# cy-rae/fast-slam

Hardware: AMD Instinct MI355X
Metric: particle-updates/s (higher is better)
Workload: dtype f64

## Files before the change

### fast-slam_amd/csrc/fs2_api.hip

```cpp
#include <hip/hip_runtime.h>

#include <sched.h>
#include <unistd.h>

#include <algorithm>
#include <atomic>
#include <chrono>
#include <condition_variable>
#include <functional>
#include <cmath>
#include <cstdarg>
#include <cstdio>
#include <cstdlib>
#include <cstring>
#include <mutex>
#include <new>
#include <string>
#include <thread>
#include <tuple>
#include <vector>

#include "../../include/fs2.h"
#include "fs2_comm.hpp"
#include "fs2_frontend.hpp"
// ... 190 lines not shown
        return n;
    }
};
ChunkCache g_chunks;

std::atomic<int> g_vm_fail_after_relocate{0};
struct GmStep {
    const char *what;
    size_t bytes;
    std::chrono::steady_clock::time_point t0 = std::chrono::steady_clock::now();
    ~GmStep() {
        static const bool on = std::getenv("FS2_TRACE") != nullptr;
        if (!on) return;
        const double ms = std::chrono::duration<double, std::milli>(std::chrono::steady_clock::now() - t0).count();
        std::fprintf(stderr, "[fs2 vmm] %s %zu MiB %.3f ms\n", what, bytes >> 20, ms);
    }
};
static void gm_drop(const GrowMem &g, size_t b, hipMemGenericAllocationHandle_t hd) {
    if (!g_chunks.put(ChunkCache::Chunk{g.device, g.shareable, b, hd})) (void)hipMemRelease(hd);
}
static hipError_t gm_grow(GrowMem &g, size_t bytes) {
    const size_t need = (bytes + g.gran - 1) / g.gran * g.gran;
    if (need <= g.mapped) return hipSuccess;
    std::vector<size_t> plan;
    size_t want = g.mapped;
    while (want < need) {
        plan.push_back(chunk_size(need - want, g.gran));
        want += plan.back();
    }
    if (want > g.reserved) {
        GmStep st{"relocate", want};
        const hipError_t e = gm_relocate(g, want);
        if (e != hipSuccess) return e;
        if (g_vm_fail_after_relocate.exchange(0)) return gm_fail(hipErrorOutOfMemory);
    }
    hipMemAllocationProp prop = gm_prop(g.device, g.shareable);
    const size_t mapped0 = g.mapped, nchunks0 = g.chunks.size();
    hipError_t e = hipSuccess;
    int cached = 0;
    {
        GmStep st{"chunks", want - mapped0};
        for (size_t b : plan) {
            hipMemGenericAllocationHandle_t hd{};
            if (g_chunks.take(g.device, g.shareable, b, &hd)) {
                ++cached;
            } else {
                e = hipMemCreate(&hd, b, &prop, 0);
                if (e == hipErrorOutOfMemory && g_chunks.release() > 0) {
                    (void)hipGetLastError();
                    e = hipMemCreate(&hd, b, &prop, 0);
                }
                if (e != hipSuccess) break;
            }
            e = hipMemMap(g.base + g.mapped, b, 0, hd, 0);
            if (e != hipSuccess) {
                gm_drop(g, b, hd);
                break;
            }
            g.chunks.push_back({hd, b});
            g.mapped += b;
        }
    }
    if (e == hipSuccess) {
        GmStep st{"access", want};
        e = gm_access(g, g.base, want);
    }
    if (e != hipSuccess) {
        while (g.chunks.size() > nchunks0) {
            const auto c = g.chunks.back();
            g.chunks.pop_back();
            g.mapped -= c.second;
            (void)hipMemUnmap(g.base + g.mapped, c.second);
            gm_drop(g, c.second, c.first);
        }
        g.mapped = mapped0;
        return gm_fail(e);
    }
    if (cached && std::getenv("FS2_TRACE")) std::fprintf(stderr, "[fs2 vmm] %d of %zu chunks from closed handles\n", cached, plan.size());
    return hipSuccess;
}
static void gm_free(GrowMem &g) {
    GmStep st{"free", g.mapped};
    size_t off = g.mapped;
    for (auto it = g.chunks.rbegin(); it != g.chunks.rend(); ++it) {
        off -= it->second;
        hipMemUnmap(g.base + off, it->second);
        gm_drop(g, it->second, it->first);
    }
    g.chunks.clear();
    if (g.base) hipMemAddressFree(g.base, g.reserved);
    g = GrowMem{};
}

struct Pool {
    const char *name;
    size_t item_bytes;
    int64_t id_limit;
    char *data = nullptr;
    int64_t n = 0;
    GrowMem vm;
    uint8_t *mark = nullptr;
    GrowMem mark_vm;
    uint32_t *freel = nullptr;
    GrowMem freel_vm;
    int64_t nfree = 0, cursor = 0;
    uint8_t epoch = 0;
    int64_t *bcnt = nullptr;
    int64_t bcnt_cap = 0;
    int64_t *nfree_dev = nullptr;

    int64_t room() const { return nfree - cursor; }
    int64_t live() const { return n - room(); }
    bool in_place() const { return vm.base && data == vm.base; }
    hipError_t next_epoch(hipStream_t s) {
        if (epoch == 255) {
            const hipError_t e = hipMemsetAsync(mark, 0, (size_t)n, s);
            if (e != hipSuccess) return e;
            epoch = 0;
        }
        epoch += 1;
        return hipSuccess;
    }
    bool mapped() const { return vm.base || mark_vm.base || freel_vm.base; }
    void release() {
        if (vm.base) gm_free(vm); else hipFree(data);
        if (mark_vm.base) gm_free(mark_vm); else hipFree(mark);
        if (freel_vm.base) gm_free(freel_vm); else hipFree(freel);
        hipFree(bcnt);
        hipFree(nfree_dev);
    }
};

}

struct MtCtx {
    fs2_mt_state in;
    double sigma = 0.0;
    int64_t N = 0, P = 0, A = 0, amb_cap = 0, pos0 = 0, have = 0, total = 0;
    int h0 = 0;
    fs2_mt_state *after = nullptr, *after_u0 = nullptr;
    double *u0_out = nullptr;
};

struct fs2_handle {
    fs2_config cfg{};
    int64_t n_global = 0, n = 0, first = 0;
    hipStream_t stream = nullptr;
    int cur = 0;
    double *x[2] = {}, *y[2] = {}, *yaw[2] = {}, *w[2] = {};
    int32_t *cnt[2] = {};
    Pool pages{"page", kPageBytes, (int64_t)kIdMask};
    Pool records{"record", kRecBytes, (int64_t)kRecIdLimit};
    Desc *pt[2] = {};
    uint32_t *bbox[2] = {};
    XDesc *rdesc = nullptr;
    XDesc *udesc = nullptr;
    size_t udesc_cap = 0;
    unsigned long long *xt_key = nullptr;
    uint32_t *xt_ref = nullptr, *xt_uidx = nullptr, *xt_cmask = nullptr, *xt_cbase = nullptr;
    uint32_t *xt_eslot = nullptr, *xt_ulist = nullptr;
    int64_t xt_cap = 0, xt_ecap = 0;
    SumFrame frame{-127.0f, 1.0f, 1.0f};
    float ext_seen = 0.0f;
    float *slb = nullptr;
    float *slb_pass = nullptr;
    uint32_t *ext_dev = nullptr;
    size_t rdesc_cap = 0;
    int rows = 0;
    uint32_t *sent_mask = nullptr;
    uint64_t collections = 0;
    int64_t u_recv = 0;
    int32_t *rank_d = nullptr, *rank_e = nullptr;
    int64_t *iblk = nullptr;
    int cap = 0, max_cap = kMaxSlots;
    double *wpart = nullptr, *part_sq = nullptr, *part_best_w = nullptr, *part_pose = nullptr;
    unsigned long long *cpart = nullptr;
    int64_t *part_best_i = nullptr;
    unsigned long long *part_slots = nullptr;
    int32_t *part_maxcnt = nullptr;
    double *cbuf = nullptr, *bsum = nullptr;
    DevStats *stats_dev = nullptr;
    char *post_host = nullptr, *post = nullptr;
    unsigned long long *post_flag = nullptr, *post_flag_dev = nullptr;
    unsigned long long post_seq = 0;
    PackPlan *plan = nullptr;
    DevStats *pub_stats = nullptr, *pub_stats_dev = nullptr;
    unsigned long long *pub_flag = nullptr, *pub_flag_dev = nullptr;
    unsigned long long pub_seq = 0;
    bool stats_clean = false;
    double *noise_dev = nullptr, *noise_pin = nullptr, *u0_dev = nullptr, *u0_pin = nullptr;
    struct MtWork {
        uint32_t *raw[2] = {};
        int64_t raw_cap[2] = {};
        int cur = 0;
        hipStream_t side = nullptr;
        hipEvent_t ev_words = nullptr, ev_pre = nullptr;
        bool pre_valid = false;
        uint32_t pre_key[2][624];
        int32_t pre_spos[2];
        int64_t pre_pos0[2];
        int64_t pre_total = 0;
        int32_t *boff = nullptr;
        int64_t boff_cap = 0;
        MtMeta *meta = nullptr, *meta_pin = nullptr;
        MtAmb *amb = nullptr, *amb_pin = nullptr;
        int64_t amb_cap = 0;
        uint32_t *words_pin = nullptr;
        int64_t *pidx = nullptr, *pidx_pin = nullptr;
        double *pval = nullptr, *pval_pin = nullptr;
        int64_t patch_cap = 0, pval_cap = 0;
        double *tab = nullptr;
        int64_t jJ = 0;
        int jG = 0;
        uint64_t *jpoly = nullptr;
        uint32_t *jwin = nullptr;
        bool tab_ready = false;
        bool armed = false;
        hipStream_t dstream = nullptr;
        hipEvent_t ev_in = nullptr, ev_noise = nullptr;
        bool deferred = false;
        MtCtx dc;
    } mt;
    int32_t *assoc_dev = nullptr;
    int64_t assoc_cap = 0;
    int32_t last_m = 0;
    uint64_t scan = 0;
    struct Pending {
        bool on = false;
        unsigned long long seq = 0;
        bool prof = false;
        int passes = 0;
        int32_t m = 0;
        uint64_t fixed_bytes = 0;
    } pending;
    struct TailCtx {
        int32_t M = 0;
        int passes = 0;
        uint64_t fixed_bytes = 0;
        bool prof = false;
        int evset = 0;
        int32_t want_collect = 0;
        bool has_u0 = false;
        int par = 0;
    };
    struct {
        bool on = false;
        int rc = FS2_OK;
        double pose[3] = {};
        fs2_iter_stats st{};
    } stash;
    uint32_t *gen_dev = nullptr;
    unsigned long long *go_dev = nullptr;
    BufSet *sets_dev = nullptr;
    uint64_t submitted = 0;
    int32_t cnt_upper = 0;
    double gate2 = 64.0;
    std::string err;
    bool profiling = false;
    int32_t prof_period = 1;
    uint64_t prof_tick = 0;
    ProfEvents ev;
    fs2_profile prof{};
    fs2comm::Transport *tp = nullptr;
    RankRecord *rec = nullptr, *recs = nullptr;
    double *totals = nullptr;
    int64_t *xrow = nullptr, *xmat = nullptr;
    int32_t *mlo = nullptr, *mhi = nullptr, *out_src = nullptr;
    uint32_t *runs_n = nullptr;
    int4 *runs = nullptr;
    uint64_t *cand = nullptr;
    int32_t *ncand = nullptr;
    char *sarena = nullptr, *rarena = nullptr;
    size_t scap = 0, rcap = 0;
    int32_t n_recv = 0;
    int32_t shard = 0;
    int8_t rank_of[kMaxRanks] = {};
    bool follow = false;
    uint64_t shard_moves = 0;

    int32_t *uinfo = nullptr, *uol = nullptr, *seql = nullptr, *bC = nullptr, *bpc = nullptr;
    uint32_t *bM = nullptr;
    int32_t *uel = nullptr, *bE = nullptr, *bpe = nullptr;
    long long *udelta = nullptr;
    unsigned long long *ugl = nullptr, *bD = nullptr, *bpd = nullptr;
    double *sout = nullptr, *part_w = nullptr, *np_part = nullptr, *np_leaf = nullptr, *sentry = nullptr;
    NpTailPlan *np_tail = nullptr;
    UnitRec *urec = nullptr;
    bool xsh_ok = false;
    bool refs = false;
    bool refs_off = false;
    bool refuse_maps = false;
    bool room_check = false;
    bool refs_shared = false;
    bool vm_share = false;
    uint32_t loc_epoch = 0;
    bool refs_live = false;
    uint64_t grows = 0;
    uint64_t vm_fallbacks = 0;
    int64_t appends_since_rcollect = 0;
    bool rcollect_exact = true;
    std::vector<uint8_t> imported;
    PeerMaps peers_host{};
    PeerMaps *peers_dev = nullptr;
    uint8_t *ep_dev = nullptr, *epochs_dev = nullptr;
    int64_t remote_rows = 0;
    int64_t remote_pages = INT64_MAX;
    int64_t remote_bound() const { return std::min(remote_rows, remote_pages); }
    int32_t collect_next = 0;
    ChainSummary *dch_send = nullptr, *dch_recv = nullptr;
    RankRecordX *recx = nullptr, *recxs = nullptr;
    double *est_base = nullptr;
    int32_t *uop = nullptr;
    NpTailPlan *np_tail_g = nullptr;
    std::vector<std::pair<hipEvent_t, hipEvent_t>> xev;
    size_t xev_used = 0;
    struct Guard {
        char *at;
        const char *name;
    };
    std::vector<Guard> guards;
    bool guard = false;
    char *json_text = nullptr;
    int64_t *json_boff = nullptr;
    size_t json_text_cap = 0, json_boff_cap = 0;
    double *post_part = nullptr, *post_out = nullptr;
    unsigned long long *post_grid = nullptr;
    size_t post_part_cap = 0, post_out_cap = 0, post_grid_cap = 0;
    char *map_scr = nullptr, *map_out = nullptr;
    double *map_part = nullptr;
    unsigned long long *map_grid = nullptr;
    size_t map_scr_cap = 0, map_out_cap = 0, map_part_cap = 0, map_grid_cap = 0;

    MapRef map() const {
        return MapRef{pages.data, pt[cur], std::max<int64_t>(n, 1), rows, records.data, frame, slb, row_boxes(cur),
                      refs_shared ? peers_dev : nullptr};
    }
    uint32_t *row_boxes(int b) const { return rows <= kBBoxRows ? bbox[b] : nullptr; }
    int64_t nblocks() const { return (n + kBlock - 1) / kBlock; }
    int reduce() const {
        const int mode = cfg.reduce_mode;
        if (tp) {
            if (mode == FS2_REDUCE_SEQUENTIAL) return FS2_REDUCE_SEQUENTIAL;
            return (mode != FS2_REDUCE_PARALLEL && xsh_ok) ? FS2_REDUCE_EXACT : FS2_REDUCE_PARALLEL;
        }
        if (mode != FS2_REDUCE_AUTO) return mode;
        return n_global <= 4096 ? FS2_REDUCE_SEQUENTIAL : FS2_REDUCE_EXACT;
    }
    ChainParams chain(const double *a, const double *bsum, double *c, double *total, bool lazy) const {
        ChainParams p{};
        p.a = a;
        p.n = n;
        p.bsum = bsum;
        p.nb = (int32_t)nblocks();
        p.lazy = lazy ? 1 : 0;
        p.uinfo = uinfo;
        p.udelta = udelta;
        p.ugl = ugl;
        p.uol = uol;
        p.bD = bD;
        p.bC = bC;
        p.bM = bM;
        p.bpd = bpd;
        p.bpc = bpc;
        p.uel = uel;
        p.bE = bE;
        p.bpe = bpe;
        p.seql = seql;
        p.sout = sout;
        p.urec = urec;
        p.sentry = sentry;
        p.c = c;
        p.total = total;
        p.stats = stats_dev;
        p.margin = std::ldexp(2.0 * (double)n_global + 8192.0, -53);
        p.chain_first = 1;
        return p;
    }
};

static hipError_t copy_sync(fs2_handle *h, void *dst, const void *src, size_t bytes, hipMemcpyKind kind) {
    hipError_t e = hipMemcpyAsync(dst, src, bytes, kind, h->stream);
    return e == hipSuccess ? hipStreamSynchronize(h->stream) : e;
}

struct CommTimer {
    fs2_handle *h;
    std::chrono::steady_clock::time_point t0 = std::chrono::steady_clock::now();
    explicit CommTimer(fs2_handle *hh) : h(hh) {}
    ~CommTimer();
};

CommTimer::~CommTimer() {
    if (!h->profiling) return;
    h->prof.comm_calls += 1;
    h->prof.comm_ms += std::chrono::duration<double, std::milli>(std::chrono::steady_clock::now() - t0).count();
}

static int recv_bufs(fs2_handle *h, size_t bytes) {
    if (bytes <= h->rdesc_cap && bytes <= h->udesc_cap) return FS2_OK;
    HIP_TRY(h, hipStreamSynchronize(h->stream));
    for (int k = 0; k < 2; ++k) {
        XDesc *&p = k ? h->udesc : h->rdesc;
        size_t &cap = k ? h->udesc_cap : h->rdesc_cap;
        if (bytes <= cap) continue;
        hipFree(p);
        p = nullptr;
        cap = 0;
        HIP_TRY(h, hipMalloc(&p, bytes));
        cap = bytes;
    }
    return FS2_OK;
}

static int reserve_xfer_table(fs2_handle *h, int64_t cap, int64_t nrows, bool in_scan);
static int xfer_bufs(fs2_handle *h) {
    const int64_t S = std::max<int64_t>(h->n, 1) * h->rows;
    int lg = 10;
    while ((int64_t(1) << lg) < 2 * S && lg < 31) ++lg;
    const int rc = reserve_xfer_table(h, int64_t(1) << lg, S, false);
    return rc ? rc : recv_bufs(h, sizeof(XDesc) * (size_t)S);
}

static int sync_sets(fs2_handle *h) {
    if (!h->sets_dev) return FS2_OK;
    BufSet b[2];
    for (int k = 0; k < 2; ++k)
        b[k] = BufSet{h->x[k], h->y[k], h->yaw[k], h->w[k], h->cnt[k], h->pt[k], h->row_boxes(k)};
    HIP_TRY(h, copy_sync(h, h->sets_dev, b, sizeof b, hipMemcpyHostToDevice));
    return FS2_OK;
}

static int grow_rows(fs2_handle *h, int need_slots) {
    if (need_slots <= h->cap) return FS2_OK;
    if (need_slots > h->max_cap)
        return set_err(&h->err, FS2_ERR_CAPACITY, "map needs %d landmark slots, limit is %d",
                       need_slots, h->max_cap);
    int rows = (need_slots + kPageSlots - 1) / kPageSlots;
    if (h->rows > 0) {
        const int geo = h->rows + std::max(h->rows / 4, 8);
        const int lim = std::min(h->max_cap / kPageSlots, rows <= kBBoxRows ? kBBoxRows : INT_MAX);
        rows = std::max(rows, std::min(geo, lim));
    }
    const size_t row_bytes = sizeof(Desc) * (size_t)std::max<int64_t>(h->n, 1);
    HIP_TRY(h, hipStreamSynchronize(h->stream));
    for (int b = 0; b < 2; ++b) {
        Desc *p = nullptr;
        HIP_TRY(h, hipMalloc(&p, row_bytes * rows));
        if (h->pt[b] && b == h->cur) HIP_TRY(h, copy_sync(h, p, h->pt[b], row_bytes * h->rows, hipMemcpyDeviceToDevice));
        hipFree(h->pt[b]);
        h->pt[b] = p;
    }
    h->rows = rows;
    h->cap = rows * kPageSlots;
    if (int rc = sync_sets(h)) return rc;
    if (h->rdesc) return xfer_bufs(h);
    return FS2_OK;
}

static int refs_short(fs2_handle *h, const char *what) {
    return set_err(&h->err, FS2_ERR_CAPACITY,
                   "page_refs mode: the %s pool ran short between collective collections (pools shared with "
                   "the other ranks cannot grow; size them with page_pool / record_pool)",
                   what);
}

static int collect_body(fs2_handle *h, bool recs_too);
struct PoolTimer {
    fs2_handle *h;
    bool grow;
    std::chrono::steady_clock::time_point t0 = std::chrono::steady_clock::now();
    ~PoolTimer() {
        const double ms = std::chrono::duration<double, std::milli>(std::chrono::steady_clock::now() - t0).count();
        if (grow) {
            h->prof.pool_grows += 1;
            h->prof.grow_ms += ms;
        } else {
            h->prof.pool_collections += 1;
            h->prof.collect_ms += ms;
        }
    }
};
static int collect(fs2_handle *h, bool recs_too) {
    PoolTimer pt{h, false};
    return collect_body(h, recs_too);
}
static int collect_records(fs2_handle *h) {
    Pool &p = h->pages, &r = h->records;
    if (r.n <= 0) return FS2_OK;
    hipStream_t s = h->stream;
    HIP_TRY(h, r.next_epoch(s));
// ... 707 lines not shown
    int prev_dev = -1;
    if (hipGetDevice(&prev_dev) != hipSuccess) prev_dev = -1;
    if (prev_dev != h->cfg.device) (void)hipSetDevice(h->cfg.device);
    if (h->stream) hipStreamSynchronize(h->stream);
    if (h->mt.dstream) hipStreamSynchronize(h->mt.dstream);
    const bool vmm = h->pages.mapped() || h->records.mapped();
    if (vmm) hipDeviceSynchronize();
    if (h->refs_shared && h->tp && !h->tp->in_process()) {
        std::string e;
        if (h->tp->allgather(h->ep_dev, h->epochs_dev, 1, h->stream, &e) == FS2_OK) hipStreamSynchronize(h->stream);
        h->tp->unshare();
        if (h->tp->allgather(h->ep_dev, h->epochs_dev, 1, h->stream, &e) == FS2_OK) hipStreamSynchronize(h->stream);
    }
    for (int s = 0; s < 2; ++s) {
        hipFree(h->x[s]); hipFree(h->y[s]); hipFree(h->yaw[s]); hipFree(h->w[s]); hipFree(h->cnt[s]);
        hipFree(h->pt[s]);
        hipFree(h->bbox[s]);
    }
    hipFree(h->rdesc); hipFree(h->udesc);
    hipFree(h->xt_key); hipFree(h->xt_ref); hipFree(h->xt_uidx); hipFree(h->xt_cmask); hipFree(h->xt_cbase);
    hipFree(h->xt_eslot); hipFree(h->xt_ulist);
    hipFree(h->sent_mask);
    h->pages.release();
    h->records.release();
    if (vmm) hipDeviceSynchronize();
    hipFree(h->slb); hipFree(h->slb_pass); hipFree(h->ext_dev);
    hipFree(h->rank_d); hipFree(h->rank_e); hipFree(h->iblk);
    hipFree(h->mlo); hipFree(h->mhi); hipFree(h->out_src); hipFree(h->runs); hipFree(h->runs_n);
    hipFree(h->rec); hipFree(h->recs); hipFree(h->totals); hipFree(h->xrow); hipFree(h->xmat);
    hipFree(h->sarena);
    hipFree(h->rarena);
    hipFree(h->cand); hipFree(h->ncand);
    hipFree(h->uinfo); hipFree(h->uol); hipFree(h->seql); hipFree(h->udelta); hipFree(h->ugl);
    hipFree(h->bD); hipFree(h->bC); hipFree(h->bM); hipFree(h->bpd); hipFree(h->bpc);
    hipFree(h->uel); hipFree(h->bE); hipFree(h->bpe);
    hipFree(h->sout); hipFree(h->np_leaf); hipFree(h->part_w); hipFree(h->np_part); hipFree(h->np_tail);
    hipFree(h->urec); hipFree(h->sentry);
    hipFree(h->dch_send); hipFree(h->dch_recv); hipFree(h->recx); hipFree(h->recxs); hipFree(h->est_base);
    hipFree(h->uop); hipFree(h->np_tail_g);
    hipFree(h->peers_dev); hipFree(h->ep_dev); hipFree(h->epochs_dev);
    hipFree(h->part_pose);
    hipFree(h->gen_dev); hipFree(h->sets_dev); hipFree(h->go_dev);
    hipFree(h->wpart); hipFree(h->cpart); hipFree(h->part_sq); hipFree(h->part_best_w); hipFree(h->part_best_i); hipFree(h->part_slots);
    hipFree(h->part_maxcnt); hipFree(h->cbuf); hipFree(h->bsum);
    hipFree(h->stats_dev); hipFree(h->noise_dev); hipFree(h->u0_dev); hipFree(h->assoc_dev);
    hipFree(h->json_text); hipFree(h->json_boff);
    hipFree(h->post_part); hipFree(h->post_out); hipFree(h->post_grid);
    hipFree(h->map_scr); hipFree(h->map_out); hipFree(h->map_part); hipFree(h->map_grid);
    if (h->post_host) hipHostFree(h->post_host);
    hipFree(h->plan);
    if (h->pub_stats) hipHostFree(h->pub_stats);
    if (h->noise_pin) hipHostFree(h->noise_pin);
    if (h->u0_pin) hipHostFree(h->u0_pin);
    if (h->mt.side) hipStreamSynchronize(h->mt.side);
    if (h->mt.dstream) {
        hipStreamSynchronize(h->mt.dstream);
        hipStreamDestroy(h->mt.dstream);
        hipEventDestroy(h->mt.ev_in);
        hipEventDestroy(h->mt.ev_noise);
    }
    hipFree(h->mt.raw[0]); hipFree(h->mt.raw[1]); hipFree(h->mt.boff);
    if (h->mt.ev_words) hipEventDestroy(h->mt.ev_words);
    if (h->mt.ev_pre) hipEventDestroy(h->mt.ev_pre);
    if (h->mt.side) hipStreamDestroy(h->mt.side); hipFree(h->mt.meta); hipFree(h->mt.amb); hipFree(h->mt.pidx);
    hipFree(h->mt.pval); hipFree(h->mt.tab); hipFree(h->mt.jpoly); hipFree(h->mt.jwin);
    if (h->mt.meta_pin) hipHostFree(h->mt.meta_pin);
    if (h->mt.amb_pin) hipHostFree(h->mt.amb_pin);
    if (h->mt.words_pin) hipHostFree(h->mt.words_pin);
    if (h->mt.pidx_pin) hipHostFree(h->mt.pidx_pin);
    if (h->mt.pval_pin) hipHostFree(h->mt.pval_pin);
    if (h->ev.ok)
        for (auto &set : h->ev.e)
            for (auto &e : set) hipEventDestroy(e);
    for (auto &e : h->xev) {
        hipEventDestroy(e.first);
        hipEventDestroy(e.second);
    }
    delete h->tp;
    if (h->stream) hipStreamDestroy(h->stream);
    const int dev = h->cfg.device;
    delete h;
    if (prev_dev >= 0 && prev_dev != dev) (void)hipSetDevice(prev_dev);
}

int fs2_create(const fs2_config *cfg, fs2_handle **out) {
    if (!cfg || !out) return set_err(nullptr, FS2_ERR_ARG, "fs2_create: null argument");
    *out = nullptr;
    if (cfg->num_particles <= 0)
        return set_err(nullptr, FS2_ERR_ARG, "num_particles must be positive");
    if (cfg->world_size < 1 || cfg->rank < 0 || cfg->rank >= cfg->world_size)
        return set_err(nullptr, FS2_ERR_ARG, "bad rank %d / world_size %d", cfg->rank, cfg->world_size);
    if (cfg->world_size > kMaxRanks)
        return set_err(nullptr, FS2_ERR_ARG, "world_size %d > %d", cfg->world_size, kMaxRanks);
    if (cfg->num_particles > (int64_t)INT32_MAX)
        return set_err(nullptr, FS2_ERR_ARG, "too many particles per rank");
    int ndev = 0;
    if (hipGetDeviceCount(&ndev) != hipSuccess || ndev == 0)
        return set_err(nullptr, FS2_ERR_HIP, "no HIP device available (libfs2 has no CPU path)");
    if (cfg->device < 0 || cfg->device >= ndev)
        return set_err(nullptr, FS2_ERR_ARG, "device %d out of range (%d devices)", cfg->device, ndev);

    fs2_handle *h = new fs2_handle();
    h->cfg = *cfg;
    h->n_global = cfg->num_particles;
    const int64_t G = cfg->world_size, r = cfg->rank;
    h->first = (h->n_global * r) / G;
    h->n = (h->n_global * (r + 1)) / G - h->first;
    h->shard = (int32_t)r;
    for (int q = 0; q < kMaxRanks; ++q) h->rank_of[q] = (int8_t)(q < G ? q : 0);
    {
        const char *e = std::getenv("FS2_SHARD_FOLLOW");
        h->follow = G > 1 && h->n_global % G == 0 && !(e && std::strcmp(e, "0") == 0);
    }
    h->max_cap = cfg->max_landmark_capacity > 0 ? std::min(cfg->max_landmark_capacity, kMaxSlots) : kMaxSlots;
    h->gate2 = gate_to_q(cfg->max_landmark_distance);
    auto fail = [&](int code) {
        std::string msg = h->err;
        free_handle(h);
        g_last_error = msg;
        return code;
    };
    if (hipSetDevice(cfg->device) != hipSuccess) return fail(set_err(&h->err, FS2_ERR_HIP, "hipSetDevice failed"));
    if (hipStreamCreateWithFlags(&h->stream, hipStreamNonBlocking) != hipSuccess)
        return fail(set_err(&h->err, FS2_ERR_HIP, "hipStreamCreate failed"));
    const int64_t n = std::max<int64_t>(h->n, 1);
    const int64_t nb = (n + kBlock - 1) / kBlock;
    const int64_t nsb = (n + 1023) / 1024;
    const bool guard = [] {
        const char *e = std::getenv("FS2_GUARD");
        return e && *e && std::strcmp(e, "0") != 0;
    }();
    h->guard = guard;
    auto alloc = [&](void **p, size_t bytes, const char *name) {
        const size_t b = bytes > 0 ? bytes : 16, tot = guard ? b + kGuardBytes : b;
        hipError_t e = hipMalloc(p, tot);
        if (e == hipErrorOutOfMemory && g_chunks.release() > 0) {
            (void)hipGetLastError();
            e = hipMalloc(p, tot);
        }
        if (e == hipSuccess && guard) {
            e = hipMemset(static_cast<char *>(*p) + b, kGuardByte, kGuardBytes);
            h->guards.push_back(fs2_handle::Guard{static_cast<char *>(*p) + b, name});
        }
        return e;
    };
#define FS2_ALLOC(ptr, bytes) alloc((void **)&(ptr), (size_t)(bytes), #ptr)
    bool ok = true;
    for (int s = 0; s < 2; ++s) {
        ok &= FS2_ALLOC(h->x[s], n * 8) == hipSuccess;
        ok &= FS2_ALLOC(h->y[s], n * 8) == hipSuccess;
        ok &= FS2_ALLOC(h->yaw[s], n * 8) == hipSuccess;
        ok &= FS2_ALLOC(h->w[s], n * 8) == hipSuccess;
        ok &= FS2_ALLOC(h->cnt[s], n * 4) == hipSuccess;
        ok &= FS2_ALLOC(h->bbox[s], nb * kBBoxRows * 4) == hipSuccess;
    }
    ok &= FS2_ALLOC(h->pages.nfree_dev, sizeof(int64_t)) == hipSuccess;
    ok &= FS2_ALLOC(h->records.nfree_dev, sizeof(int64_t)) == hipSuccess;
    ok &= FS2_ALLOC(h->slb, sizeof(float)) == hipSuccess;
    ok &= FS2_ALLOC(h->slb_pass, sizeof(float)) == hipSuccess;
    ok &= FS2_ALLOC(h->ext_dev, sizeof(uint32_t)) == hipSuccess;
    ok &= FS2_ALLOC(h->mlo, n * 4) == hipSuccess;
    ok &= FS2_ALLOC(h->mhi, n * 4) == hipSuccess;
    ok &= FS2_ALLOC(h->out_src, n * 4) == hipSuccess;
    ok &= FS2_ALLOC(h->runs, sizeof(int4) * kMaxLongRuns) == hipSuccess;
    ok &= FS2_ALLOC(h->runs_n, 4) == hipSuccess && hipMemset(h->runs_n, 0, 4) == hipSuccess;
    ok &= FS2_ALLOC(h->cand, n * 8 * kMaxCand) == hipSuccess;
    ok &= FS2_ALLOC(h->ncand, n * 4) == hipSuccess;
    ok &= FS2_ALLOC(h->rec, sizeof(RankRecord)) == hipSuccess;
    ok &= FS2_ALLOC(h->recs, sizeof(RankRecord) * G) == hipSuccess;
    ok &= FS2_ALLOC(h->totals, sizeof(double) * G) == hipSuccess;
    ok &= FS2_ALLOC(h->xrow, sizeof(int64_t) * kXrowWords * G) == hipSuccess;
    ok &= FS2_ALLOC(h->xmat, sizeof(int64_t) * kXrowWords * G * G) == hipSuccess;
    ok &= FS2_ALLOC(h->rank_d, n * 4) == hipSuccess;
    ok &= FS2_ALLOC(h->rank_e, n * 4) == hipSuccess;
    ok &= FS2_ALLOC(h->iblk, (2 * nsb + 2) * 8) == hipSuccess;
    ok &= FS2_ALLOC(h->wpart, nb * 8) == hipSuccess;
    ok &= FS2_ALLOC(h->cpart, 2 * nb * 8 * kNumCounters) == hipSuccess;
    ok &= FS2_ALLOC(h->gen_dev, 4) == hipSuccess;
    ok &= FS2_ALLOC(h->go_dev, 8) == hipSuccess;
    ok &= FS2_ALLOC(h->sets_dev, 2 * sizeof(BufSet)) == hipSuccess;
    ok &= FS2_ALLOC(h->part_sq, nb * 8) == hipSuccess;
    ok &= FS2_ALLOC(h->part_best_w, nb * 8) == hipSuccess;
    ok &= FS2_ALLOC(h->part_pose, nb * 24) == hipSuccess;
    ok &= FS2_ALLOC(h->part_best_i, nb * 8) == hipSuccess;
    ok &= FS2_ALLOC(h->part_slots, nb * 8) == hipSuccess;
    ok &= FS2_ALLOC(h->part_maxcnt, nb * 4) == hipSuccess;
    ok &= FS2_ALLOC(h->cbuf, n * 8) == hipSuccess;
    ok &= FS2_ALLOC(h->bsum, nsb * 8) == hipSuccess;
    ok &= FS2_ALLOC(h->stats_dev, sizeof(DevStats)) == hipSuccess;
    {
        const int64_t nu = (n + 63) / 64;
        ok &= FS2_ALLOC(h->uinfo, nu * 4) == hipSuccess;
        ok &= FS2_ALLOC(h->uol, nu * 4) == hipSuccess;
        const int64_t ng = (nu + kChainGroup - 1) / kChainGroup;
        ok &= FS2_ALLOC(h->bD, ng * 8) == hipSuccess;
        ok &= FS2_ALLOC(h->bC, ng * 4) == hipSuccess;
        ok &= FS2_ALLOC(h->bM, ng * 4) == hipSuccess;
        ok &= FS2_ALLOC(h->bpd, ng * 8) == hipSuccess;
        ok &= FS2_ALLOC(h->bpc, ng * 4) == hipSuccess;
        ok &= FS2_ALLOC(h->uel, nu * 4) == hipSuccess;
        ok &= FS2_ALLOC(h->bE, ng * 4) == hipSuccess;
        ok &= FS2_ALLOC(h->bpe, ng * 4) == hipSuccess;
        ok &= FS2_ALLOC(h->seql, nu * 4) == hipSuccess;
        ok &= FS2_ALLOC(h->udelta, nu * 8) == hipSuccess;
        ok &= FS2_ALLOC(h->ugl, nu * 8) == hipSuccess;
        ok &= FS2_ALLOC(h->sout, nu * 8) == hipSuccess;
        ok &= FS2_ALLOC(h->sentry, nu * 8) == hipSuccess;
        ok &= FS2_ALLOC(h->urec, nu * sizeof(UnitRec)) == hipSuccess;
        ok &= FS2_ALLOC(h->np_leaf, (np_sumsq_chunks(n) * 64 + 64) * 8) == hipSuccess;
        ok &= FS2_ALLOC(h->part_w, nb * 8) == hipSuccess;
#ifdef FS2_AB_OLD_NP_PART
        ok &= FS2_ALLOC(h->np_part, np_sumsq_chunks(n) * 8) == hipSuccess;
#else
        ok &= FS2_ALLOC(h->np_part,
                    std::max<int64_t>(np_sumsq_chunks(n), normalize_chunk_parts(n)) * 8) == hipSuccess;
#endif
    }
    ok &= FS2_ALLOC(h->noise_dev, n * 8) == hipSuccess;
    ok &= FS2_ALLOC(h->u0_dev, 8) == hipSuccess;
    {
        const size_t body = sizeof(DevStats) + sizeof(int64_t) * kXrowWords * kMaxRanks * kMaxRanks;
        const size_t off = ((body + 63) / 64) * 64;
        ok &= hipHostMalloc((void **)&h->post_host, off + 128, hipHostMallocCoherent | hipHostMallocMapped) ==
              hipSuccess;
        if (ok) {
            h->post_flag = reinterpret_cast<unsigned long long *>(h->post_host + off);
            *h->post_flag = 0;
            ok &= hipHostGetDevicePointer((void **)&h->post, h->post_host, 0) == hipSuccess;
            if (ok) h->post_flag_dev = reinterpret_cast<unsigned long long *>(h->post + off);
        }
    }
    ok &= FS2_ALLOC(h->plan, sizeof(PackPlan) * kMaxRanks) == hipSuccess;
    ok &= hipHostMalloc((void **)&h->pub_stats, sizeof(DevStats) + 128, hipHostMallocCoherent | hipHostMallocMapped) ==
          hipSuccess;
    if (ok) {
        const size_t off = ((sizeof(DevStats) + 63) / 64) * 64;
        h->pub_flag = reinterpret_cast<unsigned long long *>(reinterpret_cast<char *>(h->pub_stats) + off);
        *h->pub_flag = 0;
        ok &= hipHostGetDevicePointer((void **)&h->pub_stats_dev, h->pub_stats, 0) == hipSuccess;
        if (ok)
            h->pub_flag_dev = reinterpret_cast<unsigned long long *>(reinterpret_cast<char *>(h->pub_stats_dev) + off);
    }
    ok &= hipHostMalloc((void **)&h->noise_pin, 2 * n * 8, 0) == hipSuccess;
    ok &= hipHostMalloc((void **)&h->u0_pin, 2 * 8, 0) == hipSuccess;
    if (!ok) return fail(set_err(&h->err, FS2_ERR_OOM, "device allocation failed for %lld particles", (long long)n));
    if (hipMemsetAsync(h->cpart, 0, 2 * nb * 8 * kNumCounters, h->stream) != hipSuccess ||
        hipMemsetAsync(h->gen_dev, 0, 4, h->stream) != hipSuccess ||
        hipMemsetAsync(h->go_dev, 0, 8, h->stream) != hipSuccess ||
        hipMemsetD32Async((hipDeviceptr_t)h->slb, 0x7f7fffff, 1, h->stream) != hipSuccess)
        return fail(set_err(&h->err, FS2_ERR_HIP, "state initialisation failed"));
    for (int s = 0; s < 2; ++s) {
        if (hipMemsetAsync(h->x[s], 0, n * 8, h->stream) != hipSuccess ||
            hipMemsetAsync(h->y[s], 0, n * 8, h->stream) != hipSuccess ||
            hipMemsetAsync(h->yaw[s], 0, n * 8, h->stream) != hipSuccess ||
            hipMemsetAsync(h->cnt[s], 0, n * 4, h->stream) != hipSuccess ||
            hipMemsetD32Async((hipDeviceptr_t)h->bbox[s], (int)kBoxEmpty, nb * kBBoxRows, h->stream) != hipSuccess ||
            launch_fill(h->w[s], 1.0 / (double)h->n_global, n, h->stream) != hipSuccess)
            return fail(set_err(&h->err, FS2_ERR_HIP, "state initialisation failed"));
    }
    {
        NpTailPlan plan;
        if (np_tail_plan(h->n, &plan)) {
            if (hipMalloc(&h->np_tail, sizeof plan) != hipSuccess ||
                hipMemcpy(h->np_tail, &plan, sizeof plan, hipMemcpyHostToDevice) != hipSuccess)
                return fail(set_err(&h->err, FS2_ERR_HIP, "state initialisation failed"));
        }
    }
    if (G > 1) {
        NpTailPlan gp;
        const bool gpart = np_tail_plan(h->n_global, &gp);
        const int64_t min_shard = h->n_global / G, max_shard = (h->n_global + G - 1) / G;
        h->xsh_ok = min_shard >= kNpChunk && max_shard / kNpChunk + 1 <= kShardChunks && (!gpart || gp.nl <= 128);
        if (cfg->reduce_mode == FS2_REDUCE_EXACT && !h->xsh_ok)
            return fail(set_err(&h->err, FS2_ERR_ARG,
                                "exact reductions across %d shards need >= %d particles per shard (%lld)",
                                (int)G, kNpChunk, (long long)min_shard));
        if (h->xsh_ok) {
            const int64_t nu = (n + 63) / 64;
            bool ok2 = hipMalloc(&h->dch_send, sizeof(ChainSummary)) == hipSuccess &&
                       hipMalloc(&h->dch_recv, sizeof(ChainSummary) * G) == hipSuccess &&
                       hipMalloc(&h->recx, sizeof(RankRecordX)) == hipSuccess &&
                       hipMalloc(&h->recxs, sizeof(RankRecordX) * G) == hipSuccess &&
                       hipMalloc(&h->est_base, sizeof(double)) == hipSuccess &&
                       hipMalloc(&h->uop, sizeof(int32_t) * (size_t)std::max<int64_t>(nu, 1)) == hipSuccess;
            if (ok2 && gpart)
                ok2 = hipMalloc(&h->np_tail_g, sizeof gp) == hipSuccess &&
                      hipMemcpy(h->np_tail_g, &gp, sizeof gp, hipMemcpyHostToDevice) == hipSuccess;
            if (ok2) ok2 = hipMemset(h->recx, 0, sizeof(RankRecordX)) == hipSuccess;
            if (!ok2) return fail(set_err(&h->err, FS2_ERR_OOM, "sharded reduction buffers"));
        }
    }
    int rc = grow_rows(h, std::max(cfg->landmark_capacity, 1));
    if (rc) return fail(rc);
    const int64_t recv_pages = G > 1 ? n / 2 * h->rows : 0;
    const int64_t recv_recs = G > 1 ? n / 2 * h->rows * kPageSlots : 0;
    int64_t npages = cfg->page_pool > 0 ? cfg->page_pool : n * h->rows * 2 + 8 * n + recv_pages + 1024;
    const bool refs_wanted = cfg->page_refs == 1;
    if (G > 1 && refs_wanted) {
        const int64_t lim = (int64_t)kRefIdMask - 1024;
        if (cfg->page_pool <= 0 && npages > lim && lim >= n * h->rows + n * h->rows / 4 + 8 * n) npages = lim;
        h->refs = G <= kRefMaxRanks && npages <= lim;
        h->vm_share = h->refs && cfg->comm_mode != FS2_COMM_LOCAL;
        if (h->refs && cfg->page_pool <= 0) npages = std::min(lim, npages + 24 * n);
        if (cfg->page_refs == 1 && !h->refs)
            return fail(set_err(&h->err, FS2_ERR_ARG, "page_refs: needs 2..%d ranks and a page pool below %lld pages",
                                kRefMaxRanks, (long long)lim));
    }
    rc = grow(h, h->pages, npages);
    if (rc) return fail(rc);
    rc = grow(h, h->records, cfg->record_pool > 0 ? cfg->record_pool
                                                   : n * h->cap + n * h->cap / 4 + 64 * n + recv_recs + 1024 +
                                                         (h->refs ? 24 * n : 0));
    if (rc) return fail(rc);
    if (G > 1) {
        const int64_t K = n / 2 + 1, S = K * h->rows;
        rc = xfer_bufs(h);
        const size_t bytes = (size_t)xfer_bytes(K, S, S, 0) + 256 * kMaxRanks;
        if (!rc) rc = ensure_arena(h, h->sarena, h->scap, bytes);
        if (!rc) rc = ensure_arena(h, h->rarena, h->rcap, bytes);
        if (rc) return fail(rc == FS2_ERR_OOM ? set_err(&h->err, rc, "sharded transfer buffers") : rc);
    }
    if (G > 1 || cfg->sharded_path) {
        rc = (cfg->comm_mode == FS2_COMM_LOCAL) ? fs2comm::create_local(cfg->comm_id, (int)G, (int)r, &h->tp, &h->err)
             : (cfg->comm_mode == FS2_COMM_SHM) ? fs2comm::create_shm(cfg->comm_id, (int)G, (int)r, &h->tp, &h->err)
                                                 : fs2comm::create_rccl(cfg->comm_id, (int)G, (int)r, &h->tp, &h->err);
        if (rc) return fail(rc);
    }
    if (h->refs &&
        (hipMalloc(&h->peers_dev, sizeof(PeerMaps)) != hipSuccess || hipMalloc(&h->ep_dev, 64) != hipSuccess ||
         hipMalloc(&h->epochs_dev, 2 * kMaxRanks) != hipSuccess))
        return fail(set_err(&h->err, FS2_ERR_OOM, "page_refs tables"));
    if (hipStreamSynchronize(h->stream) != hipSuccess)
        return fail(set_err(&h->err, FS2_ERR_HIP, "initialisation sync failed"));
    *out = h;
    return FS2_OK;
}

void fs2_destroy(fs2_handle *h) { free_handle(h); }

int fs2_shard_info(const fs2_handle *h, int64_t *n_local, int64_t *first_global, int32_t *capacity) {
    if (!h) return set_err(nullptr, FS2_ERR_ARG, "null handle");
    if (n_local) *n_local = h->n;
    if (first_global) *first_global = h->first;
    if (capacity) *capacity = h->cap;
    return FS2_OK;
}

int fs2_synchronize(fs2_handle *h) {
    if (!h) return set_err(nullptr, FS2_ERR_ARG, "null handle");
    HIP_TRY(h, hipStreamSynchronize(h->stream));
    return FS2_OK;
}

int fs2_set_profiling(fs2_handle *h, int32_t enable) {
    if (!h) return set_err(nullptr, FS2_ERR_ARG, "null handle");
    if (h->pending.on) return set_err(&h->err, FS2_ERR_STATE, "a submitted scan is pending (fs2_iterate_wait first)");
    if (enable && !h->ev.ok) {
        for (auto &set : h->ev.e)
            for (auto &e : set) HIP_TRY(h, hipEventCreate(&e));
        h->ev.ok = true;
    }
    h->ev.used = 0;
    h->xev_used = 0;
    h->profiling = enable > 0;
    h->prof_period = enable > 0 ? enable : 1;
    h->prof_tick = 0;
    h->prof = fs2_profile{};
    return FS2_OK;
}

static int fold_profile(fs2_handle *h);

int fs2_get_profile(const fs2_handle *hc, fs2_profile *out) {
    if (!hc || !out) return set_err(nullptr, FS2_ERR_ARG, "null argument");
    fs2_handle *h = const_cast<fs2_handle *>(hc);
    if (h->pending.on) return set_err(&h->err, FS2_ERR_STATE, "a submitted scan is pending (fs2_iterate_wait first)");
    const int rc = fold_profile(h);
    if (rc) return rc;
    for (size_t k = 0; k < h->xev_used; ++k) {
        float ms = 0.0f;
        HIP_TRY(h, hipEventSynchronize(h->xev[k].second));
        HIP_TRY(h, hipEventElapsedTime(&ms, h->xev[k].first, h->xev[k].second));
        h->prof.exchange_ms += ms;
    }
    h->xev_used = 0;
    *out = h->prof;
    out->page_refs = h->refs_off ? -1 : (h->refs ? 1 : 0);
    return FS2_OK;
}

static int fold_one(fs2_handle *h, int set);

static int fold_profile(fs2_handle *h) {
    const int used = h->ev.used;
    h->ev.used = 0;
    for (int k = 0; k < used; ++k) {
        const int rc = fold_one(h, k);
        if (rc) return rc;
    }
    return FS2_OK;
}

static int fold_one(fs2_handle *h, int set) {
    const ProfScan &p = h->ev.scan[set];
    hipEvent_t *E = h->ev.e[set];
    HIP_TRY(h, hipEventSynchronize(E[3]));
    const DevStats &st = p.st;
    float a = 0, f = 0, r = 0, x = 0, t = 0;
    HIP_TRY(h, hipEventElapsedTime(&a, E[0], E[2]));
    HIP_TRY(h, hipEventElapsedTime(&r, E[5], E[3]));
    HIP_TRY(h, hipEventElapsedTime(&t, E[0], E[3]));
    const uint64_t n = (uint64_t)h->n, nblk = (uint64_t)h->nblocks();
    const uint64_t box_rows = h->row_boxes(h->cur) ? (uint64_t)h->rows : 0ull;
    const bool filt = h->cfg.gate_filter != 0;
    const uint64_t cand_bytes = filt ? sizeof(Desc) * st.groups + 128ull * st.opened + 8ull * st.words +
                                           8ull * n * p.passes + 4ull * box_rows * nblk
                                     : 0ull;
    const uint64_t upd_fixed = p.fixed_bytes + (filt ? 4ull * n * p.passes : 0ull) + 8ull * n * (uint64_t)p.m;
    const uint64_t exact_bytes = upd_fixed + (filt ? 8ull * st.words : 0ull) + 48ull * st.candidates +
                                 (64ull + sizeof(Desc)) * st.written + (2ull * kPageBytes + sizeof(Desc)) * st.cow_pages +
                                 8ull * box_rows * nblk;
    if (filt && p.m <= kMaxM) {
        HIP_TRY(h, hipEventElapsedTime(&f, E[0], E[1]));
        HIP_TRY(h, hipEventElapsedTime(&x, E[4], E[2]));
        h->prof.exact_launches += 1;
        h->prof.exact_ms += x;
        h->prof.filter_launches += 1;
        h->prof.filter_ms += f;
        h->prof.filter_bytes += cand_bytes;
        h->prof.model_groups += st.groups;
        h->prof.model_opened += st.opened;
        h->prof.model_words += st.words;
        h->prof.model_candidates += st.candidates;
        h->prof.model_written += st.written;
        h->prof.model_cow += st.cow_pages;
        h->prof.model_fixed_bytes += upd_fixed;
        h->prof.model_box_bytes += 12ull * box_rows * nblk;
    }
    h->prof.scans += 1;
    h->prof.update_launches += p.passes;
    h->prof.update_ms += a;
    h->prof.reduce_ms += r;
    h->prof.scan_ms += t;
    h->prof.update_bytes += cand_bytes + exact_bytes;
    if (st.resampled)
        h->prof.resample_bytes += 2ull * sizeof(Desc) * (st.resample_slots / kPageSlots) +
                                  2ull * 36ull * (uint64_t)h->n + 40ull * (uint64_t)h->n;
    return FS2_OK;
}

static int wait_flag(fs2_handle *h, unsigned long long seq) {
    const auto t0 = std::chrono::steady_clock::now();
    for (unsigned it = 0;; ++it) {
        if (__atomic_load_n(h->pub_flag, __ATOMIC_ACQUIRE) == seq) return FS2_OK;
        if ((it & 1023u) == 1023u && std::chrono::steady_clock::now() - t0 > std::chrono::milliseconds(50)) break;
        __builtin_ia32_pause();
    }
    HIP_TRY(h, hipStreamSynchronize(h->stream));
    if (__atomic_load_n(h->pub_flag, __ATOMIC_ACQUIRE) != seq)
        return set_err(&h->err, FS2_ERR_HIP, "scan statistics were not published");
    return FS2_OK;
}

static int enqueue_tail(fs2_handle *h, const fs2_handle::TailCtx &t) {
    int rc = FS2_OK;
    const int cur = h->cur;
    hipStream_t s = h->stream;
    const int G = h->cfg.world_size;
    const bool sh = h->tp != nullptr;
    const int red = h->reduce();
    const bool seq = red == FS2_REDUCE_SEQUENTIAL && !sh;
    const bool exact = red == FS2_REDUCE_EXACT;
    const double flip_margin = (red == FS2_REDUCE_PARALLEL) ? std::ldexp(2.0 * (double)h->n_global + 64.0, -53) : 0.0;
    const bool prof = t.prof;
    hipEvent_t *E = h->ev.e[t.evset];
    ReduceParams rp{};
    rp.n = h->n;
    rp.n_global = h->n_global;
    rp.gidx0 = h->first;
    rp.w = h->w[cur];
    rp.cnt = h->cnt[cur];
    rp.x = h->x[cur]; rp.y = h->y[cur]; rp.yaw = h->yaw[cur];
    rp.wpart = h->wpart;
    rp.cpart = h->cpart + (size_t)t.par * kNumCounters * (size_t)h->nblocks();
    rp.nwpart = (int32_t)h->nblocks();
    rp.part_sq = h->part_sq;
    rp.part_best_w = h->part_best_w;
    rp.part_best_i = h->part_best_i;
    rp.part_maxcnt = h->part_maxcnt;
    rp.nparts = (int32_t)h->nblocks();
    rp.floor = h->cfg.weight_floor;
    rp.sequential = seq ? 1 : 0;
    rp.exact = exact ? 1 : 0;
    rp.np_part = h->np_part;
    rp.n_np = (int32_t)np_sumsq_chunks(h->n);
    rp.flip_margin = flip_margin;
    rp.part_w = exact ? h->part_w : nullptr;
    rp.np_leaf = exact ? h->np_leaf : nullptr;
    rp.chunked = (exact && !sh) ? 1 : 0;
    if (rp.chunked) rp.nparts = normalize_chunk_parts(h->n);
    rp.part_pose = h->part_pose;
    rp.np_tail = exact ? h->np_tail : nullptr;
    rp.u0_host = t.has_u0 ? h->u0_dev : nullptr;
    rp.seed = h->cfg.seed;
    rp.scan = h->scan;
    rp.stats = h->stats_dev;
    rp.world = G;
    rp.rank = h->cfg.rank;
    rp.shard = h->shard;
    std::memcpy(rp.rank_of, h->rank_of, sizeof rp.rank_of);
    rp.rec = h->rec;
    rp.recs = sh ? h->recs : h->rec;
    rp.totals = h->totals;
    rp.want_collect = t.want_collect;

    const int nxt = 1 - cur;
    ResampleParams rs{};
    rs.n = h->n;
    rs.N = h->n_global;
    rs.a = h->first;
    rs.ao = h->first;
    rs.keep = h->shard;
    rs.ranges_mode = (sh && h->follow) ? 1 : 3;
    rs.w = h->w[cur];
    rs.c = h->cbuf;
    rs.bsum = h->bsum;
    rs.nblk = (int32_t)((h->n + 1023) / 1024);
    rs.mlo = h->mlo;
    rs.mhi = h->mhi;
    rs.out_src = h->out_src;
    rs.runs = h->runs;
    rs.runs_n = h->runs_n;
    rs.x = h->x[cur]; rs.y = h->y[cur]; rs.yaw = h->yaw[cur]; rs.cnt = h->cnt[cur];
    rs.ox = h->x[nxt]; rs.oy = h->y[nxt]; rs.oyaw = h->yaw[nxt]; rs.ow = h->w[nxt]; rs.ocnt = h->cnt[nxt];
    rs.map = h->map();
    rs.opt = h->pt[nxt];
    rs.obbox = h->row_boxes(nxt);
    rs.rank_d = h->rank_d;
    rs.rank_e = h->rank_e;
    rs.iblk = h->iblk;
    rs.part_best_w = h->part_best_w;
    rs.part_best_i = h->part_best_i;
    rs.part_slots = h->part_slots;
    rs.stats = h->stats_dev;
    rs.rec = h->rec;
    rs.flip_margin = flip_margin;
    rs.use_chain = exact ? 1 : 0;
    rs.refs = h->refs ? 1 : 0;
    if (h->refs && h->xt_key) {
        rs.tkey = h->xt_key;
        rs.tcap = h->xt_cap;
        rs.tepoch = ++h->loc_epoch;
    }
    rs.chain = ChainView{h->uinfo, h->ugl, h->uol, h->bpd, h->bpc, h->seql, h->sout, h->uel, h->bpe};
    rs.gen = sh ? nullptr : h->gen_dev;

    const bool xsh = sh && exact;
    if (prof && exact && !xsh && h->n <= 0) HIP_TRY(h, hipEventRecord(E[5], s));
    if (exact && !xsh) {
        ChainParams cp = h->chain(h->w[cur], h->wpart, nullptr, &h->stats_dev->total, false);
        cp.cpart = h->cpart + (size_t)t.par * kNumCounters * (size_t)h->nblocks();
        cp.ncpart = (int32_t)h->nblocks();
        cp.cstats = h->stats_dev;
        HIP_TRY(h, launch_chain(cp, s, prof ? E[5] : nullptr));
    } else {
        HIP_TRY(h, launch_wsum(rp, s, prof ? E[5] : nullptr));
    }
    auto chain_ops = [&](ChainParams cp, const double *est) -> int {
        cp.chain_first = h->shard == 0 ? 1 : 0;
        cp.force_list0 = 1;
        cp.est_base = est;
        cp.ops_out = h->dch_send;
        cp.uop = h->uop;
        HIP_TRY(h, launch_chain_export(cp, s));
        CommTimer ct(h);
        return h->tp->allgather(h->dch_send, h->dch_recv, sizeof(ChainSummary), s, &h->err);
    };
    if (sh) {
        {
            CommTimer ct(h);
            rc = h->tp->allgather(&h->stats_dev->total, h->totals, sizeof(double), s, &h->err);
        }
        if (rc) return rc;
        rp.est_base = xsh ? h->est_base : nullptr;
        HIP_TRY(h, launch_global_total(rp, s));
        if (xsh) {
            rc = chain_ops(h->chain(h->w[cur], h->wpart, nullptr, nullptr, false), h->est_base);
            if (rc) return rc;
            HIP_TRY(h, launch_chain_fold(h->dch_recv, G, h->shard, h->rank_of, &h->stats_dev->total, nullptr,
                                         h->stats_dev, s));
// ... 2560 lines not shown
```

### fast-slam_amd/csrc/fs2_kernels.hpp

```cpp
#pragma once

#include <hip/hip_ext.h>
#include <hip/hip_runtime.h>
#include <stdint.h>

#include <vector>

namespace fs2 {

constexpr int kBlock = 256;
constexpr int kPageSlots = 8;
constexpr int kMaxSlots = 4096;
constexpr int kMaxRows = kMaxSlots / kPageSlots;
constexpr int kMaxM = 4;
constexpr int kScanGroup = kPageSlots;
constexpr int kMaxCand = 8;

constexpr int kPageBytes = 128;
constexpr int kRecBytes = 48;
constexpr uint32_t kOwned = 0x80000000u;
constexpr uint32_t kIdMask = 0x7fffffffu;
constexpr uint32_t kRecIdLimit = 0xffffffffu;
typedef uint32_t Desc;
typedef uint2 XDesc;
// ... 73 lines not shown
}

constexpr int kNpChunk = 8192;
constexpr int kNpMaxLeaves = 256;
struct NpTailPlan {
    int32_t nl;
    int32_t off[kNpMaxLeaves], len[kNpMaxLeaves];
    int32_t a[kNpMaxLeaves], b[kNpMaxLeaves];
};

struct RankRecord {
    double sumsq;
    double best_w;
    int64_t best_gidx;
    double pose[3];
    double t_local;
    int32_t max_count;
    int32_t want_collect;
};

constexpr int kMaxRanks = 16;

constexpr int kChainOpsCap = 2046;
struct ShardOrder {
    int8_t r[kMaxRanks];
};
struct ChainSummary {
    int32_t nops;
    int32_t pad[3];
    double ops[kChainOpsCap];
};
static_assert(sizeof(ChainSummary) == 16384, "ChainSummary layout");

constexpr int kShardChunks = 1024;
struct NpEdge {
    int32_t chunk;
    int32_t leaf0, nleaf;
    int32_t cut;
    int32_t rfrom, nraw;
    int32_t pad[2];
    double leaf[128];
    double raw[128];
};
struct RankRecordX {
    RankRecord base;
    int32_t nsums;
    int32_t first_chunk;
    int32_t pad[14];
    NpEdge head, tail;
    double sums[kShardChunks];
};
static_assert(sizeof(RankRecordX) <= 16384, "RankRecordX fits an all-gather slot");

struct XferPage {
    uint32_t cbase;
    uint8_t fill;
    uint8_t cmask;
    uint16_t pad0;
    uint16_t slot[8];
    uint64_t pad1;
    double2 xy[8];
};
static_assert(sizeof(XferPage) == 160, "XferPage layout");
constexpr int kXferCovBytes = 32;
constexpr int kXrowWords = 6;
constexpr uint32_t kEntryOwned = 0x80000000u;
__host__ __device__ inline int64_t xfer_idx_off(int64_t K) { return K * 64; }
__host__ __device__ inline int64_t xfer_page_off(int64_t K, int64_t S) { return K * 64 + ((S * 4 + 63) / 64) * 64; }
__host__ __device__ inline int64_t xfer_cov_off(int64_t K, int64_t S, int64_t U) {
    return xfer_page_off(K, S) + U * (int64_t)sizeof(XferPage);
}
__host__ __device__ inline int64_t xfer_bytes(int64_t K, int64_t S, int64_t U, int64_t C) {
    return xfer_cov_off(K, S, U) + C * kXferCovBytes;
}

struct PackHeader {
    int64_t gsrc;
    int32_t out_lo, out_hi;
    int32_t cnt;
    int32_t soff;
    double x, y, yaw, w;
    int64_t pad;
};

struct PackPlan {
    int64_t i0, i1;
    int64_t e0, c0;
    int64_t K, S;
    int64_t pa, pb;
};

struct RefPreamble {
    float slb;
    float org, cell, icell;
    int32_t rank;
    int32_t pad[11];
};
static_assert(sizeof(RefPreamble) == 64, "RefPreamble layout");
__host__ __device__ inline int64_t xfer_ref_bytes(int64_t K, int64_t S) { return 64 + K * 64 + S * 8; }

struct RecvPeer {
    const PackHeader *hdr;
    const uint32_t *idx;
    const XferPage *pages;
    const double2 *covs;
    const XDesc *refs;
    const RefPreamble *pre;
    int32_t K;
    int32_t kbase;
    int64_t U;
    int64_t ubase;
};

struct XferTable {
    unsigned long long *key;
    uint32_t *ref;
    uint32_t *uidx;
    uint32_t *cmask;
    uint32_t *cbase;
    uint32_t *eslot;
    uint32_t *ulist;
    int64_t cap;
    int32_t log2cap;
    int64_t ebase[kMaxRanks + 1];
    int64_t ubase[kMaxRanks + 1];
    int64_t i_lo, i_hi;
};

struct MeasPack {
    double d[kMaxM], b[kMaxM], ox[kMaxM], oy[kMaxM];
    float fx[kMaxM], fy[kMaxM];
    float fe[kMaxM];
};

constexpr int kRefShift = 27;
constexpr uint32_t kRefIdMask = (1u << kRefShift) - 1u;
constexpr int kRefMaxRanks = 15;
struct PeerMaps {
    char *pool[kMaxRanks];
    char *recs[kMaxRanks];
    uint8_t *mark[kMaxRanks];
};
__host__ __device__ inline uint32_t ref_tag(uint32_t e) { return (e & 0x80000000u) ? 0u : (e >> kRefShift) & 15u; }
__host__ __device__ inline uint32_t ref_id(uint32_t e) { return (e & 0x80000000u) ? (e & 0x7fffffffu) : (e & kRefIdMask); }

struct MapRef {
    char *pool;
    Desc *pt;
    int64_t n;
    int32_t rows;
    char *recs;
    SumFrame frame;
    float *slb;
    uint32_t *bbox;
    const PeerMaps *peers;
};

struct PageAlloc {
    const uint32_t *freel;
    int64_t base;
    const uint32_t *rfreel;
    int64_t rbase;
};

struct BufSet {
    double *x, *y, *yaw, *w;
    int32_t *cnt;
    Desc *pt;
    uint32_t *bbox;
};

struct UpdateParams {
    int64_t n;
    int64_t blk0, blk1;
    int64_t nblk;
    int64_t gidx0;
    double *x, *y, *yaw, *w;
    int32_t *cnt;
    MapRef map;
    const double *noise;
    uint64_t seed, scan;
    double sigma;
    double rotation, translation;
    int32_t do_move;
    int32_t move_cand;
    int32_t m;
    int32_t k0;
    int32_t last_pass;
    double gate2;
    float gate2f;
    int32_t filter;
    PageAlloc alloc;
    uint64_t *cand;
    int32_t *ncand;
    double R[4];
    double init_cov[4];
    int32_t *assoc;
    double *wpart;
    unsigned long long *cpart;
    DevStats *stats;
    MeasPack meas;
    float *slb_pass;
    const uint32_t *gen;
    const BufSet *sets;
};

struct ReduceParams {
    int64_t n;
    int64_t n_global;
    int64_t gidx0;
    double *w;
    const int32_t *cnt;
    const double *x, *y, *yaw;
    const double *wpart;
    int32_t nwpart;
    unsigned long long *cpart;
    double *part_sq;
    double *part_best_w;
    int64_t *part_best_i;
    int32_t *part_maxcnt;
    int32_t nparts;
    double floor;
    int32_t sequential;
    int32_t exact;
    double *np_part;
    int32_t n_np;
    double *np_leaf;
    int32_t chunked;
    double *part_pose;
    const NpTailPlan *np_tail;
    double flip_margin;
    double *part_w;
    int32_t t_from_parts;
    int32_t want_collect;
    double *est_base;
    const double *u0_host;
    uint64_t seed, scan;
    DevStats *stats;
    RankRecord *rec;
    const RankRecord *recs;
    const double *totals;
    int32_t world, rank;
    int32_t shard;
    int8_t rank_of[kMaxRanks];
    DevStats *pub_host;
    unsigned long long *pub_flag;
    unsigned long long pub_seq;
};

struct ChainView {
    const int32_t *uinfo;
    const unsigned long long *ugl;
    const int32_t *uol;
    const unsigned long long *bpd;
    const int32_t *bpc;
    const int32_t *seql;
    const double *sout;
    const int32_t *uel;
    const int32_t *bpe;
};

struct ResampleParams {
    int64_t n;
    int64_t N;
    int64_t a;
    int64_t ao;
    int32_t keep;
    int32_t ranges_mode;
    double *w;
    double *c;
    double *bsum;
    int32_t nblk;
    int32_t lazy;
    uint32_t *gen;
    unsigned long long *tkey;
    int64_t tcap;
    uint32_t tepoch;
    double flip_margin;
    int32_t use_chain;
    ChainView chain;
    int32_t *mlo, *mhi;
    int32_t *out_src;
    int4 *runs;
    uint32_t *runs_n;
    const double *x, *y, *yaw;
    const int32_t *cnt;
    double *ox, *oy, *oyaw, *ow;
    int32_t *ocnt;
    MapRef map;
    Desc *opt;
    uint32_t *obbox;
    XDesc *rdesc;
    XDesc *udesc;
    PageAlloc alloc;
    int32_t *rank_d;
    int32_t *rank_e;
    int64_t *iblk;
    double *part_best_w;
    int64_t *part_best_i;
    unsigned long long *part_slots;
    DevStats *stats;
    RankRecord *rec;
    int32_t world, rank;
    PackPlan *plan;
    int64_t *xrow;
    char *sbuf[kMaxRanks];
    XferTable xt;
    uint32_t *sent_mask;
    double init_cov[4];
    int32_t npeers;
    RecvPeer peers[kMaxRanks];
    int32_t refs;
    int32_t est_early;
    unsigned long long *go;
    unsigned long long go_seq;
};

constexpr int kChainSegs = 8;
constexpr int kChainGroup = 16;
struct UnitRec {
    int32_t meta[kChainSegs];
    double val[kChainSegs];
};

struct ChainParams {
    const double *a;
    int64_t n;
    const double *bsum;
    int32_t nb;
    int32_t lazy;
    const unsigned long long *cpart;
    int32_t ncpart;
    DevStats *cstats;
    int32_t *uinfo;
    UnitRec *urec;
    double *sentry;
    long long *udelta;
    unsigned long long *ugl;
    int32_t *uol;
    unsigned long long *bD;
    int32_t *bC;
    uint32_t *bM;
    int32_t *uel;
    int32_t *bE;
    int32_t *bpe;
    unsigned long long *bpd;
    int32_t *bpc;
    int32_t *seql;
    double *sout;
    double *c;
    double *total;
    const DevStats *stats;
    double margin;
    int32_t chain_first;
    int32_t force_list0;
    const double *est_base;
    ChainSummary *ops_out;
    const double *s_entry;
    int32_t *uop;
};
hipError_t launch_chain(const ChainParams &p, hipStream_t s, hipEvent_t e0 = nullptr);
hipError_t launch_chain_export(const ChainParams &p, hipStream_t s);
hipError_t launch_chain_fold(const ChainSummary *all, int32_t world, int32_t shard, const int8_t *rank_of,
                             double *total, double *entry, DevStats *stats, hipStream_t s);
hipError_t launch_chain_walk_from(const ChainParams &p, hipStream_t s);
hipError_t launch_np_shard(const double *w, int64_t n, int64_t first, int64_t n_global, const NpTailPlan *gtail,
                           RankRecordX *rx, hipStream_t s);
hipError_t launch_global_finalize_x(const ReduceParams &p, const RankRecordX *all, const NpTailPlan *gtail,
                                    hipStream_t s);
bool np_tail_plan(int64_t n, NpTailPlan *out);
int64_t np_sumsq_chunks(int64_t n);

#define FS2_LAUNCH_EV(k, g, b, s, e0, e1, ...)                                   \
    do {                                                                         \
        if ((e0) || (e1)) hipExtLaunchKernelGGL(k, g, b, 0, s, e0, e1, 0, __VA_ARGS__); \
        else hipLaunchKernelGGL(k, g, b, 0, s, __VA_ARGS__);                     \
    } while (0)

hipError_t launch_candidates(const UpdateParams &p, hipStream_t s, hipEvent_t e0 = nullptr,
                             hipEvent_t e1 = nullptr);
hipError_t launch_update(const UpdateParams &p, hipStream_t s, hipEvent_t e0 = nullptr, hipEvent_t e1 = nullptr);
hipError_t launch_wsum(const ReduceParams &p, hipStream_t s, hipEvent_t e0 = nullptr);
hipError_t launch_normalize(const ReduceParams &p, hipStream_t s);
hipError_t launch_normalize_chunks(const ReduceParams &p, hipStream_t s);
int32_t normalize_chunk_parts(int64_t n);
hipError_t launch_finalize_chunked(const ReduceParams &p, hipStream_t s);
hipError_t launch_global_total(const ReduceParams &p, hipStream_t s);
hipError_t launch_prefix(const ResampleParams &p, int sequential, hipStream_t s);
hipError_t launch_finalize(const ReduceParams &p, hipStream_t s);
hipError_t launch_global_finalize(const ReduceParams &p, hipStream_t s);
hipError_t launch_resample_ranges(const ResampleParams &p, hipStream_t s, bool fill_runs = true);
hipError_t launch_pack_count(const ResampleParams &p, hipStream_t s);
hipError_t launch_pack_dedup(const ResampleParams &p, hipStream_t s);
hipError_t launch_pack_write(const ResampleParams &p, hipStream_t s);
hipError_t launch_pack_refs(const ResampleParams &p, hipStream_t s);
struct LocalizeParams {
    MapRef map;
    const int32_t *cnt;
    int64_t n;
    int64_t nblk;
    int32_t m;
    float gate2f;
    MeasPack meas;
    const uint32_t *freel;
    int64_t ftail;
    const uint32_t *rfreel;
    int64_t rtail;
    int64_t pcap, rcap;
    DevStats *stats;
    unsigned long long *key;
    uint32_t *val;
    int64_t cap;
    uint32_t epoch;
};
hipError_t launch_localize(const LocalizeParams &p, hipStream_t s);
hipError_t launch_resample_apply(const ResampleParams &p, bool estimate, hipStream_t s);
hipError_t launch_global_best(const ReduceParams &p, hipStream_t s);
hipError_t launch_publish(DevStats *stats, DevStats *host_stats, unsigned long long *host_flag,
                          unsigned long long seq, hipStream_t s, hipEvent_t e1 = nullptr);
hipError_t launch_post(const DevStats *stats, const int64_t *xmat, int32_t nx, char *host,
                       unsigned long long *host_flag, unsigned long long seq, hipStream_t s);
hipError_t launch_tail_single(const ResampleParams &r, const ReduceParams &p, DevStats *host_stats,
                              unsigned long long *host_flag, unsigned long long seq, hipStream_t s,
                              hipEvent_t e1 = nullptr);

#ifdef FS2_PHASE_TIMING
hipError_t debug_phase_times(unsigned long long out[8], int reset);
hipError_t debug_icp_phase_times(unsigned long long out[4], int reset);
hipError_t debug_chain_times(unsigned long long out[8], int reset);
hipError_t debug_fin_times(unsigned long long out[8], int reset);
hipError_t debug_tail_times_update(unsigned long long out[32], int reset);
hipError_t debug_tail_times_exact(unsigned long long out[32], int reset);
hipError_t debug_tail_times_resample(unsigned long long out[32], int reset);
#endif
hipError_t launch_import(const double *stage, const int32_t *cnt_stage, int64_t first,
                         int64_t count, int32_t lm_cap, MapRef map, PageAlloc alloc,
                         int32_t rows_each, int32_t *cnt, uint32_t *ext, const int32_t *perm,
                         int32_t perm_len, hipStream_t s);
hipError_t launch_bbox_build(MapRef map, const int32_t *cnt, hipStream_t s);
hipError_t launch_export(double *stage, int64_t first, int64_t count, int32_t lm_cap,
                         MapRef map, const int32_t *cnt, hipStream_t s);
hipError_t launch_fill(double *p, double v, int64_t n, hipStream_t s);
hipError_t launch_iota(uint32_t *p, int64_t n, hipStream_t s);
hipError_t launch_iota_from(uint32_t *p, uint32_t v0, int64_t n, hipStream_t s);

hipError_t launch_collect(MapRef map, const int32_t *cnt, int64_t npool, uint8_t *mark,
                          uint8_t epoch, int64_t *bcnt, uint32_t *freel, int64_t *nfree_dev,
                          hipStream_t s);
hipError_t launch_collect_mark(MapRef map, const int32_t *cnt, uint8_t *mark, uint8_t epoch, const uint8_t *epochs,
                               hipStream_t s);
hipError_t launch_collect_sweep(int64_t npool, uint8_t *mark, uint8_t epoch, int64_t *bcnt, uint32_t *freel,
                                int64_t *nfree_dev, hipStream_t s);
hipError_t launch_collect_records(const char *pool, int64_t npool, const uint8_t *mark, uint8_t epoch,
                                  int64_t nrecs, uint8_t *rmark, uint8_t repoch, int64_t *rbcnt,
                                  uint32_t *rfreel, int64_t *rnfree_dev, hipStream_t s);
int64_t collect_blocks(int64_t npool);
hipError_t launch_mark_records(const char *pool, int64_t npool, const uint8_t *mark, uint8_t epoch, int64_t nrecs,
                               uint8_t *rmark, uint8_t repoch, hipStream_t s);
hipError_t launch_sweep_scan(int64_t *bcnt, int64_t nb, int64_t *total, hipStream_t s);

hipError_t launch_snap_count(const uint8_t *mark, int64_t npool, uint8_t epoch, int64_t *bcnt, hipStream_t s);
hipError_t launch_snap_table(const uint8_t *mark, int64_t npool, uint8_t epoch, const int64_t *bcnt, uint32_t *tab,
                             uint32_t *list, hipStream_t s);
hipError_t launch_snap_rows(MapRef map, const int32_t *cnt, const uint32_t *ptab, int64_t npool, int r0, int nrows,
                            uint32_t *out, hipStream_t s);
hipError_t launch_snap_gather(const char *pool, const uint32_t *ids, int64_t k, int L, const uint32_t *rtab,
                              int64_t nrecs, void *out, hipStream_t s);
hipError_t launch_snap_mark_sel(MapRef map, const int32_t *cnt, const int64_t *idx, int64_t m, int R, int64_t npool,
                                uint8_t *mark, uint8_t epoch, hipStream_t s);
hipError_t launch_snap_scalars_sel(const double *src, const int64_t *idx, int64_t k, double *out, hipStream_t s);
hipError_t launch_snap_scalars_sel(const int32_t *src, const int64_t *idx, int64_t k, int32_t *out, hipStream_t s);
hipError_t launch_snap_rows_sel(MapRef map, const int32_t *cnt, const int64_t *idx, const uint8_t *sel, int64_t m,
                                const uint32_t *ptab, int64_t npool, int r0, int nrows, uint32_t *out,
                                hipStream_t s);
struct SnapView;
hipError_t launch_snap_scatter(const void *in, const uint32_t *ids, int64_t k, int L, char *pool, hipStream_t s);
hipError_t launch_snap_check(const SnapView &v, int pass, uint32_t *owners, uint8_t *shared, uint32_t *flags,
                             hipStream_t s);
hipError_t launch_snap_commit(char *pool, const uint32_t *pids, int64_t U, const uint32_t *rids, int64_t C,
                              const uint32_t *src, Desc *dst, int64_t n, int R, const int32_t *cnt, hipStream_t s);

hipError_t cluster_points(const double2 *pts, int64_t n, double eps, int64_t min_samples, double *centres_out,
                          int64_t centres_cap, int64_t *nclusters, int32_t *labels_out, int32_t *status,
                          hipStream_t s);
hipError_t gather_map_points(MapRef map, const int32_t *cnt, int64_t n, double2 **pts_out, int64_t *npts,
                             hipStream_t s);

hipError_t launch_debug_philox(int64_t n, const uint32_t *ctr, const uint32_t *key, uint32_t *out, hipStream_t s);
hipError_t launch_debug_normals(uint64_t seed, uint64_t stream, uint64_t first, int64_t n, double *out,
                                hipStream_t s);

struct MtMeta {
    int64_t accepted;
    int64_t last_attempt;
    double gauss;
    int32_t has_gauss;
    int32_t amb_n;
    int64_t E;
    int32_t pos_after, pos_after_u0;
    uint32_t w_u0[2];
    uint32_t key_after[624], key_after_u0[624];
};
struct MtAmb {
    double r2, x1, x2;
    int64_t rank;
};
hipError_t launch_mt_words(uint32_t *R, int64_t begin, int64_t end, hipStream_t s);
hipError_t launch_mt_draw(const uint32_t *R, int64_t pos0, int64_t b_in, int64_t A, int64_t P, int64_t N, int32_t h0,
                          double gauss0, double sigma, int64_t first, int64_t n_local, double *out,
                          int32_t *boff, MtMeta *meta, MtAmb *amb, int32_t amb_cap, double *tab, int32_t tab_ready,
                          MtMeta *meta_host, hipStream_t s);
hipError_t launch_mt_patch(double *out, const int64_t *idx, const double *val, int64_t n, hipStream_t s);
constexpr int kMtMaxGen = 16;
hipError_t launch_mt_words_parallel(uint32_t *R, int64_t total, const uint64_t *g, int pw, int G, int64_t J,
                                    uint32_t *win, hipStream_t s);
bool mt_jump_polys(uint64_t J, int G, std::vector<uint64_t> &out);
int mt_poly_words();
bool mt_jump_host(const uint32_t key[624], uint64_t J, uint32_t out[624]);
hipError_t launch_mt_debug_log(const double *x, int64_t n, double *out, int32_t *amb, hipStream_t s);

constexpr int kJsonBlock = 256;
constexpr int kJsonMaxDepth = 6;
const uint64_t *json_host_table();
hipError_t json_device_table(int device, const uint64_t **out);
int64_t json_max_bytes(int64_t n, int depth);
hipError_t launch_json_sizes(const uint64_t *tab, const double *x, const double *y, const double *yaw, int64_t n,
                             int depth, int64_t *boff, hipStream_t s, hipEvent_t after_sizes);
hipError_t launch_json_write(const uint64_t *tab, const double *x, const double *y, const double *yaw, int64_t n,
                             int depth, const int64_t *boff, char *text, hipStream_t s);
hipError_t launch_repr_doubles(const uint64_t *tab, const double *v, int64_t n, char *out, uint8_t *len,
                               hipStream_t s);

hipError_t launch_icp(int32_t B, int32_t P, const double *src, const double *tgt,
                      int32_t n_tgt, int32_t max_iter, double thr, double *R, double *t,
                      int32_t *iters, hipStream_t s);
hipError_t launch_best_fit(const double *src, const double *tgt, int32_t n, double *Rt,
                           hipStream_t s);
hipError_t launch_line_filter(const double *in, int32_t n, const double *taps, int32_t r,
                              double *out, hipStream_t s);
hipError_t launch_mahalanobis(const double *a, const double *b, const double *cov, int32_t K,
                              double *out, int32_t *singular, hipStream_t s);
hipError_t launch_associate(const double *obs, const double *lm, int32_t L, double gate2,
                            int32_t *out, hipStream_t s);

}
```

### fast-slam_amd/csrc/fs2_reduce.hpp

```cpp
#pragma once

#include "fs2_device.hpp"
#include "fs2_kernels.hpp"

namespace fs2 {

#ifdef FS2_PHASE_TIMING
static __device__ unsigned long long g_tail[32];
#define FS2_TAIL_READER(name)                                                                \
    hipError_t name(unsigned long long out[32], int reset) {                                 \
        hipError_t e = hipMemcpyFromSymbol(out, HIP_SYMBOL(g_tail), sizeof(unsigned long long) * 32); \
        if (e == hipSuccess && reset) {                                                      \
            unsigned long long z[32] = {};                                                   \
            e = hipMemcpyToSymbol(HIP_SYMBOL(g_tail), z, sizeof z);                          \
        }                                                                                    \
        return e;                                                                            \
    }
#define FS2_TS_DECL unsigned long long ts_last_ = 0
#define FS2_TS(base, k)                                                                      \
    do {                                                                                     \
        if (blockIdx.x == 0 && threadIdx.x == 0) {                                           \
            const unsigned long long t_ = __builtin_amdgcn_s_memrealtime();                  \
            if ((k) > 0) atomicAdd(&g_tail[(base) + (k) - 1], t_ - ts_last_);               \
            ts_last_ = t_;                                                                   \
// ... 219 lines not shown
    const int wid = threadIdx.x >> 6, lane = threadIdx.x & 63;
    __syncthreads();
    if (lane == 0) lds[wid] = v;
    __syncthreads();
    int t = lds[0];
#pragma unroll
    for (int k = 1; k < NT / 64; ++k) t = max(t, lds[k]);
    return t;
}


__device__ __forceinline__ int wave_incl_scan_int(int v) {
    const int lane = threadIdx.x & 63;
#pragma unroll
    for (int d = 1; d < 64; d <<= 1) {
        const int o = __shfl_up(v, d, 64);
        if (lane >= d) v += o;
    }
    return v;
}

__device__ __forceinline__ int block_excl_scan(int v, int *lds, int *tot) {
    const int inc = wave_incl_scan_int(v);
    const int wid = threadIdx.x >> 6, lane = threadIdx.x & 63;
    if (lane == 63) lds[wid] = inc;
    __syncthreads();
    int off = 0, t = 0;
#pragma unroll
    for (int k = 0; k < kBlock / 64; ++k) {
        if (k < wid) off += lds[k];
        t += lds[k];
    }
    *tot = t;
    return off + inc - v;
}


typedef int v4i __attribute__((ext_vector_type(4)));

__device__ __forceinline__ char *page_ptr(char *pool, uint32_t e) {
    return pool + (int64_t)(e & kIdMask) * kPageBytes;
}

__device__ __forceinline__ Desc *pt_entry(const MapRef &m, int row, int64_t i) {
    return m.pt + (int64_t)row * m.n + i;
}

__device__ __forceinline__ char *page_of(const MapRef &m, int j, int64_t i) {
    return page_ptr(m.pool, *pt_entry(m, j / kPageSlots, i));
}

__device__ __forceinline__ const char *page_ptr_any(const MapRef &m, uint32_t e) {
    const uint32_t t = m.peers ? ref_tag(e) : 0u;
    return t ? m.peers->pool[t - 1] + (int64_t)ref_id(e) * kPageBytes : page_ptr(m.pool, e);
}
__device__ __forceinline__ const char *recs_of(const MapRef &m, uint32_t e) {
    const uint32_t t = m.peers ? ref_tag(e) : 0u;
    return t ? m.peers->recs[t - 1] : m.recs;
}

__device__ __forceinline__ float4 load_mirror(const char *page, int j) {
    return reinterpret_cast<const float4 *>(page)[j & (kPageSlots - 1)];
}

__device__ __forceinline__ uint32_t mirror_rec(const float4 &m) { return __float_as_uint(m.w); }

__device__ __forceinline__ Slot load_rec(const char *recs, uint32_t r) {
    const double2 *q = reinterpret_cast<const double2 *>(recs + (int64_t)r * kRecBytes);
    const double2 a = q[0], b = q[1], c = q[2];
    return Slot{a.x, a.y, M2{b.x, b.y, c.x, c.y}};
}

__device__ __forceinline__ void store_rec(char *recs, uint32_t r, const Slot &s) {
    typedef double v2d __attribute__((ext_vector_type(2)));
    v2d *qv = reinterpret_cast<v2d *>(recs + (int64_t)r * kRecBytes);
    __builtin_nontemporal_store((v2d){s.mx, s.my}, qv);
    __builtin_nontemporal_store((v2d){s.P.a00, s.P.a01}, qv + 1);
    __builtin_nontemporal_store((v2d){s.P.a10, s.P.a11}, qv + 2);
}

__device__ __forceinline__ Slot load_slot(const MapRef &m, const char *page, int j) {
    return load_rec(m.recs, mirror_rec(load_mirror(page, j)));
}

__device__ __forceinline__ uint32_t take_page(const PageAlloc &a, int64_t n, int64_t i, int &t) {
    const uint32_t id = a.freel[a.base + (int64_t)t * n + i];
    ++t;
    return id;
}

__device__ __forceinline__ uint32_t take_rec(const PageAlloc &a, int64_t n, int64_t i, int &t) {
    const uint32_t id = a.rfreel[a.rbase + (int64_t)t * n + i];
    ++t;
    return id;
}

__device__ __forceinline__ char *writable_page(const MapRef &m, int row, int64_t i,
                                               const PageAlloc &a, int &t, unsigned &cow) {
    Desc *pe = pt_entry(m, row, i);
    const uint32_t e = *pe;
    if (e & kOwned) return page_ptr(m.pool, e);
    const uint32_t id = take_page(a, m.n, i, t);
    const v4i *src = reinterpret_cast<const v4i *>(page_ptr(m.pool, e));
    v4i *dst = reinterpret_cast<v4i *>(page_ptr(m.pool, id));
    v4i v[kPageBytes / 16];
#pragma unroll
    for (int u = 0; u < kPageBytes / 16; ++u) v[u] = src[u];
#pragma unroll
    for (int u = 0; u < kPageBytes / 16; ++u) dst[u] = v[u];
    *pe = id | kOwned;
    ++cow;
    return reinterpret_cast<char *>(dst);
}

__device__ __forceinline__ char *fresh_page(const MapRef &m, int row, int64_t i, const PageAlloc &a,
                                            int &t) {
    const uint32_t id = take_page(a, m.n, i, t);
    *pt_entry(m, row, i) = id | kOwned;
    return page_ptr(m.pool, id);
}

__device__ __forceinline__ float4 store_slot(const MapRef &m, char *page, int pos, const Slot &s, uint32_t r,
                                             int slot) {
    store_rec(m.recs, r, s);
    float4 mv = with_slot(mirror_of(s), slot);
    mv.w = __uint_as_float(r);
    reinterpret_cast<float4 *>(page)[pos & (kPageSlots - 1)] = mv;
    return mv;
}


__device__ __forceinline__ double sum_grid(const SumFrame &f, double k) { return (double)f.org + k * (double)f.cell; }
__device__ __forceinline__ uint32_t sum_lo(const SumFrame &f, float v) {
    double k = floor(((double)v - (double)f.org) * (double)f.icell);
    if (!(k >= 0.0)) return 0u;
    k = fmin(k, 254.0);
    while (k >= 0.0 && sum_grid(f, k) > (double)v) k -= 1.0;
    return k >= 0.0 ? (uint32_t)k + 1u : 0u;
}
__device__ __forceinline__ uint32_t sum_hi(const SumFrame &f, float v) {
    double k = ceil(((double)v - (double)f.org) * (double)f.icell);
    if (!(k <= 254.0)) return 255u;
    k = fmax(k, 0.0);
    while (k <= 254.0 && sum_grid(f, k) < (double)v) k += 1.0;
    return k <= 254.0 ? (uint32_t)k : 255u;
}
__device__ __forceinline__ float sum_lo_val(const SumFrame &f, uint32_t c) {
    return c == 0u ? -INFINITY : __double2float_rd(sum_grid(f, (double)(c - 1u)));
}
__device__ __forceinline__ float sum_hi_val(const SumFrame &f, uint32_t c) {
    return c == 255u ? INFINITY : __double2float_ru(sum_grid(f, (double)c));
}

__device__ __forceinline__ uint32_t page_box(const float4 *mir, int nvalid, const SumFrame &f) {
    float xmin = INFINITY, xmax = -INFINITY, ymin = INFINITY, ymax = -INFINITY, smin = INFINITY;
    bool finite = nvalid > 0;
    for (int u = 0; u < nvalid; ++u) {
        const float4 m = mir[u];
        finite &= isfinite(m.x) && isfinite(m.y);
        xmin = fminf(xmin, m.x);
        xmax = fmaxf(xmax, m.x);
        ymin = fminf(ymin, m.y);
        ymax = fmaxf(ymax, m.y);
        smin = fminf(smin, mirror_s(m));
    }
    if (!finite || !(smin > 0.0f)) return kSumOpen;
    return sum_lo(f, xmin) | (sum_hi(f, xmax) << 8) | (sum_lo(f, ymin) << 16) | (sum_hi(f, ymax) << 24);
}

__device__ __forceinline__ uint32_t point_box(const float4 &mv, const SumFrame &f) {
    if (!(isfinite(mv.x) && isfinite(mv.y)) || !(mirror_s(mv) > 0.0f)) return kSumOpen;
    return sum_lo(f, mv.x) | (sum_hi(f, mv.x) << 8) | (sum_lo(f, mv.y) << 16) | (sum_hi(f, mv.y) << 24);
}

typedef unsigned short u16x2 __attribute__((ext_vector_type(2)));
constexpr uint32_t kBoxHalf = 0x00ff00ffu;

__device__ __forceinline__ uint32_t pk_min_u16(uint32_t a, uint32_t b) {
    return __builtin_bit_cast(uint32_t, __builtin_elementwise_min(__builtin_bit_cast(u16x2, a),
                                                                  __builtin_bit_cast(u16x2, b)));
}
__device__ __forceinline__ uint32_t pk_max_u16(uint32_t a, uint32_t b) {
    return __builtin_bit_cast(uint32_t, __builtin_elementwise_max(__builtin_bit_cast(u16x2, a),
                                                                  __builtin_bit_cast(u16x2, b)));
}
__device__ __forceinline__ uint32_t box_union(uint32_t a, uint32_t b) {
    return pk_min_u16(a & kBoxHalf, b & kBoxHalf) | (pk_max_u16((a >> 8) & kBoxHalf, (b >> 8) & kBoxHalf) << 8);
}

template <int CTRL, int ROWS>
__device__ __forceinline__ void box_dpp_step(uint32_t &lo, uint32_t &hi) {
    lo = pk_min_u16(lo, (uint32_t)__builtin_amdgcn_update_dpp((int)kBoxHalf, (int)lo, CTRL, ROWS, 0xf, false));
    hi = pk_max_u16(hi, (uint32_t)__builtin_amdgcn_update_dpp(0, (int)hi, CTRL, ROWS, 0xf, false));
}

__device__ __forceinline__ uint32_t wave_box_union(uint32_t b) {
    uint32_t lo = b & kBoxHalf, hi = (b >> 8) & kBoxHalf;
    box_dpp_step<0x111, 0xf>(lo, hi);
    box_dpp_step<0x112, 0xf>(lo, hi);
    box_dpp_step<0x114, 0xf>(lo, hi);
    box_dpp_step<0x118, 0xf>(lo, hi);
    box_dpp_step<0x142, 0xa>(lo, hi);
    box_dpp_step<0x143, 0xc>(lo, hi);
    lo = (uint32_t)__builtin_amdgcn_readlane((int)lo, 63);
    hi = (uint32_t)__builtin_amdgcn_readlane((int)hi, 63);
    return lo | (hi << 8);
}

struct BoxLds {
    uint32_t lo[kBBoxRows], hi[kBBoxRows];
};
__device__ __forceinline__ void lds_box_set(BoxLds &s, int r, uint32_t b) {
    s.lo[r] = b & kBoxHalf;
    s.hi[r] = (b >> 8) & kBoxHalf;
}
__device__ __forceinline__ uint32_t lds_box_get(const BoxLds &s, int r) { return s.lo[r] | (s.hi[r] << 8); }
__device__ __forceinline__ void lds_box_merge(BoxLds &s, int r, uint32_t b) {
    const uint32_t blo = b & kBoxHalf, bhi = (b >> 8) & kBoxHalf;
    uint32_t lo = s.lo[r], hi = s.hi[r];
    for (uint32_t want = pk_min_u16(lo, blo); want != lo; want = pk_min_u16(lo, blo)) {
        const uint32_t prev = atomicCAS(&s.lo[r], lo, want);
        if (prev == lo) break;
        lo = prev;
    }
    for (uint32_t want = pk_max_u16(hi, bhi); want != hi; want = pk_max_u16(hi, bhi)) {
        const uint32_t prev = atomicCAS(&s.hi[r], hi, want);
        if (prev == hi) break;
        hi = prev;
    }
}

template <int MAXM>
__device__ __forceinline__ unsigned box_open_mask(uint32_t s, const uint32_t (&bc)[MAXM], int m) {
    const uint32_t xl = s & 0xffu, xh = (s >> 8) & 0xffu, yl = (s >> 16) & 0xffu, yh = s >> 24;
    unsigned om = 0u;
#pragma unroll
    for (int k = 0; k < MAXM; ++k)
        if (k < m && xl <= (bc[k] & 0xffu) && xh >= ((bc[k] >> 8) & 0xffu) && yl <= ((bc[k] >> 16) & 0xffu) &&
            yh >= (bc[k] >> 24))
            om |= 1u << k;
    return om;
}

__device__ __forceinline__ bool page_reject(uint32_t sum, const SumFrame &f, float slb, float fx, float fy,
                                            float fe, float gate2f) {
    const float xmin = sum_lo_val(f, sum & 0xffu), xmax = sum_hi_val(f, (sum >> 8) & 0xffu);
    const float ymin = sum_lo_val(f, (sum >> 16) & 0xffu), ymax = sum_hi_val(f, sum >> 24);
    const float Dx = fmaxf(fmaxf(xmin - fx, fx - xmax), 0.0f);
    const float Dy = fmaxf(fmaxf(ymin - fy, fy - ymax), 0.0f);
    const float Cx = fmaxf(fabsf(xmin), fabsf(xmax)) * 2.3841858e-7f;
    const float Cy = fmaxf(fabsf(ymin), fabsf(ymax)) * 2.3841858e-7f;
    const float lx = fmaxf(fmaf(Dx, 0.99999976f, -(fe + Cx)), 0.0f);
    const float ly = fmaxf(fmaf(Dy, 0.99999976f, -(fe + Cy)), 0.0f);
    return slb * fmaf(lx, lx, ly * ly) > gate2f;
}

struct Band {
    uint32_t cx, cy;
};

__device__ __forceinline__ Band band_none() { return Band{0xffu, 0xffu}; }

__device__ inline uint32_t band_codes(double f, double R, const SumFrame &fr) {
    const double cell = fr.cell, org = fr.org;
    if (!(isfinite(R) && isfinite(f) && cell > 0.0)) return 0xffu;
    const double ta = (f + R - org) / cell + 1.0 + 1e-6;
    const double tb = (f - R - org) / cell - 1e-6;
    const double A = fmin(fmax(ceil(ta), 1.0), 256.0);
    const double B = fmin(fmax(floor(tb), -1.0), 254.0);
    return (uint32_t)(A - 1.0) | ((uint32_t)(B + 1.0) << 8);
}

__device__ inline Band gate_band(float fx, float fy, float fe, float slb, float gate2f, const SumFrame &fr) {
    const double L = sqrt((double)gate2f / (double)slb);
    const double base = L * (1.0 + 1e-5) + (double)fe * (1.0 + 1e-5);
    const double Rx = (base + fabs((double)fx) * 1e-6) * (1.0 + 1e-5);
    const double Ry = (base + fabs((double)fy) * 1e-6) * (1.0 + 1e-5);
    Band b;
    b.cx = band_codes(fx, Rx, fr);
    b.cy = band_codes(fy, Ry, fr);
    return b;
}


__device__ __forceinline__ void lower_slb(float *slb, float s) {
    float v = (s > 0.0f) ? s : INFINITY;
    v = lane63(dpp_scan(v, INFINITY, [](float a, float b) { return fminf(a, b); }));
    if ((threadIdx.x & 63) == 0 && v < *slb) atomicMin(reinterpret_cast<unsigned *>(slb), __float_as_uint(v));
}

__device__ __forceinline__ unsigned ambiguous(double q, double gate2) {
    return fabs(q - gate2) <= 1e-9 * gate2 ? 1u : 0u;
}

}
```

### fast-slam_amd/csrc/fs2_resample.hip

```cpp
#include "fs2_chain.hpp"
#include "fs2_plan.hpp"

namespace fs2 {

constexpr int kScanPer = 4;
constexpr int kScanBlock = kBlock * kScanPer;


__global__ void k_global_total(const ReduceParams P) {
    double t = 0.0;
    for (int q = 0; q < P.world; ++q) {
        if (q == P.shard && P.est_base) *P.est_base = t;
        t = (q == 0) ? P.totals[P.rank_of[0]] : t + P.totals[P.rank_of[q]];
    }
    P.stats->total = t;
}

hipError_t launch_global_total(const ReduceParams &p, hipStream_t s) {
    hipLaunchKernelGGL(k_global_total, dim3(1), dim3(1), 0, s, p);
    return hipGetLastError();
}

__device__ double pairwise_sq(const double *a, int64_t n) {
    if (n < 8) {
// ... 971 lines not shown
    auto dest = [&](int64_t h) {
        const unsigned long long key = (h < c1) ? T.key[h] : 0ull;
        return key ? (int)((key >> 32) & 0xffu) - 1 : -1;
    };
    for (int64_t h = c0 + threadIdx.x; h < c0 + kAssignChunk; h += kBlock) {
        const int d = dest(h);
        uint32_t dummy = 0;
        wave_dest_add(s_cnt, d, dummy);
        if (d >= 0) {
            const uint32_t mask = T.cmask[h];
            if (mask) atomicAdd(&s_ccnt[d], (uint32_t)__popc(mask));
        }
    }
    __syncthreads();
    if (threadIdx.x < (unsigned)P.world) {
        unsigned long long *row = reinterpret_cast<unsigned long long *>(P.xrow + kXrowWords * threadIdx.x);
        if (s_cnt[threadIdx.x]) s_base[threadIdx.x] = (uint32_t)atomicAdd(row + 2, (unsigned long long)s_cnt[threadIdx.x]);
        if (s_ccnt[threadIdx.x])
            s_cbase[threadIdx.x] = (uint32_t)atomicAdd(row + 3, (unsigned long long)s_ccnt[threadIdx.x]);
    }
    __syncthreads();
    unsigned repeats = 0;
    for (int64_t h = c0 + threadIdx.x; h < c0 + kAssignChunk; h += kBlock) {
        const int d = dest(h);
        uint32_t local = 0;
        wave_dest_add(s_run, d, local);
        if (d >= 0) {
            const uint32_t u = s_base[d] + local;
            const uint32_t mask = T.cmask[h];
            T.uidx[h] = u;
            T.cbase[h] = mask ? s_cbase[d] + atomicAdd(&s_crun[d], (uint32_t)__popc(mask)) : 0u;
            T.ulist[T.ebase[d] + u] = (uint32_t)h;
            if (P.sent_mask) {
                const uint32_t page = (uint32_t)T.key[h] & kIdMask, bit = 1u << d;
                repeats += (atomicOr(&P.sent_mask[page], bit) & bit) ? 1u : 0u;
            }
        }
    }
    if (P.sent_mask) {
        __shared__ unsigned long long s_rep[kBlock / 64];
        const unsigned long long r = block_sum_u64<kBlock>(repeats, s_rep);
        if (threadIdx.x == 0 && r) atomicAdd(&P.stats->repeat_pages, r);
    }
}

hipError_t launch_pack_dedup(const ResampleParams &p, hipStream_t s) {
    const unsigned g = (unsigned)((p.xt.i_hi - p.xt.i_lo + kBlock - 1) / kBlock);
    if (p.xt.i_hi > p.xt.i_lo && p.map.rows > 0) {
        hipLaunchKernelGGL(k_dedup_insert, dim3(g, (unsigned)p.map.rows), dim3(kBlock), 0, s, p);
        hipLaunchKernelGGL(k_dedup_follow, dim3(g, (unsigned)p.map.rows), dim3(kBlock), 0, s, p);
    }
    hipLaunchKernelGGL(k_dedup_assign, dim3((unsigned)((p.xt.cap + kAssignChunk - 1) / kAssignChunk)), dim3(kBlock), 0,
                       s, p);
    return hipGetLastError();
}

__device__ __forceinline__ int dest_of(const int64_t *base, int world, int64_t e) {
    int p = 0;
    while (p + 1 < world && e >= base[p + 1]) ++p;
    return p;
}

__global__ __launch_bounds__(kBlock) void k_pack_index(const ResampleParams P, int64_t total) {
    const int64_t e = (int64_t)blockIdx.x * kBlock + threadIdx.x;
    if (e >= total) return;
    const XferTable &T = P.xt;
    const int p = dest_of(T.ebase, P.world, e);
    const uint32_t es = T.eslot[e];
    const uint32_t h = es & ~kEntryOwned;
    const bool own = (es & kEntryOwned) && T.ref[h] == 0u;
    reinterpret_cast<uint32_t *>(P.sbuf[p] + xfer_idx_off(P.plan[p].K))[e - T.ebase[p]] =
        T.uidx[h] | (own ? kEntryOwned : 0u);
}

__global__ __launch_bounds__(kBlock) void k_pack_pages(const ResampleParams P, int64_t total) {
    const int64_t t = (int64_t)blockIdx.x * kBlock + threadIdx.x;
    const int64_t g = t / kPageSlots;
    const int j = (int)(t % kPageSlots);
    if (g >= total) return;
    const XferTable &T = P.xt;
    const int p = dest_of(T.ubase, P.world, g);
    const int64_t u = g - T.ubase[p];
    const uint32_t h = T.ulist[T.ebase[p] + u];
    const unsigned long long key = T.key[h];
    const uint32_t page = (uint32_t)(key & 0xffffffffu);
    const int fill = (int)((key >> 40) & 0xfu);
    const uint32_t mask = T.cmask[h], cb = T.cbase[h];
    const PackPlan &pl = P.plan[p];
    XferPage *xp = reinterpret_cast<XferPage *>(P.sbuf[p] + xfer_page_off(pl.K, pl.S)) + u;
    if (j == 0) {
        xp->cbase = cb;
        xp->fill = (uint8_t)fill;
        xp->cmask = (uint8_t)mask;
        xp->pad0 = 0;
        xp->pad1 = 0;
    }
    uint16_t slot = 0;
    double2 xy = make_double2(0.0, 0.0);
    if (j < fill) {
        const float4 m = load_mirror(page_ptr(P.map.pool, page), j);
        const double2 *r = reinterpret_cast<const double2 *>(P.map.recs + (int64_t)mirror_rec(m) * kRecBytes);
        slot = (uint16_t)mirror_slot(m);
        xy = r[0];
        if ((mask >> j) & 1u) {
            double2 *cv = reinterpret_cast<double2 *>(P.sbuf[p] + xfer_cov_off(pl.K, pl.S, T.ubase[p + 1] - T.ubase[p])) +
                          2 * (int64_t)(cb + (uint32_t)__popc(mask & ((1u << j) - 1u)));
            cv[0] = r[1];
            cv[1] = r[2];
        }
    }
    xp->slot[j] = slot;
    xp->xy[j] = xy;
}

hipError_t launch_pack_write(const ResampleParams &p, hipStream_t s) {
    const unsigned g = (unsigned)((p.n + kBlock - 1) / kBlock);
    if (g) hipLaunchKernelGGL(k_pack_headers, dim3(g), dim3(kBlock), 0, s, p);
    const int64_t ne = p.xt.ebase[p.world], nu = p.xt.ubase[p.world];
    if (ne > 0) hipLaunchKernelGGL(k_pack_index, dim3((unsigned)((ne + kBlock - 1) / kBlock)), dim3(kBlock), 0, s, p, ne);
    if (nu > 0)
        hipLaunchKernelGGL(k_pack_pages, dim3((unsigned)((nu * kPageSlots + kBlock - 1) / kBlock)), dim3(kBlock), 0, s,
                           p, nu);
    return hipGetLastError();
}

__device__ __forceinline__ int peer_of(const ResampleParams &P, int k) {
    int p = 0;
    while (p + 1 < P.npeers && k >= P.peers[p + 1].kbase) ++p;
    return p;
}

__global__ __launch_bounds__(kBlock) void k_pack_refs(const ResampleParams P) {
    const int64_t i = P.xt.i_lo + (int64_t)blockIdx.x * kBlock + threadIdx.x;
    const int k = blockIdx.y;
    if (blockIdx.x == 0 && blockIdx.y == 0 && threadIdx.x < (unsigned)P.world) {
        const int p = threadIdx.x;
        if (p != P.keep && P.plan[p].K > 0) {
            RefPreamble pre{};
            pre.slb = *P.map.slb;
            pre.org = P.map.frame.org;
            pre.cell = P.map.frame.cell;
            pre.icell = P.map.frame.icell;
            pre.rank = P.rank;
            *reinterpret_cast<RefPreamble *>(P.sbuf[p]) = pre;
        }
    }
    if (i >= P.xt.i_hi || i >= P.n) return;
    const int c = P.cnt[i];
    if (k * kPageSlots >= c || P.mlo[i] > P.mhi[i]) return;
    const Desc e = *pt_entry(P.map, k, i);
    const uint32_t t = ref_tag(e);
    XDesc d;
    d.x = ((t ? t : (uint32_t)P.rank + 1u) << kRefShift) | ref_id(e);
    d.y = P.map.bbox ? P.map.bbox[(i / kBlock) * kBBoxRows + k] : kSumOpen;
    const int64_t c_i = P.iblk[P.nblk + i / kScanBlock] + P.rank_e[i];
    for (int p = 0; p < P.world; ++p) {
        const PackPlan &pl = P.plan[p];
        if (p == P.keep || i < pl.i0 || i >= pl.i1) continue;
        reinterpret_cast<XDesc *>(P.sbuf[p] + 64 + 64 * pl.K)[c_i - pl.c0 + k] = d;
    }
}

hipError_t launch_pack_refs(const ResampleParams &p, hipStream_t s) {
    const unsigned g = (unsigned)((p.n + kBlock - 1) / kBlock);
    if (g) {
        ResampleParams ph = p;
        for (int q = 0; q < p.world; ++q)
            if (ph.sbuf[q]) ph.sbuf[q] += 64;
        hipLaunchKernelGGL(k_pack_headers, dim3(g), dim3(kBlock), 0, s, ph);
    }
    const int64_t span = p.xt.i_hi - p.xt.i_lo;
    if (span > 0 && p.map.rows > 0)
        hipLaunchKernelGGL(k_pack_refs, dim3((unsigned)((span + kBlock - 1) / kBlock), (unsigned)p.map.rows),
                           dim3(kBlock), 0, s, p);
    else if (p.world > 0)
        hipLaunchKernelGGL(k_pack_refs, dim3(1, 1), dim3(kBlock), 0, s, p);
    return hipGetLastError();
}

__device__ __forceinline__ uint32_t recode_box(uint32_t b, const RefPreamble &pre, const SumFrame &f) {
    if (b == kSumOpen) return b;
    const SumFrame g{pre.org, pre.cell, pre.icell};
    if (g.org == f.org && g.cell == f.cell) return b;
    return sum_lo(f, sum_lo_val(g, b & 0xffu)) | (sum_hi(f, sum_hi_val(g, (b >> 8) & 0xffu)) << 8) |
           (sum_lo(f, sum_lo_val(g, (b >> 16) & 0xffu)) << 16) | (sum_hi(f, sum_hi_val(g, b >> 24)) << 24);
}

__global__ __launch_bounds__(kBlock) void k_unpack_refs(const ResampleParams P, int32_t nrecv) {
    const int r = blockIdx.x * (kBlock / 64) + (threadIdx.x >> 6);
    const int lane = threadIdx.x & 63;
    if (r >= nrecv) return;
    const int q = peer_of(P, r);
    const RecvPeer &pp = P.peers[q];
    const PackHeader &h = pp.hdr[r - pp.kbase];
    const RefPreamble pre = *pp.pre;
    const int rows = (h.cnt + kPageSlots - 1) / kPageSlots;
    for (int k = lane; k < rows; k += 64) {
        XDesc d = pp.refs[h.soff + k];
        if (ref_tag(d.x) == (uint32_t)P.rank + 1u) d.x = ref_id(d.x);
        d.y = recode_box(d.y, pre, P.map.frame);
        P.rdesc[(int64_t)r * P.map.rows + k] = d;
    }
    lower_slb(P.map.slb, pre.slb);
}



__global__ __launch_bounds__(kBlock) void k_scatter_recv(const ResampleParams P, int32_t nrecv) {
    if (!P.stats->resampled) return;
    const int k = blockIdx.x * kBlock + threadIdx.x;
    if (k >= nrecv) return;
    const int p = peer_of(P, k);
    const PackHeader &h = P.peers[p].hdr[k - P.peers[p].kbase];
    for (int64_t m = h.out_lo; m <= h.out_hi; ++m) P.out_src[m - P.ao] = -(k + 1);
}

__global__ __launch_bounds__(kBlock) void k_unpack_pages(const ResampleParams P, int64_t nu) {
    const int64_t t = (int64_t)blockIdx.x * kBlock + threadIdx.x;
    const int64_t g = min(t / kPageSlots, max(nu - 1, (int64_t)0));
    const int j = (int)(t % kPageSlots);
    const bool live = t / kPageSlots < nu;
    float smin = INFINITY;
    int q = 0;
    while (q + 1 < P.npeers && g >= P.peers[q + 1].ubase) ++q;
    const XferPage *xp = P.peers[q].pages + (g - P.peers[q].ubase);
    const int fill = xp->fill;
    const uint32_t mask = xp->cmask;
    const uint32_t id = P.alloc.freel[P.alloc.base + g];
    float bx0 = INFINITY, bx1 = -INFINITY, by0 = INFINITY, by1 = -INFINITY, bs = INFINITY;
    bool finite = true;
    if (live && j < fill) {
        const double2 xy = xp->xy[j];
        Slot sl{xy.x, xy.y, M2{P.init_cov[0], P.init_cov[1], P.init_cov[2], P.init_cov[3]}};
        if ((mask >> j) & 1u) {
            const double2 *cv = P.peers[q].covs + 2 * (int64_t)(xp->cbase + (uint32_t)__popc(mask & ((1u << j) - 1u)));
            const double2 b = cv[0], c = cv[1];
            sl.P = M2{b.x, b.y, c.x, c.y};
        }
        const uint32_t rid = P.alloc.rfreel[P.alloc.rbase + g * kPageSlots + j];
        store_rec(P.map.recs, rid, sl);
        float4 mv = with_slot(mirror_of(sl), xp->slot[j]);
        mv.w = __uint_as_float(rid);
        reinterpret_cast<float4 *>(page_ptr(P.map.pool, id))[j] = mv;
        const float s = mirror_s(mv);
        smin = s > 0.0f ? s : INFINITY;
        finite = isfinite(mv.x) && isfinite(mv.y);
        bx0 = fminf(INFINITY, mv.x);
        bx1 = fmaxf(-INFINITY, mv.x);
        by0 = fminf(INFINITY, mv.y);
        by1 = fmaxf(-INFINITY, mv.y);
        bs = fminf(INFINITY, s);
    }
#pragma unroll
    for (int o = 1; o < kPageSlots; o <<= 1) {
        bx0 = fminf(bx0, __shfl_xor(bx0, o, 64));
        bx1 = fmaxf(bx1, __shfl_xor(bx1, o, 64));
        by0 = fminf(by0, __shfl_xor(by0, o, 64));
        by1 = fmaxf(by1, __shfl_xor(by1, o, 64));
        bs = fminf(bs, __shfl_xor(bs, o, 64));
        finite = finite && (__shfl_xor((int)finite, o, 64) != 0);
    }
    if (live && j == 0) {
        XDesc d;
        d.x = id;
        if (!(finite && fill > 0) || !(bs > 0.0f))
            d.y = kSumOpen;
        else
            d.y = sum_lo(P.map.frame, bx0) | (sum_hi(P.map.frame, bx1) << 8) | (sum_lo(P.map.frame, by0) << 16) |
                  (sum_hi(P.map.frame, by1) << 24);
        P.udesc[g] = d;
    }
    lower_slb(P.map.slb, smin);
    if (blockIdx.x == 0 && threadIdx.x == 0) atomicAdd(&P.stats->new_pages, (unsigned long long)nu);
}

__global__ __launch_bounds__(kBlock) void k_unpack_rows(const ResampleParams P, int32_t nrecv) {
    const int r = blockIdx.x * (kBlock / 64) + (threadIdx.x >> 6);
    const int lane = threadIdx.x & 63;
    if (r >= nrecv) return;
    const int q = peer_of(P, r);
    const RecvPeer &pp = P.peers[q];
    const PackHeader &h = pp.hdr[r - pp.kbase];
    const int rows = (h.cnt + kPageSlots - 1) / kPageSlots;
    for (int k = lane; k < rows; k += 64) {
        const uint32_t ent = pp.idx[h.soff + k];
        XDesc d = P.udesc[pp.ubase + (ent & ~kEntryOwned)];
        d.x = (d.x & kIdMask) | ((ent & kEntryOwned) ? kOwned : 0u);
        P.rdesc[(int64_t)r * P.map.rows + k] = d;
    }
}

constexpr int kTileRows = 32;
__device__ void gather_rows(const ResampleParams &P, int64_t wg, int64_t nwg, unsigned long long *lds_u) {
    const int64_t n = P.n;
    const int64_t nblk = (n + kBlock - 1) / kBlock;
    const int64_t tiles = (int64_t)((P.map.rows + kTileRows - 1) / kTileRows) * nblk;
    unsigned nremote = 0;
    unsigned npages = 0;
    for (int64_t t = wg; t < tiles; t += nwg) {
        const int r0 = (int)(t / nblk) * kTileRows;
        const int64_t m = (t % nblk) * kBlock + threadIdx.x;
        const int32_t s = m < n ? P.out_src[m] : -1;
        if (s < 0) continue;
        const int rows = (P.cnt[s] + kPageSlots - 1) / kPageSlots;
        if (r0 >= rows) continue;
        const int64_t lo = max((int64_t)P.mlo[s], P.ao), hi = min((int64_t)P.mhi[s], P.ao + n - 1);
        const uint32_t keep = (P.refs ? P.mlo[s] == P.mhi[s] : hi == lo) ? 0xffffffffu : kIdMask;
        uint32_t e[kTileRows];
#pragma unroll
        for (int u = 0; u < kTileRows; ++u) e[u] = *pt_entry(P.map, min(r0 + u, rows - 1), s);
#pragma unroll
        for (int u = 0; u < kTileRows; ++u) {
            if (r0 + u < rows) {
                e[u] &= keep;
                if (P.refs && ref_tag(e[u])) {
                    ++nremote;
                    bool claimed = false;
                    if (P.tkey && ptable_insert(P.tkey, P.tcap, P.tepoch, e[u], &claimed) >= 0 && claimed)
                        ++npages;
                }
                __builtin_nontemporal_store(e[u], P.opt + (int64_t)(r0 + u) * n + m);
            }
        }
    }
    if (P.refs) {
        const unsigned long long br = block_sum_u64<kBlock>(nremote, lds_u);
        if (threadIdx.x == 0 && br) atomicAdd(&P.stats->remote_rows, br);
        __syncthreads();
        const unsigned long long bp = block_sum_u64<kBlock>(npages, lds_u);
        if (threadIdx.x == 0 && bp) atomicAdd(&P.stats->remote_pages, bp);
    }
}

static int64_t gather_row_groups(int64_t n, int rows) {
    const int64_t tiles = (int64_t)((rows + kTileRows - 1) / kTileRows) * ((n + kBlock - 1) / kBlock);
    return std::min<int64_t>(tiles, 2048);
}

__global__ __launch_bounds__(kBlock) void k_gather_particles(const ResampleParams P) {
    __shared__ double lds_d[kBlock / 64];
    __shared__ int64_t lds_l[kBlock / 64];
    __shared__ BoxLds s_bb;
    __shared__ int s_src[kBlock];
    __shared__ int s_sb[kBlock];
    __shared__ int s_wc[kBlock / 64];
    if (P.go ? *(volatile const unsigned long long *)P.go != P.go_seq : !P.stats->resampled) return;
    __shared__ unsigned long long lds_u[kBlock / 64];
    {
        const int64_t nblk = (P.n + kBlock - 1) / kBlock;
        if ((int64_t)blockIdx.x >= nblk) {
            gather_rows(P, (int64_t)blockIdx.x - nblk, (int64_t)gridDim.x - nblk, lds_u);
            return;
        }
    }
    const int64_t m = (int64_t)blockIdx.x * kBlock + threadIdx.x;
    if (m == 0 && P.runs_n) *P.runs_n = 0u;
    const bool bb = P.obbox != nullptr && P.map.bbox != nullptr;
    if (bb) lds_box_set(s_bb, threadIdx.x, kBoxEmpty);
    double bv = -INFINITY;
    int64_t bi = INT64_MAX;
    unsigned slots = 0;
    const int64_t n = P.n;
    int32_t s = 0;
    int rows = 0;
    const XDesc *rsrc = nullptr;
    if (m < n) {
        s = P.out_src[m];
        double w;
        int c;
        if (s >= 0) {
            P.ox[m] = P.x[s];
            P.oy[m] = P.y[s];
            P.oyaw[m] = P.yaw[s];
            w = P.w[s];
            c = P.cnt[s];
        } else {
            const int r = -s - 1;
            const int p = peer_of(P, r);
            const PackHeader &h = P.peers[p].hdr[r - P.peers[p].kbase];
            P.ox[m] = h.x;
            P.oy[m] = h.y;
            P.oyaw[m] = h.yaw;
            w = h.w;
            c = h.cnt;
            rsrc = P.rdesc + (int64_t)r * P.map.rows;
            rows = (c + kPageSlots - 1) / kPageSlots;
        }
        P.ocnt[m] = c;
        P.ow[m] = w;
        bv = w;
        bi = m;
        slots = (unsigned)c;
    }
    const bool recv = bb && __syncthreads_or(m < n && s < 0);
    if (bb) s_src[threadIdx.x] = (m < n && s >= 0) ? s / kBlock : -1;
    if (bb) __syncthreads();
    const int wrows = wave_max_i(rows);
    unsigned nremote = 0;
    unsigned npages = 0;
    for (int k0 = 0; k0 < wrows; k0 += 8) {
        uint32_t e[8], eb[8];
#pragma unroll
        for (int u = 0; u < 8; ++u) {
            e[u] = 0u;
            eb[u] = kBoxEmpty;
            if (rsrc) {
                const XDesc x = rsrc[max(min(k0 + u, rows - 1), 0)];
                e[u] = x.x;
                eb[u] = x.y;
            }
        }
#pragma unroll
        for (int u = 0; u < 8; ++u) {
            if (k0 + u < rows) {
                if (P.refs && ref_tag(e[u])) {
                    ++nremote;
                    bool claimed = false;
                    if (P.tkey && ptable_insert(P.tkey, P.tcap, P.tepoch, e[u], &claimed) >= 0 && claimed)
                        ++npages;
                }
                __builtin_nontemporal_store(e[u], P.opt + (int64_t)(k0 + u) * n + m);
            }
        }
        if (recv) {
#pragma unroll
            for (int u = 0; u < 8; ++u) {
                if (k0 + u < wrows) {
                    const uint32_t b = wave_box_union((k0 + u < rows && s < 0) ? eb[u] : kBoxEmpty);
                    if ((threadIdx.x & 63) == 0) lds_box_merge(s_bb, k0 + u, b);
                }
            }
        }
    }
    int nsb = 0;
    if (bb) {
        const int t = threadIdx.x;
        const bool first = s_src[t] >= 0 && (t == 0 || s_src[t - 1] != s_src[t]);
        const uint64_t fm = __ballot(first);
        const int wid = t >> 6, lane = t & 63;
        if (lane == 0) s_wc[wid] = __popcll(fm);
        __syncthreads();
        int off = 0;
#pragma unroll
        for (int w = 0; w < kBlock / 64; ++w) {
            off += (w < wid) ? s_wc[w] : 0;
            nsb += s_wc[w];
        }
        if (first) s_sb[off + __popcll(fm & ((1ull << lane) - 1ull))] = s_src[t];
    }
    if (P.refs) {
        const unsigned long long br = block_sum_u64<kBlock>(nremote, lds_u);
        if (threadIdx.x == 0 && br) atomicAdd(&P.stats->remote_rows, br);
        __syncthreads();
        const unsigned long long bp = block_sum_u64<kBlock>(npages, lds_u);
        if (threadIdx.x == 0 && bp) atomicAdd(&P.stats->remote_pages, bp);
        __syncthreads();
    }
    const unsigned long long bs = block_sum_u64<kBlock>(slots, lds_u);
    block_argmax<kBlock>(bv, bi, lds_d, lds_l);
    if (threadIdx.x == 0) {
        P.part_best_w[blockIdx.x] = bv;
        P.part_best_i[blockIdx.x] = bi;
        P.part_slots[blockIdx.x] = bs;
    }
    if (bb && (int)threadIdx.x < P.map.rows) {
        uint32_t b = lds_box_get(s_bb, threadIdx.x);
        for (int q = 0; q < nsb; ++q) b = box_union(b, P.map.bbox[(int64_t)s_sb[q] * kBBoxRows + threadIdx.x]);
        P.obbox[(int64_t)blockIdx.x * kBBoxRows + threadIdx.x] = b;
    }
}

__global__ __launch_bounds__(kBlock) void k_bbox_build(const MapRef map, const int32_t *cnt, int64_t n) {
    __shared__ BoxLds s_bb;
    const int64_t i = (int64_t)blockIdx.x * kBlock + threadIdx.x;
    lds_box_set(s_bb, threadIdx.x, kBoxEmpty);
    const int c = (i < n) ? cnt[i] : 0;
    const int rows = (c + kPageSlots - 1) / kPageSlots;
    __syncthreads();
    const int wrows = wave_max_i(rows);
    for (int r = 0; r < wrows; ++r) {
        uint32_t b = kBoxEmpty;
        if (r < rows) {
            const float4 *mir = reinterpret_cast<const float4 *>(page_ptr_any(map, *pt_entry(map, r, i)));
            b = page_box(mir, min(kPageSlots, c - r * kPageSlots), map.frame);
        }
        b = wave_box_union(b);
        if ((threadIdx.x & 63) == 0) lds_box_merge(s_bb, r, b);
    }
    __syncthreads();
    if ((int)threadIdx.x < map.rows) map.bbox[(int64_t)blockIdx.x * kBBoxRows + threadIdx.x] = lds_box_get(s_bb, threadIdx.x);
}

hipError_t launch_bbox_build(MapRef map, const int32_t *cnt, hipStream_t s) {
    if (!map.bbox) return hipSuccess;
    const unsigned g = (unsigned)((map.n + kBlock - 1) / kBlock);
    hipLaunchKernelGGL(k_bbox_build, dim3(g), dim3(kBlock), 0, s, map, cnt, map.n);
    return hipGetLastError();
}

__device__ void estimate_body(const ResampleParams &P, int32_t nparts) {
    __shared__ double lds_d[16];
    __shared__ int64_t lds_l[16];
    __shared__ unsigned long long lds_u[16];
    double bv = -INFINITY;
    int64_t bi = INT64_MAX;
    unsigned long long sl = 0;
    for (int k = threadIdx.x; k < nparts; k += 1024) {
        argmax_combine(bv, bi, P.part_best_w[k], P.part_best_i[k]);
        sl += P.part_slots[k];
    }
    block_argmax<1024>(bv, bi, lds_d, lds_l);
    sl = block_sum_u64<1024>(sl, lds_u);
    if (threadIdx.x == 0) {
        P.stats->resample_slots = sl;
        RankRecord r = *P.rec;
        r.best_w = bv;
        const int64_t bo = (P.est_early && bi != INT64_MAX) ? (bi >> 32) : bi;
        r.best_gidx = (bo == INT64_MAX) ? INT64_MAX : P.ao + bo;
        if (bo != INT64_MAX) {
            if (P.est_early) {
                const int32_t s = (int32_t)(bi & 0xffffffffll);
                r.pose[0] = P.x[s];
                r.pose[1] = P.y[s];
                r.pose[2] = P.yaw[s];
            } else {
                r.pose[0] = P.ox[bo];
                r.pose[1] = P.oy[bo];
                r.pose[2] = P.oyaw[bo];
            }
        }
        *P.rec = r;
    }
}

__global__ __launch_bounds__(1024) void k_estimate(const ResampleParams P, int32_t nparts) {
    if (P.stats->resampled) estimate_body(P, nparts);
}

__global__ __launch_bounds__(1024) void k_tail_single(const ResampleParams R, const ReduceParams P, int32_t nparts,
                                                     DevStats *host_stats, unsigned long long *host_flag,
                                                     unsigned long long seq) {
    if (!R.stats->resampled) return;
    if (blockIdx.x > 0) {
        fill_runs_body(R, blockIdx.x - 1, gridDim.x - 1);
        return;
    }
    estimate_body(R, nparts);
    __syncthreads();
    if (threadIdx.x == 0) {
        global_best_body(P);
        if (R.gen) *R.gen += 1u;
        if (R.go) *R.go = R.go_seq;
    }
    __syncthreads();
    publish_body(P.stats, host_stats, host_flag, seq);
}

hipError_t launch_tail_single(const ResampleParams &r, const ReduceParams &p, DevStats *host_stats,
                              unsigned long long *host_flag, unsigned long long seq, hipStream_t s,
                              hipEvent_t e1) {
    const int32_t nparts = (int32_t)((r.n + kBlock - 1) / kBlock);
    const unsigned fill = ((r.ranges_mode & 2) && r.runs) ? kTailFill : 0u;
    FS2_LAUNCH_EV(k_tail_single, dim3(1 + fill), dim3(1024), s, nullptr, e1, r, p, nparts, host_stats, host_flag, seq);
    return hipGetLastError();
}

hipError_t launch_resample_apply(const ResampleParams &p, bool estimate, hipStream_t s) {
    const unsigned g = (unsigned)((p.n + kBlock - 1) / kBlock);
    if (g == 0) return hipSuccess;
    int32_t nrecv = 0;
    int64_t nu = 0;
    for (int q = 0; q < p.npeers; ++q) {
        nrecv += p.peers[q].K;
        nu += p.peers[q].U;
    }
    if (nrecv > 0) {
        hipLaunchKernelGGL(k_scatter_recv, dim3((nrecv + kBlock - 1) / kBlock), dim3(kBlock), 0, s, p, nrecv);
        if (p.refs) {
            hipLaunchKernelGGL(k_unpack_refs, dim3((nrecv + kBlock / 64 - 1) / (kBlock / 64)), dim3(kBlock), 0, s, p,
                               nrecv);
        } else {
            if (nu > 0)
                hipLaunchKernelGGL(k_unpack_pages, dim3((unsigned)((nu * kPageSlots + kBlock - 1) / kBlock)),
                                   dim3(kBlock), 0, s, p, nu);
            hipLaunchKernelGGL(k_unpack_rows, dim3((nrecv + kBlock / 64 - 1) / (kBlock / 64)), dim3(kBlock), 0, s, p,
                               nrecv);
        }
    }
    hipLaunchKernelGGL(k_gather_particles, dim3(g + (unsigned)gather_row_groups(p.n, p.map.rows)), dim3(kBlock), 0,
                       s, p);
    if (estimate) hipLaunchKernelGGL(k_estimate, dim3(1), dim3(1024), 0, s, p, (int32_t)g);
    return hipGetLastError();
}

}
```

### fast-slam_amd/csrc/fs2_update.hip

```cpp
#include "fs2_chain.hpp"

namespace fs2 {

#ifdef FS2_PHASE_TIMING
__device__ unsigned long long g_phase[8];
#define FS2_PHASE(k)                                                                         \
    do {                                                                                     \
        const unsigned long long t_ = __builtin_amdgcn_s_memtime();                           \
        if ((threadIdx.x & 63) == 0 && (k) > 0) atomicAdd(&g_phase[(k) - 1], t_ - ph_last);   \
        ph_last = t_;                                                                        \
    } while (0)
#else
#define FS2_PHASE(k) do { } while (0)
#endif

constexpr int kDescAhead = 2;
constexpr int kCopyBatch = 8;

static_assert(kMaxCand == 8, "sort8 sorts the candidate list");

__device__ __forceinline__ uint64_t cand_entry(int slot, int pos, uint32_t rec) {
    return ((uint64_t)slot << 44) | ((uint64_t)pos << 32) | (uint64_t)rec;
}
__device__ __forceinline__ int cand_slot(uint64_t e) { return (int)(e >> 44); }
__device__ __forceinline__ int cand_pos(uint64_t e) { return (int)((e >> 32) & 0xfffu); }
__device__ __forceinline__ uint32_t cand_rec(uint64_t e) { return (uint32_t)e; }

__device__ __forceinline__ void cmpx(uint64_t &a, uint64_t &b) {
    const uint64_t lo = a < b ? a : b, hi = a < b ? b : a;
    a = lo;
    b = hi;
}
__device__ __forceinline__ void sort8(uint64_t (&e)[8]) {
    cmpx(e[0], e[1]); cmpx(e[2], e[3]); cmpx(e[4], e[5]); cmpx(e[6], e[7]);
    cmpx(e[0], e[2]); cmpx(e[1], e[3]); cmpx(e[4], e[6]); cmpx(e[5], e[7]);
    cmpx(e[1], e[2]); cmpx(e[5], e[6]);
    cmpx(e[0], e[4]); cmpx(e[1], e[5]); cmpx(e[2], e[6]); cmpx(e[3], e[7]);
    cmpx(e[2], e[4]); cmpx(e[3], e[5]);
    cmpx(e[1], e[2]); cmpx(e[3], e[4]); cmpx(e[5], e[6]);
}

__device__ __forceinline__ void move_particle(const UpdateParams &P, int64_t i, double &px, double &py,
                                              double &pyaw) {
    const double nz = P.noise ? P.noise[i] : P.sigma * philox_normal(P.seed, P.scan, (uint64_t)(P.gidx0 + i));
    double ntr, nrot;
    if (P.rotation != 0.0) {
        ntr = 0.0;
        nrot = P.rotation + nz;
    } else {
        ntr = P.translation + nz;
        nrot = 0.0;
    }
    pyaw = pymod(pyaw + nrot + kPi, kTwoPi) - kPi;
    px += ntr * cos(pyaw);
    py += ntr * sin(pyaw);
}

template <int MAXM>
__global__ __launch_bounds__(kBlock) void k_candidates(const UpdateParams P) {
    if (P.stats->error_flags & 8) return;
    __shared__ uint64_t s_list[kMaxCand][kBlock];
    __shared__ Band s_band[MAXM];
    __shared__ uint16_t s_rows[kBBoxRows];
    __shared__ uint8_t s_rmask[kBBoxRows];
    __shared__ int s_wc[kBlock / 64];
    const int tid = threadIdx.x;
    const int64_t n = P.n;
    const int64_t blk = P.blk0 + blockIdx.x;
    const int64_t i = blk * kBlock + tid;
    const bool live = i < n;
    MapRef map = P.map;
    const int32_t *cntp = P.cnt;
    double *xp = P.x, *yp = P.y, *yawp = P.yaw;
    if (P.gen) {
        const BufSet &b = P.sets[__builtin_amdgcn_readfirstlane(*(volatile const uint32_t *)P.gen) & 1u];
        map.pt = b.pt;
        map.bbox = b.bbox;
        cntp = b.cnt;
        xp = b.x;
        yp = b.y;
        yawp = b.yaw;
    }
    const int c = live ? cntp[i] : 0;
    if (P.move_cand && live) {
        double px = xp[i], py = yp[i], pyaw = yawp[i];
        move_particle(P, i, px, py, pyaw);
        xp[i] = px;
        yp[i] = py;
        yawp[i] = pyaw;
    }
    const Desc *ptrow = map.pt + (live ? i : 0);
    const float slb = *map.slb;
    if (blockIdx.x == 0 && tid == 0 && P.slb_pass) *P.slb_pass = slb;
    const int rlast = map.rows - 1;
    if (tid < MAXM) {
        Band b = band_none();
#pragma unroll
        for (int k = 0; k < MAXM; ++k)
            if (tid == k && k < P.m)
                b = gate_band(P.meas.fx[k], P.meas.fy[k], P.meas.fe[k], slb, P.gate2f, map.frame);
        s_band[tid] = b;
    }
    __syncthreads();
    uint32_t bc[MAXM];
#pragma unroll
    for (int k = 0; k < MAXM; ++k) {
        bc[k] = __builtin_amdgcn_readfirstlane(s_band[k].cx | (s_band[k].cy << 16));
    }
    int nc = 0;
    unsigned visited = 0, groups = 0, opened = 0;

    const unsigned all_m = (1u << P.m) - 1u;
    auto test_page = [&](const float4 *mir, int g, unsigned om) {
        const int j0 = g * kPageSlots;
#pragma unroll
        for (int u = 0; u < kScanGroup; ++u) {
            if (j0 + u < c) {
                ++visited;
                const float4 mv = mir[u];
                const float cx = fabsf(mv.x) * 2.3841858e-7f;
                const float cy = fabsf(mv.y) * 2.3841858e-7f;
                bool hit = false;
#pragma unroll
                for (int k = 0; k < MAXM; ++k) {
                    if ((om >> k) & 1u) {
                        hit |= !gate_reject_fast(mv, cx, cy, P.meas.fx[k], P.meas.fy[k], P.meas.fe[k],
                                                 P.gate2f);
                    }
                }
                if (hit) {
                    const uint64_t e = cand_entry(mirror_slot(mv), j0 + u, mirror_rec(mv));
                    if (nc < kMaxCand) {
                        s_list[nc][tid] = e;
                    } else {
                        int mq = 0;
                        uint64_t me = s_list[0][tid];
#pragma unroll 1
                        for (int q = 1; q < kMaxCand; ++q) {
                            const uint64_t x = s_list[q][tid];
                            if (x > me) {
                                me = x;
                                mq = q;
                            }
                        }
                        if (e < me) s_list[mq][tid] = e;
                    }
                    ++nc;
                }
            }
        }
    };
    const bool use_bb = map.bbox != nullptr;
    int nrows = map.rows;
    if (use_bb) {
        unsigned rm = 0u;
        if (tid < map.rows) rm = box_open_mask<MAXM>(map.bbox[blk * kBBoxRows + tid], bc, P.m);
        const bool pass = rm != 0u;
        const uint64_t bm = __ballot(pass);
        const int wid = tid >> 6, lane = tid & 63;
        if (lane == 0) s_wc[wid] = __popcll(bm);
        __syncthreads();
        int off = 0;
        nrows = 0;
#pragma unroll
        for (int w = 0; w < kBlock / 64; ++w) {
            off += (w < wid) ? s_wc[w] : 0;
            nrows += s_wc[w];
        }
        if (pass) {
            const int at = off + __popcll(bm & ((1ull << lane) - 1ull));
            s_rows[at] = (uint16_t)tid;
            s_rmask[at] = (uint8_t)rm;
        }
        __syncthreads();
    }
    auto row_at = [&](int q) -> int { return use_bb ? (q < nrows ? (int)s_rows[q] : 0) : min(q, rlast); };
    Desc dq[kDescAhead];
#pragma unroll
    for (int q = 0; q < kDescAhead; ++q) dq[q] = ptrow[(int64_t)row_at(q) * n];
    for (int q = 0; q < nrows; ++q) {
        const int g = row_at(q);
        if (!__any(g * kPageSlots < c)) break;
        const Desc d = dq[0];
#pragma unroll
        for (int u = 0; u + 1 < kDescAhead; ++u) dq[u] = dq[u + 1];
        dq[kDescAhead - 1] = ptrow[(int64_t)row_at(q + kDescAhead) * n];
        if (g * kPageSlots < c) ++groups;
        const unsigned om = (g * kPageSlots < c) ? (use_bb ? (unsigned)s_rmask[q] : all_m) : 0u;
        if (!__any(om)) continue;
        const char *pg = page_ptr(map.pool, om ? d : 0u);
        float4 mir[kScanGroup];
#pragma unroll
        for (int u = 0; u < kScanGroup; ++u) mir[u] = load_mirror(pg, u);
        if (om) {
            ++opened;
            test_page(mir, g, om);
        }
    }
    if (live) {
        P.ncand[i] = nc;
        uint64_t e[kMaxCand];
#pragma unroll
        for (int q = 0; q < kMaxCand; ++q) e[q] = (q < nc) ? s_list[q][tid] : ~0ull;
        sort8(e);
#pragma unroll
        for (int q = 0; q < kMaxCand; ++q)
            if (q < nc) P.cand[(int64_t)q * n + i] = e[q];
    }
    const unsigned cv[4] = {(unsigned)min(nc, kMaxCand), groups, visited, opened};
    block_counters<kBlock, kCWords, 4>(cv, P.cpart, P.nblk, blk, P.k0 == 0 ? 0xffffffffu : 0u, 0.0, nullptr);
}

template <int K>
static __device__ __forceinline__ uint32_t sel_u32(int t, const uint32_t (&a)[K]) {
    uint32_t v = 0;
#pragma unroll
    for (int q = 0; q < K; ++q)
        if (t == q) v = a[q];
    return v;
}

template <int MAXM>
__global__ __launch_bounds__(kBlock) void k_update(const UpdateParams P) {
    if (P.stats->error_flags & 8) return;
    __shared__ Meas s_ms[MAXM];
    __shared__ double s_lik[MAXM][kBlock];
    __shared__ int16_t s_idx[MAXM][kBlock];
    union WaveScratch {
        uint2 cow[64 * (MAXM + 1)];
        struct {
            int best[MAXM][64], bpos[MAXM][64];
        } ov;
    };
    __shared__ WaveScratch s_ws[kBlock / 64];
    __shared__ float4 s_mv[MAXM][kBlock];
    __shared__ BoxLds s_bb;

#ifdef FS2_PHASE_TIMING
    unsigned long long ph_last = 0;
#endif
    const int tid = threadIdx.x;
    const int64_t blk = P.blk0 + blockIdx.x;
    const int64_t i = blk * kBlock + tid;
    const bool live = i < P.n;
    const int64_t n = P.n;
    if (tid < MAXM) s_ms[tid] = Meas{P.meas.d[tid], P.meas.b[tid], P.meas.ox[tid], P.meas.oy[tid]};
#pragma unroll
    for (int k = 0; k < MAXM; ++k) s_idx[k][tid] = (int16_t)-2;
    MapRef map = P.map;
    double *xp = P.x, *yp = P.y, *yawp = P.yaw, *wp = P.w;
    int32_t *cntp = P.cnt;
    if (P.gen) {
        const BufSet &b = P.sets[__builtin_amdgcn_readfirstlane(*(volatile const uint32_t *)P.gen) & 1u];
        xp = b.x;
        yp = b.y;
        yawp = b.yaw;
        wp = b.w;
        cntp = b.cnt;
        map.pt = b.pt;
        map.bbox = b.bbox;
    }
    if (map.bbox && tid < map.rows) lds_box_set(s_bb, tid, map.bbox[blk * kBBoxRows + tid]);
    __syncthreads();

    double px = 0.0, py = 0.0, pyaw = 0.0, w = 0.0;
    int c = 0;
    if (live) {
        px = xp[i];
        py = yp[i];
        pyaw = yawp[i];
        w = wp[i];
        c = cntp[i];
    }
    const int64_t il = live ? i : 0;
    int nalloc = 0;
    int nrec = 0;
    unsigned cow = 0, fresh = 0;
    float smin_w = INFINITY;
    uint64_t mods = 0;
    int nmod = 0;
    uint32_t frec[MAXM];
#pragma unroll
    for (int t = 0; t < MAXM; ++t) {
        frec[t] = (live && t < P.m) ? P.alloc.rfreel[P.alloc.rbase + (int64_t)t * n + i] : 0u;
    }
    FS2_PHASE(0);
#ifdef FS2_AB_NO_MOVE
    if (false) {
#else
    if (live && P.do_move && !P.move_cand) {
#endif
        move_particle(P, i, px, py, pyaw);
    }

    const M2 R{P.R[0], P.R[1], P.R[2], P.R[3]};
    auto box_note = [&](int row, uint32_t b) {
        if (map.bbox) lds_box_merge(s_bb, row, b);
    };
    unsigned pend = live ? ((1u << P.m) - 1u) : 0u;
    unsigned visited = 0, candidates = 0, written = 0, amb = 0, appends = 0;
    bool singular = false;
    const double gate2 = P.gate2;

    FS2_PHASE(1);
    int ncl = 0;
    bool overflow = false;
    if (live && P.filter) {
        const int nc = P.ncand[i];
        ncl = min(nc, kMaxCand);
        overflow = nc > kMaxCand;
    }

    auto visit = [&](int slot, int pos, Slot s) {
        ++candidates;
        bool mod = false;
        M2 I;
        bool ok = inv2(s.P, I);
        singular |= !ok;
        unsigned todo = ok ? pend : 0u;
        while (todo) {
            int km = -1;
#pragma unroll
            for (int k = 0; k < MAXM; ++k) {
                if (km < 0 && ((todo >> k) & 1u)) {
                    const double qd = quad(I, s_ms[k].ox - s.mx, s_ms[k].oy - s.my);
                    amb += ambiguous(qd, gate2);
                    todo &= ~(1u << k);
                    if (qd >= 0.0 && qd < gate2) km = k;
                }
            }
            if (km < 0) break;
            s_lik[km][tid] = ekf_update(s, px, py, pyaw, s_ms[km], R, singular);
            s_idx[km][tid] = (int16_t)slot;
            pend &= ~(1u << km);
            mod = true;
            ok = inv2(s.P, I);
            singular |= !ok;
            if (!ok) todo = 0u;
        }
        if (mod) {
            const uint32_t r = sel_u32(nmod, frec);
            store_rec(map.recs, r, s);
            float4 m = with_slot(mirror_of(s), slot);
            m.w = __uint_as_float(r);
            smin_w = fminf(smin_w, mirror_s(m) > 0.0f ? mirror_s(m) : INFINITY);
            s_mv[nmod][tid] = m;
            mods |= (uint64_t)pos << (16 * nmod);
            ++nmod;
            ++written;
        }
    };

    int lo = -1;
    int nmod_list = 0;
    {
        const int nl = (pend != 0u) ? ncl : 0;
        auto entry = [&](int p) -> uint64_t { return P.cand[(int64_t)(p < nl ? p : 0) * n + il]; };
        auto rec_of = [&](int p, uint64_t e) -> uint32_t { return p < nl ? cand_rec(e) : 0u; };
        uint64_t e0 = entry(0), e1 = entry(1);
        Slot s0 = load_rec(map.recs, rec_of(0, e0));
        for (int p = 0; p < nl && pend != 0u; ++p) {
            const uint64_t e2 = entry(p + 2);
            const Slot s1 = load_rec(map.recs, rec_of(p + 1, e1));
            visit(cand_slot(e0), cand_pos(e0), s0);
            e0 = e1;
            s0 = s1;
            e1 = e2;
        }
        if (!P.filter) {
            for (int j = 0; j < c && pend != 0u; ++j) {
                const float4 mv = load_mirror(page_of(map, j, il), j);
                ++visited;
                visit(mirror_slot(mv), j, load_rec(map.recs, mirror_rec(mv)));
            }
        }
        if (overflow && ncl > 0) lo = cand_slot(P.cand[(int64_t)(ncl - 1) * n + il]);
        nmod_list = nmod;
    }
    if (overflow && pend != 0u) {
        const int rows = (c + kPageSlots - 1) / kPageSlots;
        const float slb = P.slb_pass ? *P.slb_pass : *map.slb;
#pragma unroll
        for (int k = 0; k < MAXM; ++k) {
            s_ws[tid >> 6].ov.best[k][tid & 63] = INT_MAX;
            s_ws[tid >> 6].ov.bpos[k][tid & 63] = -1;
        }
        int sing = INT_MAX;
        auto scan = [&](unsigned want, bool skip_mods) {
            for (int g = 0; g < rows; ++g) {
                const Desc d = *pt_entry(map, g, il);
                const uint32_t rb = map.bbox ? lds_box_get(s_bb, g) : kSumOpen;
                unsigned open = 0u;
#pragma unroll
                for (int k = 0; k < MAXM; ++k)
                    if (((want >> k) & 1u) &&
                        !page_reject(rb, map.frame, slb, P.meas.fx[k], P.meas.fy[k], P.meas.fe[k], P.gate2f))
                        open |= 1u << k;
                if (!open) continue;
                const char *pg = page_ptr(map.pool, d);
                for (int u = 0; u < kPageSlots && g * kPageSlots + u < c; ++u) {
                    const int pos = g * kPageSlots + u;
                    if (skip_mods) {
                        bool modded = false;
#pragma unroll
                        for (int q = 0; q < MAXM; ++q)
                            modded |= q < nmod && (int)((mods >> (16 * q)) & 0xffffu) == pos;
                        if (modded) continue;
                    }
                    const float4 mv = load_mirror(pg, u);
                    const int slot = mirror_slot(mv);
                    if (slot <= lo) continue;
                    const float cx = fabsf(mv.x) * 2.3841858e-7f, cy = fabsf(mv.y) * 2.3841858e-7f;
                    unsigned test = 0u;
#pragma unroll
                    for (int k = 0; k < MAXM; ++k)
                        if (((open >> k) & 1u) && slot < s_ws[tid >> 6].ov.best[k][tid & 63] &&
                            !gate_reject_fast(mv, cx, cy, P.meas.fx[k], P.meas.fy[k], P.meas.fe[k], P.gate2f))
                            test |= 1u << k;
                    if (!test && !(mirror_s(mv) == 0.0f && slot < sing)) continue;
                    const Slot s = load_rec(map.recs, mirror_rec(mv));
                    ++candidates;
                    M2 I;
                    if (!inv2(s.P, I)) {
                        sing = min(sing, slot);
                        continue;
                    }
#pragma unroll
                    for (int k = 0; k < MAXM; ++k) {
                        if ((test >> k) & 1u) {
                            const double qd = quad(I, s_ms[k].ox - s.mx, s_ms[k].oy - s.my);
                            amb += ambiguous(qd, gate2);
                            if (qd >= 0.0 && qd < gate2) {
                                s_ws[tid >> 6].ov.best[k][tid & 63] = slot;
                                s_ws[tid >> 6].ov.bpos[k][tid & 63] = pos;
                            }
                        }
                    }
                }
            }
        };
        scan(pend, false);
        for (int k = 0; k < MAXM; ++k) {
            if (!((pend >> k) & 1u)) continue;
            int t = -1;
            const int pb = s_ws[tid >> 6].ov.bpos[k][tid & 63];
#pragma unroll
            for (int q = 0; q < MAXM; ++q)
                if (q < nmod && pb >= 0 && (int)((mods >> (16 * q)) & 0xffffu) == pb) t = q;
            if (t >= 0) {
                s_ws[tid >> 6].ov.best[k][tid & 63] = INT_MAX;
                s_ws[tid >> 6].ov.bpos[k][tid & 63] = -1;
                scan(1u << k, true);
            }
            int bk = s_ws[tid >> 6].ov.best[k][tid & 63], pk = s_ws[tid >> 6].ov.bpos[k][tid & 63];
            int tk = -1;
            for (int q = nmod_list; q < nmod; ++q) {
                const int pos = (int)((mods >> (16 * q)) & 0xffffu);
                const float4 mq = s_mv[q][tid];
                const int slot = mirror_slot(mq);
                if (slot >= bk) continue;
                const Slot s = load_rec(map.recs, sel_u32(q, frec));
                ++candidates;
                M2 I;
                if (!inv2(s.P, I)) {
                    sing = min(sing, slot);
                    continue;
                }
                const double qd = quad(I, s_ms[k].ox - s.mx, s_ms[k].oy - s.my);
                amb += ambiguous(qd, gate2);
                if (qd >= 0.0 && qd < gate2) {
                    bk = slot;
                    pk = pos;
                    tk = q;
                }
            }
            if (sing < bk) singular = true;
            if (pk < 0) continue;
            int t2 = tk;
            if (t2 < 0) {
#pragma unroll
                for (int q = 0; q < MAXM; ++q)
                    if (q < nmod && (int)((mods >> (16 * q)) & 0xffffu) == pk) t2 = q;
            }
            Slot s = load_rec(map.recs, t2 >= 0 ? sel_u32(t2, frec)
                                                : mirror_rec(load_mirror(page_of(map, pk, il), pk)));
            s_lik[k][tid] = ekf_update(s, px, py, pyaw, s_ms[k], R, singular);
            s_idx[k][tid] = (int16_t)bk;
            pend &= ~(1u << k);
            if (t2 < 0) {
                t2 = nmod++;
                mods |= (uint64_t)pk << (16 * t2);
                ++written;
            }
            const uint32_t r = sel_u32(t2, frec);
            store_rec(map.recs, r, s);
            float4 m = with_slot(mirror_of(s), bk);
            m.w = __uint_as_float(r);
            smin_w = fminf(smin_w, mirror_s(m) > 0.0f ? mirror_s(m) : INFINITY);
#pragma unroll
            for (int q = 0; q < MAXM; ++q)
                if (q == t2) s_mv[q][tid] = m;
        }
    }

    FS2_PHASE(2);

    constexpr int NR = MAXM + 1;
    const int nrows = nmod + ((pend != 0u && c % kPageSlots != 0) ? 1 : 0);
    int rrow[NR];
    Desc rdesc[NR];
    int canon[NR];
    unsigned cowm = 0u;
#pragma unroll
    for (int t = 0; t < NR; ++t) {
        rrow[t] = (t < nmod) ? (int)((mods >> (16 * t)) & 0xffffu) / kPageSlots
                             : (t == nmod && t < nrows ? c / kPageSlots : 0);
        rdesc[t] = *pt_entry(map, rrow[t], il);
    }
    uint32_t fpage[MAXM];
#pragma unroll
    for (int t = 0; t < MAXM; ++t)
        fpage[t] = t < P.m ? P.alloc.freel[P.alloc.base + (int64_t)t * n + il] : 0u;

    {
        const int lane = tid & 63, wid = tid >> 6;
        int T = 0;
#pragma unroll
        for (int t = 0; t < NR; ++t) {
            bool task = false;
            uint32_t src = 0, dst = 0;
            canon[t] = t;
#pragma unroll
            for (int u = 0; u < t; ++u)
                if (canon[t] == t && u < nrows && rrow[u] == rrow[t]) canon[t] = u;
            if (t < nrows && canon[t] == t && !(rdesc[t] & kOwned)) {
                task = true;
                src = rdesc[t] & kIdMask;
                dst = sel_u32(nalloc, fpage);
                ++nalloc;
                rdesc[t] = dst | kOwned;
                cowm |= 1u << t;
                ++cow;
            }
            const uint64_t bm = __ballot(task);
            if (task) s_ws[wid].cow[T + __popcll(bm & ((1ull << lane) - 1ull))] = make_uint2(src, dst);
            T += __popcll(bm);
        }
        __builtin_amdgcn_fence(__ATOMIC_RELEASE, "workgroup");
        __builtin_amdgcn_wave_barrier();
        __builtin_amdgcn_fence(__ATOMIC_ACQUIRE, "workgroup");
        const int off = (lane & 7) * 16;
        constexpr int CB = kCopyBatch;
        v4i va[CB];
        uint32_t da[CB];
        auto load_batch = [&](int base, v4i *v, uint32_t *d) {
#pragma unroll
            for (int u = 0; u < CB; ++u) {
                const uint2 tk = s_ws[wid].cow[min(base + 8 * u + (lane >> 3), T - 1)];
                d[u] = tk.y;
                v[u] = *reinterpret_cast<const v4i *>(page_ptr(map.pool, tk.x) + off);
            }
        };
        auto store_batch = [&](const v4i *v, const uint32_t *d) {
#pragma unroll
            for (int u = 0; u < CB; ++u) {
                *reinterpret_cast<v4i *>(page_ptr(map.pool, d[u]) + off) = v[u];
            }
        };
        for (int base = 0; base < T; base += 8 * CB) {
            load_batch(base, va, da);
            store_batch(va, da);
        }
        __threadfence_block();
    }

    FS2_PHASE(3);
    {
#pragma unroll
        for (int t = 0; t < MAXM; ++t) {
            if (t < nmod) {
                const int j = (int)((mods >> (16 * t)) & 0xffffu);
                uint32_t id = 0;
#pragma unroll
                for (int u = 0; u < NR; ++u)
                    if (u == canon[t]) id = rdesc[u];
                const float4 m = s_mv[t][tid];
                reinterpret_cast<float4 *>(page_ptr(map.pool, id))[j & (kPageSlots - 1)] = m;
                box_note(rrow[t], point_box(m, map.frame));
            }
        }
        nrec = nmod;
#pragma unroll
        for (int t = 0; t < MAXM; ++t)
            if (t < nmod && canon[t] == t && ((cowm >> t) & 1u)) *pt_entry(map, rrow[t], il) = rdesc[t];
    }

    FS2_PHASE(4);
    int nap = 0;
    int arow = -1;
    Desc ad = 0u;
    bool ad_new = false;
    if (pend != 0u && c % kPageSlots != 0) {
        arow = c / kPageSlots;
#pragma unroll
        for (int u = 0; u < NR; ++u)
            if (u == canon[nmod]) {
                ad = rdesc[u];
                ad_new = (cowm >> u) & 1u;
            }
    }
    auto page_at = [&](int j) -> char * {
        return (j / kPageSlots == arow) ? page_ptr(map.pool, ad) : page_of(map, j, il);
    };
    while (pend) {
        const int k = __builtin_ctz(pend);
        pend &= pend - 1u;
        const Meas mk = s_ms[k];
        int hit = -1;
        for (int a = 0; a < nap; ++a) {
            const Slot s = load_slot(map, page_at(c + a), c + a);
            ++candidates;
            M2 I;
            if (!inv2(s.P, I)) {
                singular = true;
                break;
            }
            const double q = quad(I, mk.ox - s.mx, mk.oy - s.my);
            amb += ambiguous(q, gate2);
            if (q >= 0.0 && q < gate2) {
                hit = a;
                break;
            }
        }
        if (hit >= 0) {
            const int jh = c + hit;
            char *pg = page_at(jh);
            const uint32_t r = mirror_rec(load_mirror(pg, jh));
            Slot s = load_rec(map.recs, r);
            s_lik[k][tid] = ekf_update(s, px, py, pyaw, mk, R, singular);
            const float4 mv = store_slot(map, pg, jh, s, r, jh);
            smin_w = fminf(smin_w, mirror_s(mv) > 0.0f ? mirror_s(mv) : INFINITY);
            box_note(jh / kPageSlots, point_box(mv, map.frame));
            s_idx[k][tid] = (int16_t)(c + hit);
        } else {
            const Slot s{px + mk.d * cos(pyaw + mk.b), py + mk.d * sin(pyaw + mk.b),
                         M2{P.init_cov[0], P.init_cov[1], P.init_cov[2], P.init_cov[3]}};
            const int ja = c + nap;
            const uint32_t r = sel_u32(nrec, frec);
            ++nrec;
            if (ja % kPageSlots == 0) {
                if (arow >= 0 && ad_new) *pt_entry(map, arow, il) = ad;
                const uint32_t id = take_page(P.alloc, map.n, il, nalloc);
                arow = ja / kPageSlots;
                const float4 mv = store_slot(map, page_ptr(map.pool, id), ja, s, r, ja);
                smin_w = fminf(smin_w, mirror_s(mv) > 0.0f ? mirror_s(mv) : INFINITY);
                box_note(arow, point_box(mv, map.frame));
                ad = id | kOwned;
                ad_new = true;
                ++fresh;
            } else {
                const float4 mv = store_slot(map, page_ptr(map.pool, ad), ja, s, r, ja);
                smin_w = fminf(smin_w, mirror_s(mv) > 0.0f ? mirror_s(mv) : INFINITY);
                box_note(arow, point_box(mv, map.frame));
            }
            s_idx[k][tid] = (int16_t)-1;
            ++nap;
            ++appends;
        }
        ++written;
    }
    if (arow >= 0 && ad_new) *pt_entry(map, arow, il) = ad;
    c += nap;

    FS2_PHASE(5);
    unsigned hits = 0, refv = 0, napp = 0;
#pragma unroll
    for (int k = 0; k < MAXM; ++k) {
        const int ix = s_idx[k][tid];
        if (ix >= 0) {
            w *= s_lik[k][tid];
            ++hits;
            refv += (unsigned)ix + 1u;
        } else if (ix == -1) {
            refv += (unsigned)(c - nap + napp);
            ++napp;
        }
        if (live && P.assoc && k < P.m) P.assoc[(int64_t)(P.k0 + k) * n + i] = ix;
    }

    if (live) {
        if (P.do_move && !P.move_cand) {
            xp[i] = px;
            yp[i] = py;
            yawp[i] = pyaw;
        }
        wp[i] = w;
        cntp[i] = c;
    }

    FS2_PHASE(6);
    const unsigned cv[kNumCounters] = {0u, 0u, visited, 0u, candidates, written, amb, appends, hits, cow, fresh,
                                       refv, singular ? 1u : 0u};
    const unsigned assign =
        P.k0 != 0 ? 0u
                  : (P.filter ? ~((1u << kCWords) | (1u << kCGroups) | (1u << kCVisited) | (1u << kCOpened))
                              : 0xffffffffu);
    block_counters<kBlock, 0, kNumCounters>(cv, P.cpart, P.nblk, blk, assign, live ? w : 0.0,
                                            P.last_pass ? P.wpart + blk : nullptr);
    if (map.bbox && tid < map.rows) map.bbox[blk * kBBoxRows + tid] = lds_box_get(s_bb, tid);
    lower_slb(map.slb, smin_w);
}

hipError_t launch_candidates(const UpdateParams &p, hipStream_t s, hipEvent_t e0, hipEvent_t e1) {
    const unsigned grid = (unsigned)(p.blk1 - p.blk0);
    if (grid == 0 || !p.filter) return hipSuccess;
    FS2_LAUNCH_EV(k_candidates<kMaxM>, dim3(grid), dim3(kBlock), s, e0, e1, p);
    return hipGetLastError();
}

hipError_t launch_update(const UpdateParams &p, hipStream_t s, hipEvent_t e0, hipEvent_t e1) {
    const unsigned grid = (unsigned)(p.blk1 - p.blk0);
    if (grid == 0) return hipSuccess;
    FS2_LAUNCH_EV(k_update<kMaxM>, dim3(grid), dim3(kBlock), s, e0, e1, p);
    return hipGetLastError();
}

template <int MAXM, int PHASE>
__global__ __launch_bounds__(kBlock) void k_localize(const LocalizeParams P) {
    __shared__ Band s_band[MAXM];
    __shared__ uint16_t s_rows[kBBoxRows];
    __shared__ int s_wc[kBlock / 64];
    __shared__ unsigned long long s_base;
    const int tid = threadIdx.x;
    const int64_t blk = blockIdx.x;
    const int64_t i = blk * kBlock + tid;
    const bool live = i < P.n;
    const MapRef map = P.map;
    const int c = live ? P.cnt[i] : 0;
    if (tid < MAXM) {
        Band b = band_none();
#pragma unroll
        for (int k = 0; k < MAXM; ++k)
            if (tid == k && k < P.m) b = gate_band(P.meas.fx[k], P.meas.fy[k], P.meas.fe[k], *map.slb, P.gate2f, map.frame);
        s_band[tid] = b;
    }
    __syncthreads();
    uint32_t bc[MAXM];
#pragma unroll
    for (int k = 0; k < MAXM; ++k) bc[k] = __builtin_amdgcn_readfirstlane(s_band[k].cx | (s_band[k].cy << 16));
    const bool use_bb = map.bbox != nullptr;
    int nrows = map.rows;
    if (use_bb) {
        bool pass = false;
        if (tid < map.rows) pass = box_open_mask<MAXM>(map.bbox[blk * kBBoxRows + tid], bc, P.m) != 0u;
        const uint64_t bm = __ballot(pass);
        const int wid = tid >> 6, lane = tid & 63;
        if (lane == 0) s_wc[wid] = __popcll(bm);
        __syncthreads();
        int off = 0;
        nrows = 0;
#pragma unroll
        for (int w = 0; w < kBlock / 64; ++w) {
            off += (w < wid) ? s_wc[w] : 0;
            nrows += s_wc[w];
        }
        if (pass) s_rows[off + __popcll(bm & ((1ull << lane) - 1ull))] = (uint16_t)tid;
        __syncthreads();
    }
    const int arow = (c % kPageSlots) ? c / kPageSlots : -1;
    auto row_at = [&](int q) -> int { return use_bb ? (int)s_rows[q] : q; };
    auto wanted = [&](int r, const Desc &d) -> bool { return r * kPageSlots < c && ref_tag(d) != 0u; };
    auto for_wanted = [&](auto &&fn) {
        if (!live) return;
        bool arow_seen = false;
        for (int q = 0; q < nrows; ++q) {
            const int r = row_at(q);
            if (r * kPageSlots >= c) continue;
            const Desc d = *pt_entry(map, r, i);
            if (wanted(r, d)) {
                fn(r, d);
                arow_seen |= r == arow;
            }
        }
        if (arow >= 0 && !arow_seen) {
            const Desc d = *pt_entry(map, arow, i);
            if (ref_tag(d) != 0u) fn(arow, d);
        }
    };
    const unsigned long long ep = (unsigned long long)P.epoch << 32;
    const uint64_t mask = (uint64_t)P.cap - 1u;
    auto slot0 = [&](uint32_t x) -> uint64_t { return ((uint64_t)x * 0x9E3779B97F4A7C15ull >> 20) & mask; };
    if (PHASE == 1) {
        unsigned long long rows = 0;
        for_wanted([&](int r, const Desc &d) {
            const unsigned long long want = ep | d;
            uint64_t s = slot0(d);
            for (int64_t probe = 0; probe < P.cap; ++probe, s = (s + 1) & mask)
                if (P.key[s] == want) {
                    const uint32_t id = P.val[s];
                    if (!(id & 0x80000000u)) {
                        *pt_entry(map, r, i) = id;
                        ++rows;
                    }
                    break;
                }
        });
        unsigned long long tot = rows;
#pragma unroll
        for (int o = 32; o > 0; o >>= 1) tot += __shfl_xor(tot, o, 64);
        if ((tid & 63) == 0 && tot) atomicAdd(&P.stats->loc_rows, tot);
        return;
    }
    const uint32_t marker = 0x80000000u | (uint32_t)i;
    auto find = [&](uint32_t x, bool claim) -> int64_t {
        const unsigned long long want = ep | x;
        uint64_t s = slot0(x);
        for (int64_t probe = 0; probe < P.cap;) {
            const unsigned long long cur = __atomic_load_n(&P.key[s], __ATOMIC_RELAXED);
            if (cur == want) return (int64_t)s;
            if (claim && (cur >> 32) != P.epoch) {
                if (atomicCAS(&P.key[s], cur, want) == cur) {
                    P.val[s] = marker;
                    return -2 - (int64_t)s;
                }
                continue;
            }
            s = (s + 1) & mask;
            ++probe;
        }
        return -1;
    };
    int need = 0;
    for_wanted([&](int, const Desc &d) {
        if (find(d, true) <= -2) ++need;
    });
    const int wid = tid >> 6, lane = tid & 63;
    int incl = need;
#pragma unroll
    for (int o = 1; o < 64; o <<= 1) {
        const int v = __shfl_up(incl, o, 64);
        if (lane >= o) incl += v;
    }
    __syncthreads();
    if (lane == 63) s_wc[wid] = incl;
    __syncthreads();
    int woff = 0, tot = 0;
#pragma unroll
    for (int w = 0; w < kBlock / 64; ++w) {
        woff += (w < wid) ? s_wc[w] : 0;
        tot += s_wc[w];
    }
    if (tid == 0) {
        s_base = tot ? atomicAdd(&P.stats->loc_pages, (unsigned long long)tot) : 0ull;
        if (tot) atomicAdd(&P.stats->loc_recs, (unsigned long long)tot * kPageSlots);
        if (tot && ((int64_t)(s_base + tot) > P.pcap || (int64_t)(s_base + tot) * kPageSlots > P.rcap)) {
            atomicOr(&P.stats->error_flags, 8);
            s_base = ~0ull;
        }
    }
    __syncthreads();
    if (!need) return;
    const bool failed = s_base == ~0ull;
    int64_t k = (int64_t)s_base + woff + incl - need;
    for_wanted([&](int r, const Desc &d) {
        const int64_t slot = find(d, false);
        if (slot < 0 || P.val[slot] != marker) return;
        if (failed) {
            P.val[slot] = 0xffffffffu;
            return;
        }
        const uint32_t tg = ref_tag(d);
        const float4 *src = reinterpret_cast<const float4 *>(map.peers->pool[tg - 1] + (int64_t)ref_id(d) * kPageBytes);
        const char *srecs = map.peers->recs[tg - 1];
        const uint32_t id = P.freel[P.ftail - 1 - k];
        const int valid = min(kPageSlots, c - r * kPageSlots);
        float4 mv[kPageSlots];
#pragma unroll
        for (int u = 0; u < kPageSlots; ++u) mv[u] = src[u];
        Slot sl[kPageSlots];
#pragma unroll
        for (int u = 0; u < kPageSlots; ++u) sl[u] = load_rec(srecs, u < valid ? mirror_rec(mv[u]) : mirror_rec(mv[0]));
        float4 *dst = reinterpret_cast<float4 *>(page_ptr(map.pool, id));
#pragma unroll
        for (int u = 0; u < kPageSlots; ++u) {
            if (u < valid) {
                const uint32_t rid = P.rfreel[P.rtail - 1 - (kPageSlots * k + u)];
                double2 *q = reinterpret_cast<double2 *>(map.recs + (int64_t)rid * kRecBytes);
                q[0] = make_double2(sl[u].mx, sl[u].my);
                q[1] = make_double2(sl[u].P.a00, sl[u].P.a01);
                q[2] = make_double2(sl[u].P.a10, sl[u].P.a11);
                mv[u].w = __uint_as_float(rid);
            } else {
                mv[u] = make_float4(0.0f, 0.0f, 0.0f, 0.0f);
            }
            dst[u] = mv[u];
        }
        P.val[slot] = id;
        ++k;
    });
}

hipError_t launch_localize(const LocalizeParams &p, hipStream_t s) {
    if (p.nblk <= 0) return hipSuccess;
    hipLaunchKernelGGL((k_localize<kMaxM, 0>), dim3((unsigned)p.nblk), dim3(kBlock), 0, s, p);
    hipLaunchKernelGGL((k_localize<kMaxM, 1>), dim3((unsigned)p.nblk), dim3(kBlock), 0, s, p);
    return hipGetLastError();
}
// ... 403 lines not shown
```

Before: 463.6 million.

## Replace packed 8-bit row bounding boxes with float half-page boxes

Per-row landmark bounding boxes move from a quantized 32-bit code to two float4 boxes per row, one for each half page. Gate tests run on exact float bounds and half-page granularity, so more pages and half-pages can be rejected and fewer slots scanned. In k_update, box updates are deferred and merged with a wave-level DPP union, and the overflow scan uses a precomputed per-row open mask. The cost is eight times more box memory traffic, heavier LDS atomics and larger shared memory, which may reduce occupancy.

After: 394.8 million. 0.851x the previous value.

```diff
diff --git a/fast-slam_amd/csrc/fs2_api.hip b/fast-slam_amd/csrc/fs2_api.hip
--- a/fast-slam_amd/csrc/fs2_api.hip
+++ b/fast-slam_amd/csrc/fs2_api.hip
@@ -366,7 +366,7 @@
     Pool pages{"page", kPageBytes, (int64_t)kIdMask};
     Pool records{"record", kRecBytes, (int64_t)kRecIdLimit};
     Desc *pt[2] = {};
-    uint32_t *bbox[2] = {};
+    float4 *bbox[2] = {};
     XDesc *rdesc = nullptr;
     XDesc *udesc = nullptr;
     size_t udesc_cap = 0;
@@ -549,7 +549,7 @@
         return MapRef{pages.data, pt[cur], std::max<int64_t>(n, 1), rows, records.data, frame, slb, row_boxes(cur),
                       refs_shared ? peers_dev : nullptr};
     }
-    uint32_t *row_boxes(int b) const { return rows <= kBBoxRows ? bbox[b] : nullptr; }
+    float4 *row_boxes(int b) const { return rows <= kBBoxRows ? bbox[b] : nullptr; }
     int64_t nblocks() const { return (n + kBlock - 1) / kBlock; }
     int reduce() const {
         const int mode = cfg.reduce_mode;
@@ -1563,7 +1563,7 @@
         ok &= FS2_ALLOC(h->yaw[s], n * 8) == hipSuccess;
         ok &= FS2_ALLOC(h->w[s], n * 8) == hipSuccess;
         ok &= FS2_ALLOC(h->cnt[s], n * 4) == hipSuccess;
-        ok &= FS2_ALLOC(h->bbox[s], nb * kBBoxRows * 4) == hipSuccess;
+        ok &= FS2_ALLOC(h->bbox[s], nb * kBBoxRows * 2 * sizeof(float4)) == hipSuccess;
     }
     ok &= FS2_ALLOC(h->pages.nfree_dev, sizeof(int64_t)) == hipSuccess;
     ok &= FS2_ALLOC(h->records.nfree_dev, sizeof(int64_t)) == hipSuccess;
@@ -1665,7 +1665,7 @@
             hipMemsetAsync(h->y[s], 0, n * 8, h->stream) != hipSuccess ||
             hipMemsetAsync(h->yaw[s], 0, n * 8, h->stream) != hipSuccess ||
             hipMemsetAsync(h->cnt[s], 0, n * 4, h->stream) != hipSuccess ||
-            hipMemsetD32Async((hipDeviceptr_t)h->bbox[s], (int)kBoxEmpty, nb * kBBoxRows, h->stream) != hipSuccess ||
+            launch_bbox_clear(h->bbox[s], (int64_t)nb * kBBoxRows * 2, h->stream) != hipSuccess ||
             launch_fill(h->w[s], 1.0 / (double)h->n_global, n, h->stream) != hipSuccess)
             return fail(set_err(&h->err, FS2_ERR_HIP, "state initialisation failed"));
     }
@@ -1823,14 +1823,15 @@
     HIP_TRY(h, hipEventElapsedTime(&t, E[0], E[3]));
     const uint64_t n = (uint64_t)h->n, nblk = (uint64_t)h->nblocks();
     const uint64_t box_rows = h->row_boxes(h->cur) ? (uint64_t)h->rows : 0ull;
+    const uint64_t box_b = 2ull * sizeof(float4);
     const bool filt = h->cfg.gate_filter != 0;
     const uint64_t cand_bytes = filt ? sizeof(Desc) * st.groups + 128ull * st.opened + 8ull * st.words +
-                                           8ull * n * p.passes + 4ull * box_rows * nblk
+                                           8ull * n * p.passes + box_b * box_rows * nblk
                                      : 0ull;
     const uint64_t upd_fixed = p.fixed_bytes + (filt ? 4ull * n * p.passes : 0ull) + 8ull * n * (uint64_t)p.m;
     const uint64_t exact_bytes = upd_fixed + (filt ? 8ull * st.words : 0ull) + 48ull * st.candidates +
                                  (64ull + sizeof(Desc)) * st.written + (2ull * kPageBytes + sizeof(Desc)) * st.cow_pages +
-                                 8ull * box_rows * nblk;
+                                 2ull * box_b * box_rows * nblk;
     if (filt && p.m <= kMaxM) {
         HIP_TRY(h, hipEventElapsedTime(&f, E[0], E[1]));
         HIP_TRY(h, hipEventElapsedTime(&x, E[4], E[2]));
@@ -1846,7 +1847,7 @@
         h->prof.model_written += st.written;
         h->prof.model_cow += st.cow_pages;
         h->prof.model_fixed_bytes += upd_fixed;
-        h->prof.model_box_bytes += 12ull * box_rows * nblk;
+        h->prof.model_box_bytes += 3ull * box_b * box_rows * nblk;
     }
     h->prof.scans += 1;
     h->prof.update_launches += p.passes;
diff --git a/fast-slam_amd/csrc/fs2_kernels.hpp b/fast-slam_amd/csrc/fs2_kernels.hpp
--- a/fast-slam_amd/csrc/fs2_kernels.hpp
+++ b/fast-slam_amd/csrc/fs2_kernels.hpp
@@ -249,7 +249,7 @@
     char *recs;
     SumFrame frame;
     float *slb;
-    uint32_t *bbox;
+    float4 *bbox;
     const PeerMaps *peers;
 };
 
@@ -264,7 +264,7 @@
     double *x, *y, *yaw, *w;
     int32_t *cnt;
     Desc *pt;
-    uint32_t *bbox;
+    float4 *bbox;
 };
 
 struct UpdateParams {
@@ -386,7 +386,7 @@
     int32_t *ocnt;
     MapRef map;
     Desc *opt;
-    uint32_t *obbox;
+    float4 *obbox;
     XDesc *rdesc;
     XDesc *udesc;
     PageAlloc alloc;
@@ -535,6 +535,7 @@
                          int32_t rows_each, int32_t *cnt, uint32_t *ext, const int32_t *perm,
                          int32_t perm_len, hipStream_t s);
 hipError_t launch_bbox_build(MapRef map, const int32_t *cnt, hipStream_t s);
+hipError_t launch_bbox_clear(float4 *bbox, int64_t nboxes, hipStream_t s);
 hipError_t launch_export(double *stage, int64_t first, int64_t count, int32_t lm_cap,
                          MapRef map, const int32_t *cnt, hipStream_t s);
 hipError_t launch_fill(double *p, double v, int64_t n, hipStream_t s);
diff --git a/fast-slam_amd/csrc/fs2_reduce.hpp b/fast-slam_amd/csrc/fs2_reduce.hpp
--- a/fast-slam_amd/csrc/fs2_reduce.hpp
+++ b/fast-slam_amd/csrc/fs2_reduce.hpp
@@ -395,27 +395,6 @@
     return c == 255u ? INFINITY : __double2float_ru(sum_grid(f, (double)c));
 }
 
-__device__ __forceinline__ uint32_t page_box(const float4 *mir, int nvalid, const SumFrame &f) {
-    float xmin = INFINITY, xmax = -INFINITY, ymin = INFINITY, ymax = -INFINITY, smin = INFINITY;
-    bool finite = nvalid > 0;
-    for (int u = 0; u < nvalid; ++u) {
-        const float4 m = mir[u];
-        finite &= isfinite(m.x) && isfinite(m.y);
-        xmin = fminf(xmin, m.x);
-        xmax = fmaxf(xmax, m.x);
-        ymin = fminf(ymin, m.y);
-        ymax = fmaxf(ymax, m.y);
-        smin = fminf(smin, mirror_s(m));
-    }
-    if (!finite || !(smin > 0.0f)) return kSumOpen;
-    return sum_lo(f, xmin) | (sum_hi(f, xmax) << 8) | (sum_lo(f, ymin) << 16) | (sum_hi(f, ymax) << 24);
-}
-
-__device__ __forceinline__ uint32_t point_box(const float4 &mv, const SumFrame &f) {
-    if (!(isfinite(mv.x) && isfinite(mv.y)) || !(mirror_s(mv) > 0.0f)) return kSumOpen;
-    return sum_lo(f, mv.x) | (sum_hi(f, mv.x) << 8) | (sum_lo(f, mv.y) << 16) | (sum_hi(f, mv.y) << 24);
-}
-
 typedef unsigned short u16x2 __attribute__((ext_vector_type(2)));
 constexpr uint32_t kBoxHalf = 0x00ff00ffu;
 
@@ -427,10 +406,6 @@
     return __builtin_bit_cast(uint32_t, __builtin_elementwise_max(__builtin_bit_cast(u16x2, a),
                                                                   __builtin_bit_cast(u16x2, b)));
 }
-__device__ __forceinline__ uint32_t box_union(uint32_t a, uint32_t b) {
-    return pk_min_u16(a & kBoxHalf, b & kBoxHalf) | (pk_max_u16((a >> 8) & kBoxHalf, (b >> 8) & kBoxHalf) << 8);
-}
-
 template <int CTRL, int ROWS>
 __device__ __forceinline__ void box_dpp_step(uint32_t &lo, uint32_t &hi) {
     lo = pk_min_u16(lo, (uint32_t)__builtin_amdgcn_update_dpp((int)kBoxHalf, (int)lo, CTRL, ROWS, 0xf, false));
@@ -450,81 +425,98 @@
     return lo | (hi << 8);
 }
 
+__device__ __forceinline__ float4 hbox_empty() { return make_float4(INFINITY, INFINITY, -INFINITY, -INFINITY); }
+__device__ __forceinline__ float4 hbox_open() { return make_float4(-INFINITY, -INFINITY, INFINITY, INFINITY); }
+__device__ __forceinline__ float4 hbox_union(const float4 &a, const float4 &b) {
+    return make_float4(fminf(a.x, b.x), fminf(a.y, b.y), fmaxf(a.z, b.z), fmaxf(a.w, b.w));
+}
+__device__ __forceinline__ int box_half(int pos) { return (pos & (kPageSlots - 1)) >> 2; }
+__device__ __forceinline__ float4 hbox_point(const float4 &mv) {
+    if (!(isfinite(mv.x) && isfinite(mv.y)) || !(mirror_s(mv) > 0.0f)) return hbox_open();
+    return make_float4(mv.x, mv.y, mv.x, mv.y);
+}
+__device__ __forceinline__ void page_hboxes(const float4 *mir, int nvalid, float4 (&hb)[2]) {
+    hb[0] = hbox_empty();
+    hb[1] = hbox_empty();
+    float4 m[kPageSlots];
+#pragma unroll
+    for (int u = 0; u < kPageSlots; ++u) m[u] = mir[u];
+#pragma unroll
+    for (int u = 0; u < kPageSlots; ++u)
+        if (u < nvalid) hb[u >> 2] = hbox_union(hb[u >> 2], hbox_point(m[u]));
+}
+__device__ __forceinline__ float4 wave_hbox_union(const float4 &b) {
+    auto mn = [](float a, float c) { return fminf(a, c); };
+    auto mx = [](float a, float c) { return fmaxf(a, c); };
+    return make_float4(lane63(dpp_scan(b.x, INFINITY, mn)), lane63(dpp_scan(b.y, INFINITY, mn)),
+                       lane63(dpp_scan(b.z, -INFINITY, mx)), lane63(dpp_scan(b.w, -INFINITY, mx)));
+}
+__device__ __forceinline__ uint32_t hbox_codes(const float4 &b, const SumFrame &f) {
+    return sum_lo(f, b.x) | (sum_hi(f, b.z) << 8) | (sum_lo(f, b.y) << 16) | (sum_hi(f, b.w) << 24);
+}
+__device__ __forceinline__ float4 hbox_of_codes(uint32_t c, const SumFrame &f) {
+    if (c == kBoxEmpty) return hbox_empty();
+    return make_float4(sum_lo_val(f, c & 0xffu), sum_lo_val(f, (c >> 16) & 0xffu), sum_hi_val(f, (c >> 8) & 0xffu),
+                       sum_hi_val(f, c >> 24));
+}
+
 struct BoxLds {
-    uint32_t lo[kBBoxRows], hi[kBBoxRows];
+    float4 b[kBBoxRows][2];
 };
-__device__ __forceinline__ void lds_box_set(BoxLds &s, int r, uint32_t b) {
-    s.lo[r] = b & kBoxHalf;
-    s.hi[r] = (b >> 8) & kBoxHalf;
-}
-__device__ __forceinline__ uint32_t lds_box_get(const BoxLds &s, int r) { return s.lo[r] | (s.hi[r] << 8); }
-__device__ __forceinline__ void lds_box_merge(BoxLds &s, int r, uint32_t b) {
-    const uint32_t blo = b & kBoxHalf, bhi = (b >> 8) & kBoxHalf;
-    uint32_t lo = s.lo[r], hi = s.hi[r];
-    for (uint32_t want = pk_min_u16(lo, blo); want != lo; want = pk_min_u16(lo, blo)) {
-        const uint32_t prev = atomicCAS(&s.lo[r], lo, want);
-        if (prev == lo) break;
-        lo = prev;
-    }
-    for (uint32_t want = pk_max_u16(hi, bhi); want != hi; want = pk_max_u16(hi, bhi)) {
-        const uint32_t prev = atomicCAS(&s.hi[r], hi, want);
-        if (prev == hi) break;
-        hi = prev;
-    }
-}
-
-template <int MAXM>
-__device__ __forceinline__ unsigned box_open_mask(uint32_t s, const uint32_t (&bc)[MAXM], int m) {
-    const uint32_t xl = s & 0xffu, xh = (s >> 8) & 0xffu, yl = (s >> 16) & 0xffu, yh = s >> 24;
-    unsigned om = 0u;
-#pragma unroll
-    for (int k = 0; k < MAXM; ++k)
-        if (k < m && xl <= (bc[k] & 0xffu) && xh >= ((bc[k] >> 8) & 0xffu) && yl <= ((bc[k] >> 16) & 0xffu) &&
-            yh >= (bc[k] >> 24))
-            om |= 1u << k;
-    return om;
-}
-
-__device__ __forceinline__ bool page_reject(uint32_t sum, const SumFrame &f, float slb, float fx, float fy,
-                                            float fe, float gate2f) {
-    const float xmin = sum_lo_val(f, sum & 0xffu), xmax = sum_hi_val(f, (sum >> 8) & 0xffu);
-    const float ymin = sum_lo_val(f, (sum >> 16) & 0xffu), ymax = sum_hi_val(f, sum >> 24);
-    const float Dx = fmaxf(fmaxf(xmin - fx, fx - xmax), 0.0f);
-    const float Dy = fmaxf(fmaxf(ymin - fy, fy - ymax), 0.0f);
-    const float Cx = fmaxf(fabsf(xmin), fabsf(xmax)) * 2.3841858e-7f;
-    const float Cy = fmaxf(fabsf(ymin), fabsf(ymax)) * 2.3841858e-7f;
+__device__ __forceinline__ void lds_fmin(float *a, float v) {
+    uint32_t *ua = reinterpret_cast<uint32_t *>(a);
+    uint32_t cur = *ua;
+    while (v < __uint_as_float(cur)) {
+        const uint32_t prev = atomicCAS(ua, cur, __float_as_uint(v));
+        if (prev == cur) break;
+        cur = prev;
+    }
+}
+__device__ __forceinline__ void lds_fmax(float *a, float v) {
+    uint32_t *ua = reinterpret_cast<uint32_t *>(a);
+    uint32_t cur = *ua;
+    while (v > __uint_as_float(cur)) {
+        const uint32_t prev = atomicCAS(ua, cur, __float_as_uint(v));
+        if (prev == cur) break;
+        cur = prev;
+    }
+}
+__device__ __forceinline__ void lds_box_merge(BoxLds &s, int r, int h, const float4 &p) {
+    float4 &q = s.b[r][h];
+    const float4 cur = q;
+    if (p.x < cur.x) lds_fmin(&q.x, p.x);
+    if (p.y < cur.y) lds_fmin(&q.y, p.y);
+    if (p.z > cur.z) lds_fmax(&q.z, p.z);
+    if (p.w > cur.w) lds_fmax(&q.w, p.w);
+}
+
+__device__ __forceinline__ bool hbox_reject(const float4 &b, float slb, float fx, float fy, float fe,
+                                            float gate2f) {
+    if (!(b.x <= b.z)) return true;
+    const float Dx = fmaxf(fmaxf(b.x - fx, fx - b.z), 0.0f);
+    const float Dy = fmaxf(fmaxf(b.y - fy, fy - b.w), 0.0f);
+    const float Cx = fmaxf(fabsf(b.x), fabsf(b.z)) * 2.3841858e-7f;
+    const float Cy = fmaxf(fabsf(b.y), fabsf(b.w)) * 2.3841858e-7f;
     const float lx = fmaxf(fmaf(Dx, 0.99999976f, -(fe + Cx)), 0.0f);
     const float ly = fmaxf(fmaf(Dy, 0.99999976f, -(fe + Cy)), 0.0f);
     return slb * fmaf(lx, lx, ly * ly) > gate2f;
 }
 
-struct Band {
-    uint32_t cx, cy;
-};
-
-__device__ __forceinline__ Band band_none() { return Band{0xffu, 0xffu}; }
-
-__device__ inline uint32_t band_codes(double f, double R, const SumFrame &fr) {
-    const double cell = fr.cell, org = fr.org;
-    if (!(isfinite(R) && isfinite(f) && cell > 0.0)) return 0xffu;
-    const double ta = (f + R - org) / cell + 1.0 + 1e-6;
-    const double tb = (f - R - org) / cell - 1e-6;
-    const double A = fmin(fmax(ceil(ta), 1.0), 256.0);
-    const double B = fmin(fmax(floor(tb), -1.0), 254.0);
-    return (uint32_t)(A - 1.0) | ((uint32_t)(B + 1.0) << 8);
-}
-
-__device__ inline Band gate_band(float fx, float fy, float fe, float slb, float gate2f, const SumFrame &fr) {
-    const double L = sqrt((double)gate2f / (double)slb);
-    const double base = L * (1.0 + 1e-5) + (double)fe * (1.0 + 1e-5);
-    const double Rx = (base + fabs((double)fx) * 1e-6) * (1.0 + 1e-5);
-    const double Ry = (base + fabs((double)fy) * 1e-6) * (1.0 + 1e-5);
-    Band b;
-    b.cx = band_codes(fx, Rx, fr);
-    b.cy = band_codes(fy, Ry, fr);
-    return b;
-}
-
+template <int MAXM>
+__device__ __forceinline__ unsigned row_open_mask(const float4 *rb, float slb, const MeasPack &ms, int m,
+                                                  float gate2f) {
+    static_assert(2 * MAXM <= 8, "a row's open mask is one byte");
+    const float4 b0 = rb[0], b1 = rb[1];
+    unsigned om = 0u;
+#pragma unroll
+    for (int k = 0; k < MAXM; ++k) {
+        if (k < m) {
+            if (!hbox_reject(b0, slb, ms.fx[k], ms.fy[k], ms.fe[k], gate2f)) om |= 1u << k;
+            if (!hbox_reject(b1, slb, ms.fx[k], ms.fy[k], ms.fe[k], gate2f)) om |= 1u << (MAXM + k);
+        }
+    }
+    return om;
+}
 
 __device__ __forceinline__ void lower_slb(float *slb, float s) {
     float v = (s > 0.0f) ? s : INFINITY;
diff --git a/fast-slam_amd/csrc/fs2_resample.hip b/fast-slam_amd/csrc/fs2_resample.hip
--- a/fast-slam_amd/csrc/fs2_resample.hip
+++ b/fast-slam_amd/csrc/fs2_resample.hip
@@ -1147,7 +1147,11 @@
     const uint32_t t = ref_tag(e);
     XDesc d;
     d.x = ((t ? t : (uint32_t)P.rank + 1u) << kRefShift) | ref_id(e);
-    d.y = P.map.bbox ? P.map.bbox[(i / kBlock) * kBBoxRows + k] : kSumOpen;
+    d.y = kSumOpen;
+    if (P.map.bbox) {
+        const float4 *rb = P.map.bbox + ((i / kBlock) * kBBoxRows + k) * 2;
+        d.y = hbox_codes(hbox_union(rb[0], rb[1]), P.map.frame);
+    }
     const int64_t c_i = P.iblk[P.nblk + i / kScanBlock] + P.rank_e[i];
     for (int p = 0; p < P.world; ++p) {
         const PackPlan &pl = P.plan[p];
@@ -1351,7 +1355,7 @@
     const int64_t m = (int64_t)blockIdx.x * kBlock + threadIdx.x;
     if (m == 0 && P.runs_n) *P.runs_n = 0u;
     const bool bb = P.obbox != nullptr && P.map.bbox != nullptr;
-    if (bb) lds_box_set(s_bb, threadIdx.x, kBoxEmpty);
+    if (bb) s_bb.b[threadIdx.x][0] = s_bb.b[threadIdx.x][1] = hbox_empty();
     double bv = -INFINITY;
     int64_t bi = INT64_MAX;
     unsigned slots = 0;
@@ -1422,7 +1426,11 @@
             for (int u = 0; u < 8; ++u) {
                 if (k0 + u < wrows) {
                     const uint32_t b = wave_box_union((k0 + u < rows && s < 0) ? eb[u] : kBoxEmpty);
-                    if ((threadIdx.x & 63) == 0) lds_box_merge(s_bb, k0 + u, b);
+                    if ((threadIdx.x & 63) == 0 && b != kBoxEmpty) {
+                        const float4 fb = hbox_of_codes(b, P.map.frame);
+                        lds_box_merge(s_bb, k0 + u, 0, fb);
+                        lds_box_merge(s_bb, k0 + u, 1, fb);
+                    }
                 }
             }
         }
@@ -1459,31 +1467,56 @@
         P.part_slots[blockIdx.x] = bs;
     }
     if (bb && (int)threadIdx.x < P.map.rows) {
-        uint32_t b = lds_box_get(s_bb, threadIdx.x);
-        for (int q = 0; q < nsb; ++q) b = box_union(b, P.map.bbox[(int64_t)s_sb[q] * kBBoxRows + threadIdx.x]);
-        P.obbox[(int64_t)blockIdx.x * kBBoxRows + threadIdx.x] = b;
+        float4 b0 = s_bb.b[threadIdx.x][0], b1 = s_bb.b[threadIdx.x][1];
+        for (int q = 0; q < nsb; ++q) {
+            const float4 *sb = P.map.bbox + ((int64_t)s_sb[q] * kBBoxRows + threadIdx.x) * 2;
+            b0 = hbox_union(b0, sb[0]);
+            b1 = hbox_union(b1, sb[1]);
+        }
+        float4 *ob = P.obbox + ((int64_t)blockIdx.x * kBBoxRows + threadIdx.x) * 2;
+        ob[0] = b0;
+        ob[1] = b1;
     }
 }
 
 __global__ __launch_bounds__(kBlock) void k_bbox_build(const MapRef map, const int32_t *cnt, int64_t n) {
     __shared__ BoxLds s_bb;
     const int64_t i = (int64_t)blockIdx.x * kBlock + threadIdx.x;
-    lds_box_set(s_bb, threadIdx.x, kBoxEmpty);
+    s_bb.b[threadIdx.x][0] = s_bb.b[threadIdx.x][1] = hbox_empty();
     const int c = (i < n) ? cnt[i] : 0;
     const int rows = (c + kPageSlots - 1) / kPageSlots;
     __syncthreads();
     const int wrows = wave_max_i(rows);
     for (int r = 0; r < wrows; ++r) {
-        uint32_t b = kBoxEmpty;
+        float4 hb[2] = {hbox_empty(), hbox_empty()};
         if (r < rows) {
             const float4 *mir = reinterpret_cast<const float4 *>(page_ptr_any(map, *pt_entry(map, r, i)));
-            b = page_box(mir, min(kPageSlots, c - r * kPageSlots), map.frame);
-        }
-        b = wave_box_union(b);
-        if ((threadIdx.x & 63) == 0) lds_box_merge(s_bb, r, b);
+            page_hboxes(mir, min(kPageSlots, c - r * kPageSlots), hb);
+        }
+        const float4 u0 = wave_hbox_union(hb[0]), u1 = wave_hbox_union(hb[1]);
+        if ((threadIdx.x & 63) == 0) {
+            lds_box_merge(s_bb, r, 0, u0);
+            lds_box_merge(s_bb, r, 1, u1);
+        }
     }
     __syncthreads();
-    if ((int)threadIdx.x < map.rows) map.bbox[(int64_t)blockIdx.x * kBBoxRows + threadIdx.x] = lds_box_get(s_bb, threadIdx.x);
+    if ((int)threadIdx.x < map.rows) {
+        float4 *ob = map.bbox + ((int64_t)blockIdx.x * kBBoxRows + threadIdx.x) * 2;
+        ob[0] = s_bb.b[threadIdx.x][0];
+        ob[1] = s_bb.b[threadIdx.x][1];
+    }
+}
+
+__global__ __launch_bounds__(kBlock) void k_bbox_clear(float4 *bbox, int64_t nboxes) {
+    const int64_t t = (int64_t)blockIdx.x * kBlock + threadIdx.x;
+    if (t < nboxes) bbox[t] = hbox_empty();
+}
+
+hipError_t launch_bbox_clear(float4 *bbox, int64_t nboxes, hipStream_t s) {
+    if (!bbox || nboxes <= 0) return hipSuccess;
+    hipLaunchKernelGGL(k_bbox_clear, dim3((unsigned)((nboxes + kBlock - 1) / kBlock)), dim3(kBlock), 0, s, bbox,
+                       nboxes);
+    return hipGetLastError();
 }
 
 hipError_t launch_bbox_build(MapRef map, const int32_t *cnt, hipStream_t s) {
diff --git a/fast-slam_amd/csrc/fs2_update.hip b/fast-slam_amd/csrc/fs2_update.hip
--- a/fast-slam_amd/csrc/fs2_update.hip
+++ b/fast-slam_amd/csrc/fs2_update.hip
@@ -60,7 +60,6 @@
 __global__ __launch_bounds__(kBlock) void k_candidates(const UpdateParams P) {
     if (P.stats->error_flags & 8) return;
     __shared__ uint64_t s_list[kMaxCand][kBlock];
-    __shared__ Band s_band[MAXM];
     __shared__ uint16_t s_rows[kBBoxRows];
     __shared__ uint8_t s_rmask[kBBoxRows];
     __shared__ int s_wc[kBlock / 64];
@@ -93,31 +92,18 @@
     const float slb = *map.slb;
     if (blockIdx.x == 0 && tid == 0 && P.slb_pass) *P.slb_pass = slb;
     const int rlast = map.rows - 1;
-    if (tid < MAXM) {
-        Band b = band_none();
-#pragma unroll
-        for (int k = 0; k < MAXM; ++k)
-            if (tid == k && k < P.m)
-                b = gate_band(P.meas.fx[k], P.meas.fy[k], P.meas.fe[k], slb, P.gate2f, map.frame);
-        s_band[tid] = b;
-    }
-    __syncthreads();
-    uint32_t bc[MAXM];
-#pragma unroll
-    for (int k = 0; k < MAXM; ++k) {
-        bc[k] = __builtin_amdgcn_readfirstlane(s_band[k].cx | (s_band[k].cy << 16));
-    }
     int nc = 0;
     unsigned visited = 0, groups = 0, opened = 0;
 
     const unsigned all_m = (1u << P.m) - 1u;
-    auto test_page = [&](const float4 *mir, int g, unsigned om) {
+    auto test_page = [&](const float4 *mir, int g, unsigned om8) {
         const int j0 = g * kPageSlots;
 #pragma unroll
         for (int u = 0; u < kScanGroup; ++u) {
             if (j0 + u < c) {
                 ++visited;
                 const float4 mv = mir[u];
+                const unsigned om = (u < kPageSlots / 2) ? om8 : (om8 >> MAXM);
                 const float cx = fabsf(mv.x) * 2.3841858e-7f;
                 const float cy = fabsf(mv.y) * 2.3841858e-7f;
                 bool hit = false;
@@ -154,7 +140,8 @@
     int nrows = map.rows;
     if (use_bb) {
         unsigned rm = 0u;
-        if (tid < map.rows) rm = box_open_mask<MAXM>(map.bbox[blk * kBBoxRows + tid], bc, P.m);
+        if (tid < map.rows)
+            rm = row_open_mask<MAXM>(map.bbox + (blk * kBBoxRows + tid) * 2, slb, P.meas, P.m, P.gate2f);
         const bool pass = rm != 0u;
         const uint64_t bm = __ballot(pass);
         const int wid = tid >> 6, lane = tid & 63;
@@ -186,7 +173,7 @@
         for (int u = 0; u + 1 < kDescAhead; ++u) dq[u] = dq[u + 1];
         dq[kDescAhead - 1] = ptrow[(int64_t)row_at(q + kDescAhead) * n];
         if (g * kPageSlots < c) ++groups;
-        const unsigned om = (g * kPageSlots < c) ? (use_bb ? (unsigned)s_rmask[q] : all_m) : 0u;
+        const unsigned om = (g * kPageSlots < c) ? (use_bb ? (unsigned)s_rmask[q] : (all_m | (all_m << MAXM))) : 0u;
         if (!__any(om)) continue;
         const char *pg = page_ptr(map.pool, om ? d : 0u);
         float4 mir[kScanGroup];
@@ -235,6 +222,8 @@
     __shared__ WaveScratch s_ws[kBlock / 64];
     __shared__ float4 s_mv[MAXM][kBlock];
     __shared__ BoxLds s_bb;
+    __shared__ uint8_t s_open[kBlock / 64][kBBoxRows];
+    static_assert(kBBoxRows == kBlock, "one thread per row box");
 
 #ifdef FS2_PHASE_TIMING
     unsigned long long ph_last = 0;
@@ -260,7 +249,7 @@
         map.pt = b.pt;
         map.bbox = b.bbox;
     }
-    if (map.bbox && tid < map.rows) lds_box_set(s_bb, tid, map.bbox[blk * kBBoxRows + tid]);
+    if (map.bbox) s_bb.b[tid][0] = s_bb.b[tid][1] = hbox_empty();
     __syncthreads();
 
     double px = 0.0, py = 0.0, pyaw = 0.0, w = 0.0;
@@ -294,8 +283,10 @@
     }
 
     const M2 R{P.R[0], P.R[1], P.R[2], P.R[3]};
-    auto box_note = [&](int row, uint32_t b) {
-        if (map.bbox) lds_box_merge(s_bb, row, b);
+    int nnote = 0;
+    auto box_note = [&](const float4 &mv) {
+        s_mv[nnote][tid] = mv;
+        ++nnote;
     };
     unsigned pend = live ? ((1u << P.m) - 1u) : 0u;
     unsigned visited = 0, candidates = 0, written = 0, amb = 0, appends = 0;
@@ -377,9 +368,19 @@
         if (overflow && ncl > 0) lo = cand_slot(P.cand[(int64_t)(ncl - 1) * n + il]);
         nmod_list = nmod;
     }
-    if (overflow && pend != 0u) {
+    const bool ovf = overflow && pend != 0u;
+    if (map.bbox && __any(ovf)) {
+        const float slbp = P.slb_pass ? *P.slb_pass : *map.slb;
+        for (int r = tid & 63; r < map.rows; r += 64) {
+            const unsigned rm = row_open_mask<MAXM>(map.bbox + (blk * kBBoxRows + r) * 2, slbp, P.meas, P.m, P.gate2f);
+            s_open[tid >> 6][r] = (uint8_t)(rm | (rm >> MAXM));
+        }
+        __builtin_amdgcn_fence(__ATOMIC_RELEASE, "workgroup");
+        __builtin_amdgcn_wave_barrier();
+        __builtin_amdgcn_fence(__ATOMIC_ACQUIRE, "workgroup");
+    }
+    if (ovf) {
         const int rows = (c + kPageSlots - 1) / kPageSlots;
-        const float slb = P.slb_pass ? *P.slb_pass : *map.slb;
 #pragma unroll
         for (int k = 0; k < MAXM; ++k) {
             s_ws[tid >> 6].ov.best[k][tid & 63] = INT_MAX;
@@ -389,13 +390,7 @@
         auto scan = [&](unsigned want, bool skip_mods) {
             for (int g = 0; g < rows; ++g) {
                 const Desc d = *pt_entry(map, g, il);
-                const uint32_t rb = map.bbox ? lds_box_get(s_bb, g) : kSumOpen;
-                unsigned open = 0u;
-#pragma unroll
-                for (int k = 0; k < MAXM; ++k)
-                    if (((want >> k) & 1u) &&
-                        !page_reject(rb, map.frame, slb, P.meas.fx[k], P.meas.fy[k], P.meas.fe[k], P.gate2f))
-                        open |= 1u << k;
+                const unsigned open = map.bbox ? (want & s_open[tid >> 6][g]) : want;
                 if (!open) continue;
                 const char *pg = page_ptr(map.pool, d);
                 for (int u = 0; u < kPageSlots && g * kPageSlots + u < c; ++u) {
@@ -586,10 +581,10 @@
                     if (u == canon[t]) id = rdesc[u];
                 const float4 m = s_mv[t][tid];
                 reinterpret_cast<float4 *>(page_ptr(map.pool, id))[j & (kPageSlots - 1)] = m;
-                box_note(rrow[t], point_box(m, map.frame));
             }
         }
         nrec = nmod;
+        nnote = nmod;
 #pragma unroll
         for (int t = 0; t < MAXM; ++t)
             if (t < nmod && canon[t] == t && ((cowm >> t) & 1u)) *pt_entry(map, rrow[t], il) = rdesc[t];
@@ -640,7 +635,7 @@
             s_lik[k][tid] = ekf_update(s, px, py, pyaw, mk, R, singular);
             const float4 mv = store_slot(map, pg, jh, s, r, jh);
             smin_w = fminf(smin_w, mirror_s(mv) > 0.0f ? mirror_s(mv) : INFINITY);
-            box_note(jh / kPageSlots, point_box(mv, map.frame));
+            box_note(mv);
             s_idx[k][tid] = (int16_t)(c + hit);
         } else {
             const Slot s{px + mk.d * cos(pyaw + mk.b), py + mk.d * sin(pyaw + mk.b),
@@ -654,14 +649,14 @@
                 arow = ja / kPageSlots;
                 const float4 mv = store_slot(map, page_ptr(map.pool, id), ja, s, r, ja);
                 smin_w = fminf(smin_w, mirror_s(mv) > 0.0f ? mirror_s(mv) : INFINITY);
-                box_note(arow, point_box(mv, map.frame));
+                box_note(mv);
                 ad = id | kOwned;
                 ad_new = true;
                 ++fresh;
             } else {
                 const float4 mv = store_slot(map, page_ptr(map.pool, ad), ja, s, r, ja);
                 smin_w = fminf(smin_w, mirror_s(mv) > 0.0f ? mirror_s(mv) : INFINITY);
-                box_note(arow, point_box(mv, map.frame));
+                box_note(mv);
             }
             s_idx[k][tid] = (int16_t)-1;
             ++nap;
@@ -671,6 +666,26 @@
     }
     if (arow >= 0 && ad_new) *pt_entry(map, arow, il) = ad;
     c += nap;
+
+    if (map.bbox) {
+#pragma unroll
+        for (int t = 0; t < MAXM; ++t) {
+            const bool v = t < nnote;
+            const uint64_t vm = __ballot(v);
+            if (vm == 0ull) break;
+            const float4 mv = s_mv[t][tid];
+            const int pos = (t < nmod) ? (int)((mods >> (16 * t)) & 0xffffu) : mirror_slot(mv);
+            const int key = v ? pos >> 2 : -1;
+            const int k0 = __shfl(key, __builtin_ctzll(vm), 64);
+            const float4 pb = v ? hbox_point(mv) : hbox_empty();
+            if (__all(!v || key == k0)) {
+                const float4 u = wave_hbox_union(pb);
+                if ((tid & 63) == 0) lds_box_merge(s_bb, k0 >> 1, k0 & 1, u);
+            } else if (v) {
+                lds_box_merge(s_bb, key >> 1, key & 1, pb);
+            }
+        }
+    }
 
     FS2_PHASE(5);
     unsigned hits = 0, refv = 0, napp = 0;
@@ -707,7 +722,16 @@
                               : 0xffffffffu);
     block_counters<kBlock, 0, kNumCounters>(cv, P.cpart, P.nblk, blk, assign, live ? w : 0.0,
                                             P.last_pass ? P.wpart + blk : nullptr);
-    if (map.bbox && tid < map.rows) map.bbox[blk * kBBoxRows + tid] = lds_box_get(s_bb, tid);
+    if (map.bbox && tid < map.rows) {
+#pragma unroll
+        for (int h = 0; h < 2; ++h) {
+            const float4 g = s_bb.b[tid][h];
+            if (g.x <= g.z) {
+                float4 *q = map.bbox + (blk * kBBoxRows + tid) * 2 + h;
+                *q = hbox_union(*q, g);
+            }
+        }
+    }
     lower_slb(map.slb, smin_w);
 }
 
@@ -727,7 +751,6 @@
 
 template <int MAXM, int PHASE>
 __global__ __launch_bounds__(kBlock) void k_localize(const LocalizeParams P) {
-    __shared__ Band s_band[MAXM];
     __shared__ uint16_t s_rows[kBBoxRows];
     __shared__ int s_wc[kBlock / 64];
     __shared__ unsigned long long s_base;
@@ -737,22 +760,13 @@
     const bool live = i < P.n;
     const MapRef map = P.map;
     const int c = live ? P.cnt[i] : 0;
-    if (tid < MAXM) {
-        Band b = band_none();
-#pragma unroll
-        for (int k = 0; k < MAXM; ++k)
-            if (tid == k && k < P.m) b = gate_band(P.meas.fx[k], P.meas.fy[k], P.meas.fe[k], *map.slb, P.gate2f, map.frame);
-        s_band[tid] = b;
-    }
-    __syncthreads();
-    uint32_t bc[MAXM];
-#pragma unroll
-    for (int k = 0; k < MAXM; ++k) bc[k] = __builtin_amdgcn_readfirstlane(s_band[k].cx | (s_band[k].cy << 16));
+    const float slb = *map.slb;
     const bool use_bb = map.bbox != nullptr;
     int nrows = map.rows;
     if (use_bb) {
         bool pass = false;
-        if (tid < map.rows) pass = box_open_mask<MAXM>(map.bbox[blk * kBBoxRows + tid], bc, P.m) != 0u;
+        if (tid < map.rows)
+            pass = row_open_mask<MAXM>(map.bbox + (blk * kBBoxRows + tid) * 2, slb, P.meas, P.m, P.gate2f) != 0u;
         const uint64_t bm = __ballot(pass);
         const int wid = tid >> 6, lane = tid & 63;
         if (lane == 0) s_wc[wid] = __popcll(bm);
```
